# ethnhe/FFB6D

Measured on NVIDIA H100. Metric: fused KNN+gather points/sec at 12288 pts, higher is better.
Workload: dtype f32

## Files before the change

### ffb6d_b200/_lib.py

```python
import ctypes as C
import os

_HERE = os.path.dirname(os.path.abspath(__file__))
LIB_PATH = os.path.join(_HERE, "libffb6d_b200.so")

OK = 0
ERR_INVALID = -1
ERR_CUDA = -2
ERR_WORKSPACE = -3
ERR_NO_DEVICE = -4
LAYOUT_NCS = 0
LAYOUT_NSC = 1
MAX_K = 64


class FFB6DError(RuntimeError):

    def __init__(self, code, msg):
        super().__init__("libffb6d_b200 error %d: %s" % (code, msg))
        self.code = code


def _load():
    if not os.path.exists(LIB_PATH):
        raise ImportError(
            "%s not found: the CUDA library has not been built (run __graft_entry__.build() "
            "or `make -C ffb6d_b200/csrc`). There is no CPU fallback." % LIB_PATH)
    lib = C.CDLL(LIB_PATH)
    vp, i64, sz, ci, fp = C.c_void_p, C.c_int64, C.c_size_t, C.c_int, C.c_float
    sig = {
        "ffb6d_version": (ci, []),
        "ffb6d_last_error": (C.c_char_p, []),
        "ffb6d_device_count": (ci, []),
        "ffb6d_launch_count": (C.c_uint64, []),
        "ffb6d_knn_workspace_bytes": (sz, [i64, i64, i64, ci]),
        "ffb6d_knn_batch": (ci, [vp, vp, i64, i64, i64, ci, vp, ci, vp, sz, vp]),
        "ffb6d_knn_batch_algo": (ci, [vp, vp, i64, i64, i64, ci, vp, ci, vp, sz, ci, vp]),
        "ffb6d_knn_grid_bytes": (sz, [i64, i64]),
        "ffb6d_knn_grid_query_bytes": (sz, [i64, i64]),
        "ffb6d_knn_grid_build": (ci, [vp, i64, i64, ci, vp, sz, vp]),
        "ffb6d_knn_grid_query": (ci, [vp, vp, i64, i64, i64, ci, vp, ci, vp, sz, vp, sz, vp]),
        "ffb6d_knn_grid_query_organized": (ci, [vp, vp, i64, i64, i64, ci, vp, ci, vp, sz, vp, sz, i64, vp]),
        "ffb6d_knn_subset_nn": (ci, [vp, vp, i64, i64, i64, vp, ci, vp, ci, vp, sz, vp]),
        "ffb6d_build_indices_workspace_bytes": (sz, [i64, i64, i64, i64, ci]),
        "ffb6d_build_indices": (ci, [vp, vp, vp, vp, i64, i64, i64, i64, ci, vp, ci, vp, sz, vp]),
        "ffb6d_knn_grid_tune": (None, [fp, ci]),
        "ffb6d_knn_grid_tune_k1": (None, [fp]),
        "ffb6d_knn_batch_host": (ci, [vp, sz, sz, sz, vp, sz, sz, vp]),
        "ffb6d_knn_host": (ci, [vp, sz, sz, vp, sz, sz, vp]),
        "ffb6d_gather_max_fwd": (ci, [vp, vp, ci, i64, i64, i64, i64, ci, ci, vp, vp]),
        "ffb6d_check_indices": (ci, [vp, ci, i64, i64, vp]),
        "ffb6d_gather_kernel_name": (C.c_char_p, [i64, i64, i64, i64, ci, ci]),
        "ffb6d_gather_max_bwd": (ci, [vp, vp, ci, vp, i64, i64, i64, i64, ci, ci, vp, vp]),
        "ffb6d_gather_neighbour_fwd": (ci, [vp, vp, ci, i64, i64, i64, i64, ci, vp, vp]),
        "ffb6d_gather_neighbour_bwd": (ci, [vp, vp, ci, i64, i64, i64, i64, ci, vp, vp]),
        "ffb6d_relative_pos_encoding_fwd": (ci, [vp, vp, ci, i64, i64, ci, vp, vp]),
        "ffb6d_fusion_mlp_fwd": (ci, [vp, i64, vp, i64, vp, vp, vp, i64, i64, i64, ci, fp, vp, vp]),
        "ffb6d_fusion_mlp_pack_bytes": (sz, [i64, i64]),
        "ffb6d_fusion_mlp_pack": (ci, [vp, i64, i64, vp, sz, vp]),
        "ffb6d_fusion_mlp_fwd_packed": (ci, [vp, i64, vp, i64, vp, vp, vp, i64, i64, i64, ci, fp, vp, vp]),
        "ffb6d_fusion_mlp_fwd_ex": (ci, [vp, i64, vp, i64, vp, vp, vp, i64, i64, i64, ci, fp, vp, vp, ci, i64, ci, vp, vp]),
        "ffb6d_bn_workspace_bytes": (sz, [i64, i64]),
        "ffb6d_bn_train_fwd": (ci, [vp, i64, i64, i64, vp, vp, fp, fp, vp, vp, ci, fp, vp, vp, vp, sz, vp]),
        "ffb6d_bn_train_bwd": (ci, [vp, vp, vp, i64, i64, i64, ci, fp, vp, vp, vp, vp, sz, vp]),
        "ffb6d_bn_sync_moments": (ci, [vp, i64, i64, i64, vp, vp, sz, vp]),
        "ffb6d_bn_sync_fwd": (ci, [vp, i64, i64, i64, vp, i64, vp, vp, fp, fp, vp, vp, ci, fp, vp, vp, vp, vp]),
        "ffb6d_bn_sync_bwd_sums": (ci, [vp, vp, vp, i64, i64, i64, ci, fp, vp, vp, vp, vp, sz, vp]),
        "ffb6d_bn_sync_bwd": (ci, [vp, vp, vp, i64, i64, i64, vp, i64, vp, ci, fp, vp, vp, sz, vp]),
        "ffb6d_act_bwd": (ci, [vp, vp, i64, ci, fp, vp, vp]),
        "ffb6d_fusion_mlp_wgrad": (ci, [vp, vp, i64, vp, i64, i64, i64, i64, vp, vp]),
        "ffb6d_segment_plan_bytes": (sz, [i64, i64, i64]),
        "ffb6d_segment_plan": (ci, [vp, ci, i64, i64, i64, vp, sz, vp]),
        "ffb6d_segment_sum": (ci, [vp, vp, sz, i64, i64, i64, i64, vp, vp]),
        "ffb6d_segment_csr_bytes": (sz, [i64, i64, i64]),
        "ffb6d_segment_csr": (ci, [vp, ci, i64, i64, i64, vp, sz, vp]),
        "ffb6d_segment_sum_csr": (ci, [vp, vp, sz, i64, i64, i64, i64, vp, vp]),
        "ffb6d_gather_max_bwd_det_workspace_bytes": (sz, [i64, i64, i64, i64, ci]),
        "ffb6d_gather_max_bwd_det": (ci, [vp, vp, ci, vp, i64, i64, i64, i64, ci, ci, vp, sz, vp, vp]),
        "ffb6d_gather_neighbour_bwd_det_workspace_bytes": (sz, [i64, i64, i64, ci]),
        "ffb6d_gather_neighbour_bwd_det": (ci, [vp, vp, ci, i64, i64, i64, i64, ci, vp, sz, vp, vp]),
        "ffb6d_fusion_mlp_wgrad_det_workspace_bytes": (sz, [i64, i64, i64, i64, i64]),
        "ffb6d_fusion_mlp_wgrad_det": (ci, [vp, vp, i64, vp, i64, i64, i64, i64, vp, sz, vp, vp]),
        "ffb6d_att_pool_bwd": (ci, [vp, i64, vp, i64, vp, vp, i64, i64, ci, vp, vp, vp, vp]),
        "ffb6d_lfa_att_pool_fused": (ci, [vp, vp, ci, vp, vp, vp, vp, vp, vp, vp, vp, vp, vp, vp, i64, i64, ci, i64, i64, fp, vp, vp]),
        "ffb6d_att_pool_fwd": (ci, [vp, i64, vp, i64, vp, i64, i64, ci, vp, vp]),
        "ffb6d_relative_pos_encoding_cm_fwd": (ci, [vp, vp, ci, i64, i64, ci, vp, vp]),
        "ffb6d_backproject": (ci, [vp, i64, i64, i64, vp, ci, vp, i64, vp, vp, vp, vp, vp]),
        "ffb6d_sample_pixels_workspace_bytes": (sz, [i64, i64, i64]),
        "ffb6d_sample_pixels": (ci, [vp, i64, i64, i64, fp, i64, C.c_uint64, vp, vp, vp, sz, vp]),
        "ffb6d_fill_depth_workspace_bytes": (sz, [i64, i64, i64]),
        "ffb6d_fill_depth": (ci, [vp, i64, i64, i64, fp, vp, vp, vp, sz, vp]),
        "ffb6d_mean_shift_workspace_bytes": (sz, [i64, i64]),
        "ffb6d_mean_shift_fit": (ci, [vp, vp, i64, i64, i64, fp, ci, vp, vp, vp, vp, vp, sz, vp]),
        "ffb6d_best_fit_transform": (ci, [vp, vp, i64, i64, vp, vp]),
        "ffb6d_grid_subsample_host": (ci, [vp, sz, vp, sz, vp, sz, fp, vp, vp, vp, C.POINTER(sz)]),
    }
    for name, (res, args) in sig.items():
        fn = getattr(lib, name)
        fn.restype = res
        fn.argtypes = args
    return lib, sorted(sig)


lib, SYMBOLS = _load()


def last_error():
    return lib.ffb6d_last_error().decode("utf-8", "replace")


def check(rc):
    if rc != OK:
        raise FFB6DError(rc, last_error())


def launch_count():
    return int(lib.ffb6d_launch_count())
```

### ffb6d_b200/csrc/api.cu

```cuda
#include "common.cuh"
#include "knn_common.cuh"

#include <atomic>
#include <mutex>
#include <string.h>
#include <stdlib.h>

namespace ffb6d {

static thread_local char g_err[512] = "";
static std::atomic<uint64_t> g_launches{0};

void set_error(const char *fmt, ...)
{
    va_list ap;
    va_start(ap, fmt);
    vsnprintf(g_err, sizeof(g_err), fmt, ap);
    va_end(ap);
}
void count_launch(int n) { g_launches.fetch_add((uint64_t)n, std::memory_order_relaxed); }

int current_device()
{
    int dev = 0;
    if (cudaGetDevice(&dev) != cudaSuccess) {
        cudaGetLastError();
        dev = 0;
    }
    return dev;
}

const DeviceInfo &device_info()
{
    static DeviceInfo info[kMaxDevices];
    static std::atomic<unsigned long long> known{0};
    const int dev = current_device() & (kMaxDevices - 1);
    if (!((known.load(std::memory_order_acquire) >> dev) & 1ull)) {
        DeviceInfo d;
        if (cudaDeviceGetAttribute(&d.num_sms, cudaDevAttrMultiProcessorCount, dev) != cudaSuccess || d.num_sms < 1) {
            cudaGetLastError();
            d.num_sms = 132;
        }
        if (cudaDeviceGetAttribute(&d.max_smem_optin, cudaDevAttrMaxSharedMemoryPerBlockOptin, dev) != cudaSuccess) {
            cudaGetLastError();
            d.max_smem_optin = 48 * 1024;
        }
        info[dev] = d;
        known.fetch_or(1ull << dev, std::memory_order_release);
    }
    return info[dev];
}

const Env &env()
{
    static const Env e = [] {
        Env v;
        auto on = [](const char *n) { const char *x = getenv(n); return x && *x && strcmp(x, "0") != 0; };
        v.gather_direct = on("FFB6D_GATHER_DIRECT");
        v.check_indices = on("FFB6D_CHECK_INDICES");
        v.grid_thread_search = on("FFB6D_GRID_THREAD_SEARCH");
        v.subset_nn = on("FFB6D_SUBSET_NN");
        const char *x;
        v.grid_scale = (x = getenv("FFB6D_GRID_SCALE")) ? (float)atof(x) : 1.0f;
        v.grid_scale_k1 = (x = getenv("FFB6D_GRID_SCALE_K1")) ? (float)atof(x) : 2.5f;
        v.grid_quantile = (x = getenv("FFB6D_GRID_QUANTILE")) ? atoi(x) : 17;
        if (v.grid_quantile < 0) v.grid_quantile = 0;
        if (v.grid_quantile > 31) v.grid_quantile = 31;
        return v;
    }();
    return e;
}

struct HostScratch {
    std::mutex mu;
    void *buf[4] = {nullptr, nullptr, nullptr, nullptr};
    size_t cap[4] = {0, 0, 0, 0};
    int device = -1;
    int get(int slot, size_t bytes, void **out)
    {
        int dev = 0;
        FFB6D_CUDA(cudaGetDevice(&dev));
        if (dev != device) {
            for (int s = 0; s < 4; ++s) {
                if (buf[s]) {
                    cudaSetDevice(device);
                    cudaFree(buf[s]);
                    cudaSetDevice(dev);
                }
                buf[s] = nullptr;
                cap[s] = 0;
            }
            device = dev;
        }
        if (bytes > cap[slot]) {
            if (buf[slot]) FFB6D_CUDA(cudaFree(buf[slot]));
            buf[slot] = nullptr;
            cap[slot] = 0;
            const size_t want = align_up(bytes + bytes / 4, 1 << 20);
            FFB6D_CUDA(cudaMalloc(&buf[slot], want));
            cap[slot] = want;
        }
        *out = buf[slot];
        return FFB6D_OK;
    }
};
static HostScratch g_scratch;

static int knn_dispatch(const float *support, const float *query, int64_t B, int64_t S, int64_t Q,
                        int K, void *idx_out, int idx_is_i64, void *ws, size_t ws_bytes, int algo,
                        cudaStream_t st)
{
    FFB6D_CHECK_ARG(B >= 0 && S >= 0 && Q >= 0, "knn: negative size (B=%lld S=%lld Q=%lld)",
                    (long long)B, (long long)S, (long long)Q);
    FFB6D_CHECK_ARG(K >= 1 && K <= FFB6D_MAX_K, "knn: K=%d outside [1,%d]", K, FFB6D_MAX_K);
    FFB6D_CHECK_ARG(S < (1ll << 31) && Q < (1ll << 31) && B < 65536, "knn: size too large");
    FFB6D_CHECK_ARG(algo >= 0 && algo <= 2, "knn: unknown algo %d", algo);
    if (B == 0 || Q == 0) return FFB6D_OK;
    FFB6D_CHECK_ARG(query && idx_out, "knn: null query/idx_out");
    FFB6D_CHECK_ARG(S == 0 || support, "knn: null support");
    if (algo == 0) algo = knn_grid_workspace_bytes(B, S, Q, K) ? 2 : 1;
    if (algo == 2) {
        const size_t need = knn_grid_workspace_bytes(B, S, Q, K);
        if (need == 0) {
            algo = 1;
        } else {
            if (!ws || ws_bytes < need) {
                set_error("knn: workspace of %zu bytes required, %zu given", need, ws_bytes);
                return FFB6D_ERR_WORKSPACE;
            }
            return knn_grid_launch(support, query, B, S, Q, K, idx_out, idx_is_i64, ws, ws_bytes, st);
        }
    }
    return knn_brute_launch(support, query, B, S, Q, K, idx_out, idx_is_i64, st);
}

}

using namespace ffb6d;

extern "C" {

int ffb6d_version(void) { return 1; }
const char *ffb6d_last_error(void) { return g_err; }
uint64_t ffb6d_launch_count(void) { return g_launches.load(std::memory_order_relaxed); }

int ffb6d_device_count(void)
{
    int n = 0;
    if (cudaGetDeviceCount(&n) != cudaSuccess) {
        cudaGetLastError();
        return 0;
    }
    return n;
}

size_t ffb6d_knn_workspace_bytes(int64_t B, int64_t S, int64_t Q, int K)
{
    if (B <= 0 || S <= 0 || Q <= 0 || K < 1 || K > FFB6D_MAX_K) return 0;
    return knn_grid_workspace_bytes(B, S, Q, K);
}

int ffb6d_knn_batch(const float *support, const float *query, int64_t B, int64_t S, int64_t Q,
                    int K, void *idx_out, int idx_is_i64, void *workspace, size_t workspace_bytes,
                    ffb6d_stream_t stream)
{
    return knn_dispatch(support, query, B, S, Q, K, idx_out, idx_is_i64, workspace,
                        workspace_bytes, 0, (cudaStream_t)stream);
}

int ffb6d_knn_batch_algo(const float *support, const float *query, int64_t B, int64_t S, int64_t Q,
                         int K, void *idx_out, int idx_is_i64, void *workspace,
                         size_t workspace_bytes, int algo, ffb6d_stream_t stream)
{
    return knn_dispatch(support, query, B, S, Q, K, idx_out, idx_is_i64, workspace,
                        workspace_bytes, algo, (cudaStream_t)stream);
}

size_t ffb6d_knn_grid_bytes(int64_t B, int64_t S)
{
    if (B <= 0 || S <= 0) return 0;
    return knn_grid_store_bytes(B, S);
}

size_t ffb6d_knn_grid_query_bytes(int64_t B, int64_t Q)
{
    if (B <= 0 || Q <= 0) return 0;
    return knn_grid_query_bytes(B, Q);
}

int ffb6d_knn_grid_build(const float *support, int64_t B, int64_t S, int K_hint, void *grid,
                         size_t grid_bytes, ffb6d_stream_t stream)
{
    FFB6D_CHECK_ARG(B >= 1 && S >= 1 && B < 65536 && S < (1ll << 31), "knn_grid_build: bad size");
    FFB6D_CHECK_ARG(K_hint >= 1 && K_hint <= FFB6D_MAX_K, "knn_grid_build: K_hint=%d outside [1,%d]",
                    K_hint, FFB6D_MAX_K);
    FFB6D_CHECK_ARG(support && grid, "knn_grid_build: null pointer");
    return knn_grid_build(support, B, S, K_hint, grid, grid_bytes, (cudaStream_t)stream);
}

int ffb6d_knn_grid_query(const float *support, const float *query, int64_t B, int64_t S, int64_t Q,
                         int K, void *idx_out, int idx_is_i64, const void *grid, size_t grid_bytes,
                         void *scratch, size_t scratch_bytes, ffb6d_stream_t stream)
{
    FFB6D_CHECK_ARG(B >= 0 && S >= 1 && Q >= 0 && B < 65536 && S < (1ll << 31) && Q < (1ll << 31),
                    "knn_grid_query: bad size");
    FFB6D_CHECK_ARG(K >= 1 && K <= FFB6D_MAX_K, "knn_grid_query: K=%d outside [1,%d]", K, FFB6D_MAX_K);
    if (B == 0 || Q == 0) return FFB6D_OK;
    FFB6D_CHECK_ARG(support && query && idx_out && grid && scratch, "knn_grid_query: null pointer");
    return knn_grid_query(support, query, B, S, Q, K, idx_out, idx_is_i64, grid, grid_bytes, scratch,
                          scratch_bytes, (cudaStream_t)stream);
}

int ffb6d_knn_grid_query_organized(const float *support, const float *query, int64_t B, int64_t S, int64_t Q,
                                   int K, void *idx_out, int idx_is_i64, const void *grid, size_t grid_bytes,
                                   void *scratch, size_t scratch_bytes, int64_t query_width, ffb6d_stream_t stream)
{
    FFB6D_CHECK_ARG(B >= 0 && S >= 1 && Q >= 0 && B < 65536 && S < (1ll << 31) && Q < (1ll << 31),
                    "knn_grid_query: bad size");
    FFB6D_CHECK_ARG(K >= 1 && K <= FFB6D_MAX_K, "knn_grid_query: K=%d outside [1,%d]", K, FFB6D_MAX_K);
    FFB6D_CHECK_ARG(query_width >= 0 && (query_width == 0 || Q % query_width == 0),
                    "knn_grid_query: query_width=%lld does not divide Q=%lld", (long long)query_width, (long long)Q);
    if (B == 0 || Q == 0) return FFB6D_OK;
    FFB6D_CHECK_ARG(support && query && idx_out && grid && scratch, "knn_grid_query: null pointer");
    return knn_grid_query(support, query, B, S, Q, K, idx_out, idx_is_i64, grid, grid_bytes, scratch,
                          scratch_bytes, (cudaStream_t)stream, query_width);
}

int ffb6d_knn_subset_nn(const float *support, const float *query, int64_t B, int64_t S, int64_t Q, const void *knn_idx,
                        int K_list, void *idx_out, int idx_is_i64, void *scratch, size_t scratch_bytes,
                        ffb6d_stream_t stream)
{
    FFB6D_CHECK_ARG(B >= 0 && S >= 1 && Q >= 0 && B < 65536 && S < (1ll << 31) && Q < (1ll << 31),
                    "knn_subset_nn: bad size");
    FFB6D_CHECK_ARG(S <= Q || Q == 0, "knn_subset_nn: the support (%lld rows) must be a row prefix of the %lld queries",
                    (long long)S, (long long)Q);
    FFB6D_CHECK_ARG(K_list >= 1 && K_list <= FFB6D_MAX_K, "knn_subset_nn: K_list=%d outside [1,%d]", K_list, FFB6D_MAX_K);
    if (B == 0 || Q == 0) return FFB6D_OK;
    FFB6D_CHECK_ARG(support && query && knn_idx && idx_out && scratch, "knn_subset_nn: null pointer");
    return knn_subset_nn_from_knn(support, query, B, S, Q, knn_idx, K_list, idx_out, idx_is_i64, scratch, scratch_bytes,
                                  (cudaStream_t)stream);
}

void ffb6d_knn_grid_tune(float cell_scale, int quantile) { knn_grid_tune(cell_scale, quantile); }
void ffb6d_knn_grid_tune_k1(float cell_scale_k1) { knn_grid_tune_k1(cell_scale_k1); }

int ffb6d_knn_batch_host(const float *batch_data, size_t batch_size, size_t npts, size_t dim,
                         const float *queries, size_t nqueries, size_t K, long *batch_indices)
{
    FFB6D_CHECK_ARG(dim == 3, "knn_batch_host: dim=%zu, only 3 is supported", dim);
    FFB6D_CHECK_ARG(K >= 1 && K <= FFB6D_MAX_K, "knn_batch_host: K=%zu outside [1,%d]", K,
                    FFB6D_MAX_K);
    if (batch_size == 0 || nqueries == 0) return FFB6D_OK;
    FFB6D_CHECK_ARG(queries && batch_indices && (npts == 0 || batch_data),
                    "knn_batch_host: null pointer");
    if (ffb6d_device_count() == 0) {
        set_error("knn_batch_host: no CUDA device visible");
        return FFB6D_ERR_NO_DEVICE;
    }
    std::lock_guard<std::mutex> lock(g_scratch.mu);
    const size_t sup_b = batch_size * npts * 3 * sizeof(float);
    const size_t qry_b = batch_size * nqueries * 3 * sizeof(float);
    const size_t idx_b = batch_size * nqueries * K * sizeof(long);
    const size_t ws_b = ffb6d_knn_workspace_bytes((int64_t)batch_size, (int64_t)npts,
                                                  (int64_t)nqueries, (int)K);
    void *d_sup, *d_qry, *d_idx, *d_ws;
    int rc;
    if ((rc = g_scratch.get(0, sup_b ? sup_b : 16, &d_sup))) return rc;
    if ((rc = g_scratch.get(1, qry_b, &d_qry))) return rc;
    if ((rc = g_scratch.get(2, idx_b, &d_idx))) return rc;
    if ((rc = g_scratch.get(3, ws_b ? ws_b : 16, &d_ws))) return rc;
    cudaStream_t st = 0;
    if (sup_b) FFB6D_CUDA(cudaMemcpyAsync(d_sup, batch_data, sup_b, cudaMemcpyHostToDevice, st));
    FFB6D_CUDA(cudaMemcpyAsync(d_qry, queries, qry_b, cudaMemcpyHostToDevice, st));
    rc = knn_dispatch((const float *)d_sup, (const float *)d_qry, (int64_t)batch_size,
                      (int64_t)npts, (int64_t)nqueries, (int)K, d_idx, 1, d_ws, ws_b, 0, st);
    if (rc) return rc;
    FFB6D_CUDA(cudaMemcpyAsync(batch_indices, d_idx, idx_b, cudaMemcpyDeviceToHost, st));
    FFB6D_CUDA(cudaStreamSynchronize(st));
    return FFB6D_OK;
}

int ffb6d_knn_host(const float *points, size_t npts, size_t dim, const float *queries,
                   size_t nqueries, size_t K, long *indices)
{
    return ffb6d_knn_batch_host(points, 1, npts, dim, queries, nqueries, K, indices);
}

}
```

### ffb6d_b200/csrc/common.cuh

```cuda
#pragma once
#include <cuda_runtime.h>
#include <stdint.h>
#include <stdio.h>
#include <stdarg.h>
#include <atomic>

#include "../../include/ffb6d_b200.h"

namespace ffb6d {

void set_error(const char *fmt, ...);
void count_launch(int n = 1);

#define FFB6D_CHECK_ARG(cond, ...)                         \
    do {                                                   \
        if (!(cond)) {                                     \
            ::ffb6d::set_error(__VA_ARGS__);               \
            return FFB6D_ERR_INVALID;                      \
        }                                                  \
    } while (0)

#define FFB6D_CUDA(call)                                                             \
    do {                                                                             \
        cudaError_t e__ = (call);                                                    \
        if (e__ != cudaSuccess) {                                                    \
            ::ffb6d::set_error("%s failed: %s (%s:%d)", #call, cudaGetErrorString(e__), \
                               __FILE__, __LINE__);                                  \
            return FFB6D_ERR_CUDA;                                                   \
        }                                                                            \
    } while (0)

#define FFB6D_LAUNCH_OK(name)                                                          \
    do {                                                                               \
        cudaError_t e__ = cudaGetLastError();                                          \
        if (e__ != cudaSuccess) {                                                      \
            ::ffb6d::set_error("launch of %s failed: %s", name, cudaGetErrorString(e__)); \
            return FFB6D_ERR_CUDA;                                                     \
        }                                                                              \
        ::ffb6d::count_launch();                                                       \
    } while (0)

static inline int64_t ceil_div(int64_t a, int64_t b) { return (a + b - 1) / b; }
static inline size_t align_up(size_t x, size_t a) { return (x + a - 1) / a * a; }

constexpr int kMaxDevices = 64;
struct DeviceInfo {
    int num_sms;
    int max_smem_optin;
};
int current_device();
const DeviceInfo &device_info();
static inline int num_sms() { return device_info().num_sms; }

#define FFB6D_OPTIN_SMEM(kern, bytes)                                                              \
    do {                                                                                           \
        static std::atomic<unsigned long long> done__{0};                                          \
        const int dev__ = ::ffb6d::current_device() & (::ffb6d::kMaxDevices - 1);                  \
        if (!((done__.load(std::memory_order_relaxed) >> dev__) & 1ull)) {                         \
            FFB6D_CUDA(cudaFuncSetAttribute(kern, cudaFuncAttributeMaxDynamicSharedMemorySize,     \
                                            (int)(bytes)));                                        \
            done__.fetch_or(1ull << dev__, std::memory_order_relaxed);                             \
        }                                                                                          \
    } while (0)

int wgrad_small_launch(const float *grad_z, const float *x1, int64_t C1, const float *x2, int64_t C2, int64_t B, int64_t Co,
                       int64_t P, float *grad_w, cudaStream_t st);
int64_t wgrad_small_splits(int64_t B, int64_t P);
int wgrad_small_det_launch(const float *grad_z, const float *x1, int64_t C1, const float *x2, int64_t C2, int64_t B,
                           int64_t Co, int64_t P, float *part, cudaStream_t st);

struct Env {
    bool gather_direct;
    bool check_indices;
    bool grid_thread_search;
    bool subset_nn;
    float grid_scale, grid_scale_k1;
    int grid_quantile;
};
const Env &env();

__device__ __forceinline__ float ref_sqdist(float qx, float qy, float qz, float sx, float sy,
                                            float sz)
{
    const float dx = __fsub_rn(qx, sx);
    const float dy = __fsub_rn(qy, sy);
    const float dz = __fsub_rn(qz, sz);
    return __fadd_rn(__fadd_rn(__fmul_rn(dx, dx), __fmul_rn(dy, dy)), __fmul_rn(dz, dz));
}

}
```

### ffb6d_b200/csrc/knn_common.cuh

```cuda
#pragma once
#include "common.cuh"

namespace ffb6d {

template <int KCAP>
struct TopK {
    float d[KCAP];
    int i[KCAP];

    __device__ __forceinline__ void init()
    {
#pragma unroll
        for (int j = 0; j < KCAP; ++j) {
            d[j] = __int_as_float(0x7f800000);
            i[j] = 0;
        }
    }
    __device__ __forceinline__ float worst() const { return d[KCAP - 1]; }
    __device__ __forceinline__ float kth(int K) const
    {
        float v = d[KCAP - 1];
#pragma unroll
        for (int j = KCAP - 2; j >= 0; --j) v = (j >= K - 1) ? d[j] : v;
        return v;
    }
    __device__ __forceinline__ int worst_idx() const { return i[KCAP - 1]; }

    __device__ __forceinline__ void push_ordered(float dist, int id)
    {
#pragma unroll
        for (int j = KCAP - 1; j > 0; --j) {
            const bool shift = d[j - 1] > dist;
            const bool here = !shift && (d[j] > dist);
            const float nd = shift ? d[j - 1] : (here ? dist : d[j]);
            const int ni = shift ? i[j - 1] : (here ? id : i[j]);
            d[j] = nd;
            i[j] = ni;
        }
        if (d[0] > dist) {
            d[0] = dist;
            i[0] = id;
        }
    }

    __device__ __forceinline__ bool accepts(float dist, int id) const
    {
        return dist < d[KCAP - 1] || (dist == d[KCAP - 1] && id < i[KCAP - 1]);
    }

    __device__ __forceinline__ void push_any(float dist, int id)
    {
#pragma unroll
        for (int j = KCAP - 1; j > 0; --j) {
            const bool shift = d[j - 1] > dist || (d[j - 1] == dist && i[j - 1] > id);
            const bool after = d[j] > dist || (d[j] == dist && i[j] > id);
            const bool here = !shift && after;
            const float nd = shift ? d[j - 1] : (here ? dist : d[j]);
            const int ni = shift ? i[j - 1] : (here ? id : i[j]);
            d[j] = nd;
            i[j] = ni;
        }
        if (d[0] > dist || (d[0] == dist && i[0] > id)) {
            d[0] = dist;
            i[0] = id;
        }
    }
};

int knn_brute_launch(const float *support, const float *query, int64_t B, int64_t S, int64_t Q,
                     int K, void *idx_out, int idx_is_i64, cudaStream_t st);
size_t knn_grid_workspace_bytes(int64_t B, int64_t S, int64_t Q, int K);
int knn_grid_launch(const float *support, const float *query, int64_t B, int64_t S, int64_t Q,
                    int K, void *idx_out, int idx_is_i64, void *workspace, size_t workspace_bytes,
                    cudaStream_t st);
void knn_grid_tune(float cell_scale, int quantile);
void knn_grid_tune_k1(float cell_scale_k1);
size_t knn_grid_store_bytes(int64_t B, int64_t S);
size_t knn_grid_query_bytes(int64_t B, int64_t Q);
int knn_grid_build(const float *support, int64_t B, int64_t S, int K, void *grid_mem,
                   size_t grid_bytes, cudaStream_t st);
int knn_grid_query(const float *support, const float *query, int64_t B, int64_t S, int64_t Q, int K,
                   void *idx_out, int idx_is_i64, const void *grid_mem, size_t grid_bytes,
                   void *scratch, size_t scratch_bytes, cudaStream_t st, int64_t query_width = 0);

int knn_subset_nn_from_knn(const float *support, const float *query, int64_t B, int64_t S, int64_t Q, const void *knn,
                           int KL, void *idx_out, int idx_is_i64, void *scratch, size_t scratch_bytes, cudaStream_t st);

}
```

### ffb6d_b200/csrc/knn_grid.cu

```cuda
#include "common.cuh"
#include "knn_common.cuh"

#include <algorithm>
#include <cooperative_groups.h>
#include <math.h>
#include <stdlib.h>

namespace ffb6d {

constexpr int RMAX = 4;
constexpr int N_SAMPLES = 32;
constexpr int BUILD_CTAS = 8;
constexpr int BUILD_THREADS = 512;
constexpr int BUILD_WARPS = BUILD_THREADS / 32;
constexpr int BUILD_GT = BUILD_CTAS * BUILD_THREADS;
static_assert(N_SAMPLES == BUILD_CTAS * 4 && BUILD_WARPS == 16, "4 samples per CTA, 4 warps per sample");

struct __align__(16) GridParams {
    float lo[3];
    float h;
    float inv_h;
    float slack;
    int n[3];
    int ncells;
    float hi[3];
    int pad[3];
};
static_assert(sizeof(GridParams) == 64, "GridParams layout");

struct __align__(16) QueryState {
    int ovf_count;
    int dup_count;
    int rep_q;
    int pad;
};

struct GridStore {
    GridParams *params;
    int *cursor;
    int *rank;
    float4 *sorted;
    size_t maxc;
    size_t bytes;
};

struct QueryScratch {
    QueryState *state;
    int *ovf;
    size_t bytes;
};

static size_t max_cells_for(int64_t S)
{
    size_t m = (size_t)S * 8;
    if (m < 4096) m = 4096;
    if (m > ((size_t)1 << 22)) m = (size_t)1 << 22;
    return (m + 4095) / 4096 * 4096;
}

static GridStore carve_grid(void *base, int64_t B, int64_t S)
{
    GridStore w;
    w.maxc = max_cells_for(S);
    size_t off = 0;
    char *p = (char *)base;
    auto take = [&](size_t bytes) {
        char *r = p + off;
        off = align_up(off + bytes, 256);
        return r;
    };
    w.params = (GridParams *)take((size_t)B * sizeof(GridParams));
    w.cursor = (int *)take((size_t)B * w.maxc * sizeof(int));
    w.rank = (int *)take((size_t)B * (size_t)S * sizeof(int));
    w.sorted = (float4 *)take((size_t)B * (size_t)S * sizeof(float4));
    w.bytes = off;
    return w;
}

static QueryScratch carve_query(void *base, int64_t B, int64_t Q)
{
    QueryScratch w;
    size_t off = 0;
    char *p = (char *)base;
    w.state = (QueryState *)(p + off);
    off = align_up(off + (size_t)B * sizeof(QueryState), 256);
    w.ovf = (int *)(p + off);
    off = align_up(off + (size_t)B * (size_t)Q * sizeof(int), 256);
    w.bytes = off;
    return w;
}

size_t knn_grid_store_bytes(int64_t B, int64_t S) { return carve_grid(nullptr, B, S).bytes; }
size_t knn_grid_query_bytes(int64_t B, int64_t Q) { return carve_query(nullptr, B, Q).bytes; }

static bool grid_worthwhile(int64_t B, int64_t S, int64_t Q, int K)
{
    (void)B;
    (void)K;
    return S >= 512 && (double)S * (double)Q >= 2.0e5;
}

size_t knn_grid_workspace_bytes(int64_t B, int64_t S, int64_t Q, int K)
{
    if (!grid_worthwhile(B, S, Q, K)) return 0;
    return knn_grid_store_bytes(B, S) + knn_grid_query_bytes(B, Q);
}

__device__ __forceinline__ int cell_of(float p, float lo, float inv_h, int n)
{
    const int c = (int)floorf((p - lo) * inv_h);
    return min(max(c, 0), n - 1);
}

__global__ void __cluster_dims__(BUILD_CTAS, 1, 1) __launch_bounds__(BUILD_THREADS)
grid_build_kernel(const float *__restrict__ support, int S, int K, int maxc, float cell_scale, int quantile,
                  GridParams *__restrict__ params, int *__restrict__ cursor_all, int *__restrict__ rank_all,
                  float4 *__restrict__ sorted_all)
{
    namespace cg = cooperative_groups;
    cg::cluster_group cluster = cg::this_cluster();
    const int crank = (int)cluster.block_rank();
    const int b = blockIdx.y;
    const int tid = threadIdx.x, lane = tid & 31, wid = tid >> 5;
    const int gtid = crank * BUILD_THREADS + tid;
    const float *sup = support + (size_t)b * S * 3;
    int *cur = cursor_all + (size_t)b * maxc;
    int *rnk = rank_all + (size_t)b * S;
    float4 *sorted = sorted_all + (size_t)b * S;
    const float INF = __int_as_float(0x7f800000);

    __shared__ float s_red[6][BUILD_WARPS];
    __shared__ float s_box[6];
    __shared__ float s_cand[4][4][4];
    __shared__ float s_est[4];
    __shared__ float s_all[N_SAMPLES];
    __shared__ float s_pick;
    __shared__ GridParams s_P;
    __shared__ int s_tot[BUILD_CTAS];
    __shared__ int s_wsum[BUILD_WARPS];
    __shared__ int s_base;

    {
        float mn[3] = {INF, INF, INF}, mx[3] = {-INF, -INF, -INF};
        for (int s = gtid; s < S; s += BUILD_GT) {
#pragma unroll
            for (int a = 0; a < 3; ++a) {
                const float v = __ldg(sup + (size_t)s * 3 + a);
                mn[a] = fminf(mn[a], v);
                mx[a] = fmaxf(mx[a], v);
            }
        }
#pragma unroll
        for (int a = 0; a < 3; ++a) {
#pragma unroll
            for (int o = 16; o > 0; o >>= 1) {
                mn[a] = fminf(mn[a], __shfl_xor_sync(0xffffffffu, mn[a], o));
                mx[a] = fmaxf(mx[a], __shfl_xor_sync(0xffffffffu, mx[a], o));
            }
            if (lane == 0) {
                s_red[a][wid] = mn[a];
                s_red[3 + a][wid] = mx[a];
            }
        }
        if (tid < BUILD_CTAS) s_tot[tid] = 0;
        __syncthreads();
        if (wid == 0) {
#pragma unroll
            for (int a = 0; a < 3; ++a) {
                float u = lane < BUILD_WARPS ? s_red[a][lane] : INF, v = lane < BUILD_WARPS ? s_red[3 + a][lane] : -INF;
#pragma unroll
                for (int o = 16; o > 0; o >>= 1) {
                    u = fminf(u, __shfl_xor_sync(0xffffffffu, u, o));
                    v = fmaxf(v, __shfl_xor_sync(0xffffffffu, v, o));
                }
                if (lane == 0) {
                    s_box[a] = u;
                    s_box[3 + a] = v;
                }
            }
        }
    }
    {
        const int stride = max((S + 4095) / 4096, (K + 3) / 4);
        const int kk = max(1, (K + stride - 1) / stride);
        const int smp = crank * 4 + (wid >> 2), w4 = wid & 3;
        const int me = (int)((((long long)smp * S) / N_SAMPLES + S / (2 * N_SAMPLES)) % max(S, 1));
        float out[4] = {INF, INF, INF, INF};
        if (S > 1) {
            const float qx = __ldg(sup + (size_t)me * 3), qy = __ldg(sup + (size_t)me * 3 + 1),
                        qz = __ldg(sup + (size_t)me * 3 + 2);
            TopK<4> t4;
            t4.init();
            const int nsub = (S + stride - 1) / stride;
            for (int i0 = w4 * 32 + lane; i0 < nsub; i0 += 4 * 128) {
                float px[4], py[4], pz[4];
#pragma unroll
                for (int u = 0; u < 4; ++u) {
                    const int s = min((i0 + u * 128) * stride, S - 1);
                    px[u] = __ldg(sup + (size_t)s * 3);
                    py[u] = __ldg(sup + (size_t)s * 3 + 1);
                    pz[u] = __ldg(sup + (size_t)s * 3 + 2);
                }
#pragma unroll
                for (int u = 0; u < 4; ++u) {
                    const int i = i0 + u * 128, s = i * stride;
                    const float d = ref_sqdist(qx, qy, qz, px[u], py[u], pz[u]);
                    if (i < nsub && s != me && d < t4.worst()) t4.push_ordered(d, s);
                }
            }
#pragma unroll
            for (int round = 0; round < 4; ++round) {
                if (round >= kk) break;
                float m = t4.d[0];
#pragma unroll
                for (int o = 16; o > 0; o >>= 1) m = fminf(m, __shfl_xor_sync(0xffffffffu, m, o));
                const unsigned who = __ballot_sync(0xffffffffu, t4.d[0] == m);
                if (lane == __ffs(who) - 1) {
                    t4.d[0] = t4.d[1];
                    t4.d[1] = t4.d[2];
                    t4.d[2] = t4.d[3];
                    t4.d[3] = INF;
                }
                out[round] = m;
            }
        }
        if (lane == 0) {
#pragma unroll
            for (int j = 0; j < 4; ++j) s_cand[wid >> 2][w4][j] = out[j];
        }
        __syncthreads();
        if (wid < 4) {
            const float mine = lane < 16 ? s_cand[wid][lane >> 2][lane & 3] : INF;
            int rank = 0;
            for (int j = 0; j < 16; ++j) {
                const float o = __shfl_sync(0xffffffffu, mine, j);
                rank += (o < mine || (o == mine && j < lane)) ? 1 : 0;
            }
            if (lane < 16 && rank == kk - 1) {
                const float r = (S > 1) ? sqrtf(mine) * sqrtf((float)K / (float)(kk * stride)) : 0.f;
                s_est[wid] = (r == r && r < INF) ? r : 0.f;
            }
        }
    }
    cluster.sync();
    if (crank == 0) {
        if (wid == 0) {
            s_all[lane] = cluster.map_shared_rank(s_est, lane >> 2)[lane & 3];
            if (lane < 6) {
                float v = (lane < 3) ? INF : -INF;
                for (int c = 0; c < BUILD_CTAS; ++c) {
                    const float o = cluster.map_shared_rank(s_box, c)[lane];
                    v = (lane < 3) ? fminf(v, o) : fmaxf(v, o);
                }
                s_red[lane][0] = v;
            }
            __syncwarp();
            const float mine = s_all[lane];
            int rank = 0;
            for (int j = 0; j < N_SAMPLES; ++j) {
                const float o = s_all[j];
                rank += (o < mine || (o == mine && j < lane)) ? 1 : 0;
            }
            if (rank == quantile) s_pick = mine;
            __syncwarp();
            if (lane == 0) {
                float mn[3], mx[3];
                for (int a = 0; a < 3; ++a) {
                    mn[a] = s_red[a][0];
                    mx[a] = s_red[3 + a][0];
                }
                const float r_est = s_pick;
                GridParams P;
                float L[3], scale = 0.f;
                bool finite = true;
                for (int a = 0; a < 3; ++a) {
                    L[a] = mx[a] - mn[a];
                    finite = finite && isfinite(L[a]) && isfinite(mn[a]);
                    scale = fmaxf(scale, fmaxf(fabsf(mn[a]), fabsf(mx[a])));
                    P.lo[a] = mn[a];
                    P.hi[a] = mx[a];
                }
                const float l1 = fmaxf(L[0], fmaxf(L[1], L[2]));
                const float l3 = fminf(L[0], fminf(L[1], L[2]));
                const float l2 = L[0] + L[1] + L[2] - l1 - l3;
                float h = cell_scale * r_est;
                if (!(h > 0.f)) h = sqrtf((float)K * l1 * l2 / (float)max(S, 1));
                if (!(h > 0.f)) h = l1 * (float)K / (float)max(S, 1);
                int n[3] = {1, 1, 1};
                if (finite && h > 0.f && l1 > 0.f) {
                    for (int it = 0; it < 200; ++it) {
                        double prod = 1.0;
                        for (int a = 0; a < 3; ++a) {
                            const float f = floorf(L[a] / h);
                            n[a] = (f >= 4.0e6f) ? 4000000 : (int)f + 1;
                            prod *= (double)n[a];
                        }
                        if (prod <= (double)maxc) break;
                        h *= 1.2f;
                        if (it == 199) n[0] = n[1] = n[2] = 1;
                    }
                }
                const bool single = (n[0] == 1 && n[1] == 1 && n[2] == 1);
                P.h = single ? INF : h;
                P.inv_h = single ? 0.f : 1.0f / h;
                P.slack = 1e-5f * (scale + l1) + 1e-30f;
                P.n[0] = n[0];
                P.n[1] = n[1];
                P.n[2] = n[2];
                P.ncells = n[0] * n[1] * n[2];
                for (int a = 0; a < 3; ++a) P.pad[a] = 0;
                s_P = P;
                params[b] = P;
            }
        }
    }
    cluster.sync();
    if (crank != 0 && tid < 16)
        reinterpret_cast<float *>(&s_P)[tid] = reinterpret_cast<const float *>(cluster.map_shared_rank(&s_P, 0))[tid];
    __syncthreads();
    const GridParams P = s_P;
    const int ncells = P.ncells;
    const int slice = ((ncells + BUILD_CTAS * 128 - 1) / (BUILD_CTAS * 128)) * 128;
    {
        int4 *c4 = reinterpret_cast<int4 *>(cur);
        const int n4 = min((ncells + 3) / 4, maxc / 4);
        for (int i = gtid; i < n4; i += BUILD_GT) c4[i] = make_int4(0, 0, 0, 0);
    }
    cluster.sync();
    {
        int acc = 0;
        const int iters = (S + BUILD_GT - 1) / BUILD_GT;
        for (int it = 0; it < iters; ++it) {
            const int s = it * BUILD_GT + gtid;
            int sl = -1;
            if (s < S) {
                const float *p = sup + (size_t)s * 3;
                const int cx = cell_of(__ldg(p), P.lo[0], P.inv_h, P.n[0]);
                const int cy = cell_of(__ldg(p + 1), P.lo[1], P.inv_h, P.n[1]);
                const int cz = cell_of(__ldg(p + 2), P.lo[2], P.inv_h, P.n[2]);
                const int cell = (cz * P.n[1] + cy) * P.n[0] + cx;
                rnk[s] = atomicAdd(cur + cell, 1);
                sl = cell / slice;
            }
#pragma unroll
            for (int j = 0; j < BUILD_CTAS; ++j) {
                const int v = __popc(__ballot_sync(0xffffffffu, sl == j));
                if (lane == j) acc += v;
            }
        }
        if (lane < BUILD_CTAS && acc) atomicAdd(&s_tot[lane], acc);
    }
    cluster.sync();
    {
        if (wid == 0) {
            int t = 0;
            if (lane < BUILD_CTAS)
                for (int c = 0; c < BUILD_CTAS; ++c) t += cluster.map_shared_rank(s_tot, c)[lane];
            int before = (lane < crank) ? t : 0;
#pragma unroll
            for (int o = 16; o > 0; o >>= 1) before += __shfl_xor_sync(0xffffffffu, before, o);
            if (lane == 0) s_base = before;
        }
        const int lo = crank * slice, hi = min(ncells, lo + slice);
        const int run = ((slice / 128 + BUILD_WARPS - 1) / BUILD_WARPS) * 128;
        const int wlo = min(hi, lo + wid * run), whi = min(hi, wlo + run);
        int tot = 0;
        for (int i = wlo + 4 * lane; i < whi; i += 128) {
            const int4 v = *reinterpret_cast<const int4 *>(cur + i);
            tot += v.x + (i + 1 < whi ? v.y : 0) + (i + 2 < whi ? v.z : 0) + (i + 3 < whi ? v.w : 0);
        }
#pragma unroll
        for (int o = 16; o > 0; o >>= 1) tot += __shfl_xor_sync(0xffffffffu, tot, o);
        if (lane == 0) s_wsum[wid] = tot;
        __syncthreads();
        int carry = s_base;
        for (int w = 0; w < wid; ++w) carry += s_wsum[w];
        for (int i0 = wlo; i0 < whi; i0 += 128) {
            const int i = i0 + 4 * lane;
            int4 v = make_int4(0, 0, 0, 0);
            if (i < whi) {
                v = *reinterpret_cast<const int4 *>(cur + i);
                if (i + 1 >= whi) v.y = 0;
                if (i + 2 >= whi) v.z = 0;
                if (i + 3 >= whi) v.w = 0;
            }
            const int t = v.x + v.y + v.z + v.w;
            int incl = t;
#pragma unroll
            for (int o = 1; o < 32; o <<= 1) {
                const int u = __shfl_up_sync(0xffffffffu, incl, o);
                if (lane >= o) incl += u;
            }
            const int start = carry + incl - t;
            if (i < whi) {
                int4 e;
                e.x = start + v.x;
                e.y = e.x + v.y;
                e.z = e.y + v.z;
                e.w = e.z + v.w;
                if (i + 3 < whi) {
                    *reinterpret_cast<int4 *>(cur + i) = e;
                } else {
                    cur[i] = e.x;
                    if (i + 1 < whi) cur[i + 1] = e.y;
                    if (i + 2 < whi) cur[i + 2] = e.z;
                }
            }
            carry += __shfl_sync(0xffffffffu, incl, 31);
        }
    }
    cluster.sync();
    for (int s = gtid; s < S; s += BUILD_GT) {
        const float *p = sup + (size_t)s * 3;
        const float x = __ldg(p), y = __ldg(p + 1), z = __ldg(p + 2);
        const int cx = cell_of(x, P.lo[0], P.inv_h, P.n[0]);
        const int cy = cell_of(y, P.lo[1], P.inv_h, P.n[1]);
        const int cz = cell_of(z, P.lo[2], P.inv_h, P.n[2]);
        const int cell = (cz * P.n[1] + cy) * P.n[0] + cx;
        const int pos = (cell > 0 ? cur[cell - 1] : 0) + rnk[s];
        sorted[pos] = make_float4(x, y, z, __int_as_float(s));
    }
}

__constant__ signed char kRowOrder[81][2] = {{0,0}, {-1,0}, {0,-1}, {0,1}, {1,0}, {-1,-1}, {-1,1}, {1,-1}, {1,1}, {-2,0}, {0,-2}, {0,2}, {2,0}, {-2,-1}, {-2,1}, {-1,-2}, {-1,2}, {1,-2}, {1,2}, {2,-1}, {2,1}, {-2,-2}, {-2,2}, {2,-2}, {2,2}, {-3,0}, {0,-3}, {0,3}, {3,0}, {-3,-1}, {-3,1}, {-1,-3}, {-1,3}, {1,-3}, {1,3}, {3,-1}, {3,1}, {-3,-2}, {-3,2}, {-2,-3}, {-2,3}, {2,-3}, {2,3}, {3,-2}, {3,2}, {-3,-3}, {-3,3}, {3,-3}, {3,3}, {-4,0}, {0,-4}, {0,4}, {4,0}, {-4,-1}, {-4,1}, {-1,-4}, {-1,4}, {1,-4}, {1,4}, {4,-1}, {4,1}, {-4,-2}, {-4,2}, {-2,-4}, {-2,4}, {2,-4}, {2,4}, {4,-2}, {4,2}, {-4,-3}, {-4,3}, {-3,-4}, {-3,4}, {3,-4}, {3,4}, {4,-3}, {4,3}, {-4,-4}, {-4,4}, {4,-4}, {4,4}};

__device__ __forceinline__ float slab_dist2(float q, float lo, float h, int c, float slack)
{
    const float a = lo + (float)c * h, b = lo + (float)(c + 1) * h;
    const float d = fmaxf(fmaxf(a - q, q - b) - slack, 0.f);
    return d * d;
}

template <int KCAP>
__device__ __forceinline__ bool thread_search(float qx, float qy, float qz, int K, const GridParams &Ps,
                                              const int *__restrict__ cell_end, const float4 *__restrict__ sorted,
                                              TopK<KCAP> &top)
{
    const int nx = Ps.n[0], ny = Ps.n[1], nz = Ps.n[2];
    const float h = Ps.h, slack = Ps.slack;
    const int cx = cell_of(qx, Ps.lo[0], Ps.inv_h, nx);
    const int cy = cell_of(qy, Ps.lo[1], Ps.inv_h, ny);
    const int cz = cell_of(qz, Ps.lo[2], Ps.inv_h, nz);
    const float INF = __int_as_float(0x7f800000);
    const float out = fmaxf(fmaxf(fmaxf(Ps.lo[0] - qx, qx - Ps.hi[0]), fmaxf(Ps.lo[1] - qy, qy - Ps.hi[1])),
                            fmaxf(Ps.lo[2] - qz, qz - Ps.hi[2]));
    bool done = false;
    auto scan_range = [&](int beg, int end) {
        for (int p = beg; p < end; p += 4) {
            float4 c[4];
#pragma unroll
            for (int u = 0; u < 4; ++u) c[u] = __ldg(sorted + min(p + u, end - 1));
#pragma unroll
            for (int u = 0; u < 4; ++u) {
                const float d = ref_sqdist(qx, qy, qz, c[u].x, c[u].y, c[u].z);
                const int id = __float_as_int(c[u].w);
                if (p + u < end && top.accepts(d, id)) top.push_any(d, id);
            }
        }
    };
    auto cells = [&](int row, int a, int b2) {
        const int beg = (row + a > 0) ? __ldg(cell_end + row + a - 1) : 0;
        scan_range(beg, __ldg(cell_end + row + b2));
    };
    const int r_first = (out > (float)RMAX * h) ? RMAX + 1 : 1;
    int px0 = 1, px1 = 0, py0 = 1, py1 = 0, pz0 = 1, pz1 = 0;
    for (int r = r_first; r <= RMAX && !done; ++r) {
        const int x0 = max(cx - r, 0), x1 = min(cx + r, nx - 1);
        const int y0 = max(cy - r, 0), y1 = min(cy + r, ny - 1);
        const int z0 = max(cz - r, 0), z1 = min(cz + r, nz - 1);
        const int e0 = (2 * r - 1) * (2 * r - 1) * (r > r_first ? 1 : 0);
        const int e1 = (2 * r + 1) * (2 * r + 1);
        if (r > r_first) {
            for (int e = 0; e < e0; ++e) {
                const int z = cz + kRowOrder[e][0], y = cy + kRowOrder[e][1];
                if (z < pz0 || z > pz1 || y < py0 || y > py1) continue;
                const int row = (z * ny + y) * nx;
                if (x0 < px0) cells(row, x0, px0 - 1);
                if (x1 > px1) cells(row, px1 + 1, x1);
            }
        }
        for (int e = e0; e < e1; ++e) {
            const int z = cz + kRowOrder[e][0], y = cy + kRowOrder[e][1];
            if (z < z0 || z > z1 || y < y0 || y > y1) continue;
            const float dmin2 = slab_dist2(qy, Ps.lo[1], h, y, slack) + slab_dist2(qz, Ps.lo[2], h, z, slack);
            if (dmin2 > top.kth(K)) continue;
            cells((z * ny + y) * nx, x0, x1);
        }
        px0 = x0; px1 = x1; py0 = y0; py1 = y1; pz0 = z0; pz1 = z1;
        float m = INF;
        if (x0 > 0) m = fminf(m, qx - (Ps.lo[0] + (float)x0 * h));
        if (x1 < nx - 1) m = fminf(m, (Ps.lo[0] + (float)(x1 + 1) * h) - qx);
        if (y0 > 0) m = fminf(m, qy - (Ps.lo[1] + (float)y0 * h));
        if (y1 < ny - 1) m = fminf(m, (Ps.lo[1] + (float)(y1 + 1) * h) - qy);
        if (z0 > 0) m = fminf(m, qz - (Ps.lo[2] + (float)z0 * h));
        if (z1 < nz - 1) m = fminf(m, (Ps.lo[2] + (float)(z1 + 1) * h) - qz);
        if (m == INF) {
            done = true;
        } else {
            const float ms = m - slack;
            const float kth = top.kth(K);
            done = ms > 0.f && kth <= ms * ms * (1.0f - 1e-5f);
        }
    }
    return done;
}

__device__ __forceinline__ void register_overflow(const float *__restrict__ query, int Q, int b, int q, float qx, float qy,
                                                  float qz, QueryState *state_all, int *__restrict__ ovf_all)
{
    QueryState *Pw = state_all + b;
    int rep = *(volatile int *)&Pw->rep_q;
    if (rep == 0) rep = atomicCAS(&Pw->rep_q, 0, q + 1);
    rep -= 1;
    bool dup = false;
    if (rep != -1 && rep != q) {
        const float *rp = query + ((size_t)b * Q + rep) * 3;
        dup = (__ldg(rp) == qx) && (__ldg(rp + 1) == qy) && (__ldg(rp + 2) == qz);
    }
    if (dup) {
        auto g = cooperative_groups::coalesced_threads();
        int base = 0;
        if (g.thread_rank() == 0) base = atomicAdd(&Pw->dup_count, (int)g.size());
        const int slot = g.shfl(base, 0) + (int)g.thread_rank();
        ovf_all[(size_t)b * Q + (Q - 1 - slot)] = q;
    } else {
        auto g = cooperative_groups::coalesced_threads();
        int base = 0;
        if (g.thread_rank() == 0) base = atomicAdd(&Pw->ovf_count, (int)g.size());
        const int slot = g.shfl(base, 0) + (int)g.thread_rank();
        ovf_all[(size_t)b * Q + slot] = q;
    }
}

template <int KCAP, typename IdxT, bool SELF>
__global__ void __launch_bounds__(128)
grid_search_kernel(const float *__restrict__ query, int S, int Q, int K,
                   const GridParams *__restrict__ params_all, const int *__restrict__ cursor_all,
                   size_t cursor_stride, const float4 *__restrict__ sorted_all,
                   IdxT *__restrict__ idx_out, QueryState *state_all, int *__restrict__ ovf_all)
{
    const int b = blockIdx.y;
    const int t = blockIdx.x * blockDim.x + threadIdx.x;
    if (t >= Q) return;
    const GridParams Ps = params_all[b];
    const int *cell_end = cursor_all + (size_t)b * cursor_stride;
    const float4 *sorted = sorted_all + (size_t)b * S;
    float qx, qy, qz;
    int q;
    if (SELF) {
        const float4 me = sorted[t];
        qx = me.x;
        qy = me.y;
        qz = me.z;
        q = __float_as_int(me.w);
    } else {
        const float *qp = query + ((size_t)b * Q + t) * 3;
        qx = __ldg(qp);
        qy = __ldg(qp + 1);
        qz = __ldg(qp + 2);
        q = t;
    }
    TopK<KCAP> top;
    top.init();
    if (thread_search<KCAP>(qx, qy, qz, K, Ps, cell_end, sorted, top)) {
        IdxT *o = idx_out + ((size_t)b * Q + q) * K;
#pragma unroll
        for (int j = 0; j < KCAP; ++j)
            if (j < K) o[j] = (IdxT)top.i[j];
        return;
    }
    register_overflow(query, Q, b, q, qx, qy, qz, state_all, ovf_all);
}

typedef unsigned long long key_t64;

__device__ __forceinline__ key_t64 make_key(float d, int i)
{
    return ((key_t64)__float_as_uint(d) << 32) | (unsigned)i;
}
__device__ __forceinline__ float key_dist(key_t64 k) { return __uint_as_float((unsigned)(k >> 32)); }

constexpr key_t64 KEY_EMPTY = 0x7f80000000000000ull;
constexpr key_t64 KEY_INVALID = 0x7f8000007fffffffull;

__device__ __forceinline__ void warp_minmax(key_t64 &k, int j, bool keep_min)
{
    const key_t64 o = __shfl_xor_sync(0xffffffffu, k, j);
    if ((o < k) == keep_min) k = o;
}

__device__ __forceinline__ void warp_sort(key_t64 &k, int lane)
{
#pragma unroll
    for (int kk = 2; kk <= 32; kk <<= 1) {
#pragma unroll
        for (int j = kk >> 1; j > 0; j >>= 1) {
            const bool up = (lane & kk) == 0;
            warp_minmax(k, j, ((lane & j) == 0) == up);
        }
    }
}

__device__ __forceinline__ void warp_list_offer(key_t64 &mine, key_t64 cand, int K, int lane, bool &list_empty)
{
    const unsigned FULL = 0xffffffffu;
    if (list_empty) {
        warp_sort(cand, lane);
        mine = (cand < KEY_EMPTY) ? cand : KEY_EMPTY;
        list_empty = false;
        return;
    }
    const key_t64 thr = __shfl_sync(FULL, mine, K - 1);
    unsigned mask = __ballot_sync(FULL, cand < thr);
    if (__popc(mask) > 12) {
        warp_sort(cand, lane);
        const key_t64 rev = __shfl_sync(FULL, cand, 31 - lane);
        if (rev < mine) mine = rev;
#pragma unroll
        for (int jj = 16; jj > 0; jj >>= 1) warp_minmax(mine, jj, (lane & jj) == 0);
        if (mine > KEY_EMPTY) mine = KEY_EMPTY;
    } else {
        while (mask) {
            const int src = __ffs(mask) - 1;
            mask &= mask - 1;
            const key_t64 x = __shfl_sync(FULL, cand, src);
            const key_t64 pred = __shfl_up_sync(FULL, mine, 1);
            if (x < mine) mine = (lane > 0 && x < pred) ? pred : x;
        }
    }
}


template <typename IdxT>
__device__ __forceinline__ void register_far_k1(const float *__restrict__ query, int Q, int b, int q, float qx, float qy,
                                                float qz, QueryState *state_all, int *__restrict__ ovf_all,
                                                IdxT *__restrict__ idx_out)
{
    QueryState *Pw = state_all + b;
    int rep = *(volatile int *)&Pw->rep_q;
    if (rep == 0) rep = atomicCAS(&Pw->rep_q, 0, q + 1);
    rep -= 1;
    bool dup = false;
    if (rep != -1 && rep != q) {
        const float *rp = query + ((size_t)b * Q + rep) * 3;
        dup = (__ldg(rp) == qx) && (__ldg(rp + 1) == qy) && (__ldg(rp + 2) == qz);
    }
    if (dup) {
        idx_out[(size_t)b * Q + q] = (IdxT)-1;
    } else {
        auto g = cooperative_groups::coalesced_threads();
        int base = 0;
        if (g.thread_rank() == 0) base = atomicAdd(&Pw->ovf_count, (int)g.size());
        const int slot = g.shfl(base, 0) + (int)g.thread_rank();
        ovf_all[(size_t)b * Q + slot] = q;
    }
}

template <typename IdxT>
__global__ void __launch_bounds__(256)
grid_far_fill_kernel(int Q, const QueryState *__restrict__ state_all, IdxT *__restrict__ idx_out)
{
    const int b = blockIdx.y;
    const int rep = state_all[b].rep_q - 1;
    if (rep < 0) return;
    IdxT *o = idx_out + (size_t)b * Q;
    const IdxT v = o[rep];
    for (int q = blockIdx.x * blockDim.x + threadIdx.x; q < Q; q += gridDim.x * blockDim.x)
        if (o[q] == (IdxT)-1) o[q] = v;
}

template <typename IdxT, int NW>
__global__ void __launch_bounds__(NW * 32, 1024 / (NW * 32))
grid_search_k1_tile_kernel(const float *__restrict__ query, int S, int Q, int qw, int qh, int tiles_x, int n_tiles, int exact_div,
                            const GridParams *__restrict__ params_all, const int *__restrict__ cursor_all,
                            size_t cursor_stride, const float4 *__restrict__ sorted_all,
                            IdxT *__restrict__ idx_out, QueryState *state_all, int *__restrict__ ovf_all)
{
    constexpr int TW = 8, TH = 4;
    constexpr int MAX_ROWS = 32, MAX_X = 8;
    constexpr int TILE_CAND = 128;
    __shared__ float4 s_cand[NW][TILE_CAND];
    __shared__ int s_list[NW * 32];
    __shared__ int s_count;
    const unsigned FULL = 0xffffffffu;
    const int b = blockIdx.y;
    const int lane = threadIdx.x & 31, wid = threadIdx.x >> 5;
    const int tile = blockIdx.x * NW + wid;
    const GridParams Ps = params_all[b];
    const int *cell_end = cursor_all + (size_t)b * cursor_stride;
    const float4 *sorted = sorted_all + (size_t)b * S;
    const float INF = __int_as_float(0x7f800000);
    if (threadIdx.x == 0) s_count = 0;
    if (NW > 1) __syncthreads();
    else __syncwarp();

    const int trow = exact_div ? tile / tiles_x : (int)(((float)tile + 0.5f) * (1.0f / (float)tiles_x));
    const int px = (tile - trow * tiles_x) * TW + (lane & (TW - 1)), py = trow * TH + (lane >> 3);
    const bool inimg = tile < n_tiles && px < qw && py < qh;
    const int q = inimg ? py * qw + px : 0;
    float qx = 0.f, qy = 0.f, qz = 0.f;
    if (inimg) {
        const float *qp = query + ((size_t)b * Q + q) * 3;
        qx = __ldg(qp);
        qy = __ldg(qp + 1);
        qz = __ldg(qp + 2);
    }
    const int nx = Ps.n[0], ny = Ps.n[1], nz = Ps.n[2];
    const float h = Ps.h, slack = Ps.slack;
    const float out = fmaxf(fmaxf(fmaxf(Ps.lo[0] - qx, qx - Ps.hi[0]), fmaxf(Ps.lo[1] - qy, qy - Ps.hi[1])),
                            fmaxf(Ps.lo[2] - qz, qz - Ps.hi[2]));
    int state = !inimg ? 3 : ((out > (float)RMAX * h || !(qx == qx && qy == qy && qz == qz)) ? 2 : 1);
    const bool part = state == 1;
    const int cx = cell_of(qx, Ps.lo[0], Ps.inv_h, nx);
    const int cy = cell_of(qy, Ps.lo[1], Ps.inv_h, ny);
    const int cz = cell_of(qz, Ps.lo[2], Ps.inv_h, nz);
    const int big = 0x3fffffff;
    int X0 = __reduce_min_sync(FULL, part ? cx : big), X1 = __reduce_max_sync(FULL, part ? cx : -1);
    int Y0 = __reduce_min_sync(FULL, part ? cy : big), Y1 = __reduce_max_sync(FULL, part ? cy : -1);
    int Z0 = __reduce_min_sync(FULL, part ? cz : big), Z1 = __reduce_max_sync(FULL, part ? cz : -1);
    if (X1 >= 0) {
        X0 = max(X0 - 1, 0); X1 = min(X1 + 1, nx - 1);
        Y0 = max(Y0 - 1, 0); Y1 = min(Y1 + 1, ny - 1);
        Z0 = max(Z0 - 1, 0); Z1 = min(Z1 + 1, nz - 1);
        const int by = Y1 - Y0 + 1, nrows = by * (Z1 - Z0 + 1);
        if (nrows <= MAX_ROWS && X1 - X0 + 1 <= MAX_X) {
            int beg = 0, end = 0;
            if (lane < nrows) {
                const int rz = (int)(((float)lane + 0.5f) * (1.0f / (float)by));
                const int row = ((Z0 + rz) * ny + (Y0 + lane - rz * by)) * nx;
                beg = (row + X0 > 0) ? __ldg(cell_end + row + X0 - 1) : 0;
                end = __ldg(cell_end + row + X1);
            }
            const int cnt = end - beg;
            int incl = cnt;
#pragma unroll
            for (int o = 1; o < 32; o <<= 1) {
                const int u = __shfl_up_sync(FULL, incl, o);
                if (lane >= o) incl += u;
            }
            const int total = __shfl_sync(FULL, incl, 31);
            const int excl = incl - cnt;
            float4 *stage = s_cand[wid];
            key_t64 best = KEY_EMPTY;
            for (int c0 = 0; c0 < total; c0 += TILE_CAND) {
                const int n = min(TILE_CAND, total - c0);
                const int n4 = (n + 3) & ~3;
                __syncwarp();
                for (int u0 = 0; u0 < n4; u0 += 32) {
                    const int j = c0 + u0 + lane;
                    int seg = 0;
#pragma unroll
                    for (int step = 16; step > 0; step >>= 1) {
                        const int v = __shfl_sync(FULL, incl, seg + step - 1);
                        if (v <= j) seg += step;
                    }
                    const int sb = __shfl_sync(FULL, beg, seg & 31), se = __shfl_sync(FULL, excl, seg & 31);
                    float4 c = make_float4(INF, INF, INF, __int_as_float(0x7fffffff));
                    if (j < total) c = __ldg(sorted + sb + (j - se));
                    if (u0 + lane < n4) stage[u0 + lane] = c;
                }
                __syncwarp();
                for (int p = 0; p < n4; p += 4) {
                    float4 c[4];
#pragma unroll
                    for (int u = 0; u < 4; ++u) c[u] = stage[p + u];
#pragma unroll
                    for (int u = 0; u < 4; ++u) {
                        const key_t64 k = make_key(ref_sqdist(qx, qy, qz, c[u].x, c[u].y, c[u].z), __float_as_int(c[u].w));
                        best = k < best ? k : best;
                    }
                }
            }
            if (part) {
                const float bd = key_dist(best);
                float m = INF;
                if (X0 > 0) m = fminf(m, qx - (Ps.lo[0] + (float)X0 * h));
                if (X1 < nx - 1) m = fminf(m, (Ps.lo[0] + (float)(X1 + 1) * h) - qx);
                if (Y0 > 0) m = fminf(m, qy - (Ps.lo[1] + (float)Y0 * h));
                if (Y1 < ny - 1) m = fminf(m, (Ps.lo[1] + (float)(Y1 + 1) * h) - qy);
                if (Z0 > 0) m = fminf(m, qz - (Ps.lo[2] + (float)Z0 * h));
                if (Z1 < nz - 1) m = fminf(m, (Ps.lo[2] + (float)(Z1 + 1) * h) - qz);
                const float ms = m - slack;
                const bool ok = (m == INF) ? (bd < INF || S == 0) : (ms > 0.f && bd <= ms * ms * (1.0f - 1e-5f));
                if (ok) {
                    idx_out[(size_t)b * Q + q] = (IdxT)(unsigned)(best & 0xffffffffu);
                    state = 0;
                }
            }
        }
    }
    if (state == 1) s_list[atomicAdd(&s_count, 1)] = q;
    if (NW > 1) __syncthreads();
    else __syncwarp();
    const int n_retry = s_count;
    int q2 = -1;
    float rx = 0.f, ry = 0.f, rz = 0.f;
    bool retry_failed = false;
    if ((int)threadIdx.x < n_retry) {
        q2 = s_list[threadIdx.x];
        const float *qp = query + ((size_t)b * Q + q2) * 3;
        rx = __ldg(qp);
        ry = __ldg(qp + 1);
        rz = __ldg(qp + 2);
        TopK<1> top;
        top.init();
        if (thread_search<1>(rx, ry, rz, 1, Ps, cell_end, sorted, top))
            idx_out[(size_t)b * Q + q2] = (IdxT)top.i[0];
        else
            retry_failed = true;
    }
    if (retry_failed) register_overflow(query, Q, b, q2, rx, ry, rz, state_all, ovf_all);
    if (state == 2) register_far_k1<IdxT>(query, Q, b, q, qx, qy, qz, state_all, ovf_all, idx_out);
}

template <typename IdxT, bool SELF>
__global__ void __launch_bounds__(256, 5)
grid_search_warp_kernel(const float *__restrict__ query, int S, int Q, int K,
                        const GridParams *__restrict__ params_all, const int *__restrict__ cursor_all,
                        size_t cursor_stride, const float4 *__restrict__ sorted_all,
                        IdxT *__restrict__ idx_out, QueryState *state_all, int *__restrict__ ovf_all)
{
    const unsigned FULL = 0xffffffffu;
    const int b = blockIdx.y;
    const int lane = threadIdx.x & 31;
    const int t = blockIdx.x * (blockDim.x >> 5) + (threadIdx.x >> 5);
    if (t >= Q) return;
    const GridParams Ps = params_all[b];
    const int *cell_end = cursor_all + (size_t)b * cursor_stride;
    const float4 *sorted = sorted_all + (size_t)b * S;
    float qx, qy, qz;
    int q;
    if (SELF) {
        const float4 me = __ldg(sorted + t);
        qx = me.x;
        qy = me.y;
        qz = me.z;
        q = __float_as_int(me.w);
    } else {
        const float *qp = query + ((size_t)b * Q + t) * 3;
        qx = __ldg(qp);
        qy = __ldg(qp + 1);
        qz = __ldg(qp + 2);
        q = t;
    }
    const int nx = Ps.n[0], ny = Ps.n[1], nz = Ps.n[2];
    const float h = Ps.h, slack = Ps.slack;
    const int cx = cell_of(qx, Ps.lo[0], Ps.inv_h, nx);
    const int cy = cell_of(qy, Ps.lo[1], Ps.inv_h, ny);
    const int cz = cell_of(qz, Ps.lo[2], Ps.inv_h, nz);
    const float INF = __int_as_float(0x7f800000);
    const float out = fmaxf(fmaxf(fmaxf(Ps.lo[0] - qx, qx - Ps.hi[0]), fmaxf(Ps.lo[1] - qy, qy - Ps.hi[1])),
                            fmaxf(Ps.lo[2] - qz, qz - Ps.hi[2]));

    auto margin = [&](int r) {
        float m = INF;
        if (cx - r > 0) m = fminf(m, qx - (Ps.lo[0] + (float)(cx - r) * h));
        if (cx + r < nx - 1) m = fminf(m, (Ps.lo[0] + (float)(cx + r + 1) * h) - qx);
        if (cy - r > 0) m = fminf(m, qy - (Ps.lo[1] + (float)(cy - r) * h));
        if (cy + r < ny - 1) m = fminf(m, (Ps.lo[1] + (float)(cy + r + 1) * h) - qy);
        if (cz - r > 0) m = fminf(m, qz - (Ps.lo[2] + (float)(cz - r) * h));
        if (cz + r < nz - 1) m = fminf(m, (Ps.lo[2] + (float)(cz + r + 1) * h) - qz);
        return m;
    };

    key_t64 mine = KEY_EMPTY;
    bool list_empty = true;
    bool done = false;
    int r = (out > (float)RMAX * h) ? RMAX + 1 : 1;
    int e_prev = 0;
    int px0 = 0, px1 = -1;
    while (r <= RMAX) {
        const int x0 = max(cx - r, 0), x1 = min(cx + r, nx - 1);
        const int y0 = max(cy - r, 0), y1 = min(cy + r, ny - 1);
        const int z0 = max(cz - r, 0), z1 = min(cz + r, nz - 1);
        const int e_end = (2 * r + 1) * (2 * r + 1);
        const int nseg = 2 * e_prev + (e_end - e_prev);
        for (int s0 = 0; s0 < nseg; s0 += 32) {
            const float kth_now = key_dist(__shfl_sync(FULL, mine, K - 1));
            const int sidx = s0 + lane;
            int beg = 0, end = 0;
            if (sidx < nseg) {
                const bool old = sidx < 2 * e_prev;
                const int e = old ? (sidx >> 1) : (sidx - e_prev);
                const int z = cz + kRowOrder[e][0], y = cy + kRowOrder[e][1];
                int a = x0, c = x1;
                if (old) {
                    if (sidx & 1) a = px1 + 1;
                    else c = px0 - 1;
                }
                if (z >= z0 && z <= z1 && y >= y0 && y <= y1 && a <= c) {
                    const float dmin2 = slab_dist2(qy, Ps.lo[1], h, y, slack) + slab_dist2(qz, Ps.lo[2], h, z, slack);
                    if (!(dmin2 > kth_now)) {
                        const int row = (z * ny + y) * nx;
                        beg = (row + a > 0) ? __ldg(cell_end + row + a - 1) : 0;
                        end = __ldg(cell_end + row + c);
                    }
                }
            }
            const int cnt = end - beg;
            int incl = cnt;
#pragma unroll
            for (int o = 1; o < 32; o <<= 1) {
                const int u = __shfl_up_sync(FULL, incl, o);
                if (lane >= o) incl += u;
            }
            const int total = __shfl_sync(FULL, incl, 31);
            const int excl = incl - cnt;
            for (int j0 = 0; j0 < total; j0 += 32) {
                const int j = j0 + lane;
                int seg = 0;
#pragma unroll
                for (int step = 16; step > 0; step >>= 1) {
                    const int v = __shfl_sync(FULL, incl, seg + step - 1);
                    if (v <= j) seg += step;
                }
                const int sb = __shfl_sync(FULL, beg, seg);
                const int se = __shfl_sync(FULL, excl, seg);
                key_t64 cand = KEY_INVALID;
                if (j < total) {
                    const float4 c = __ldg(sorted + sb + (j - se));
                    cand = make_key(ref_sqdist(qx, qy, qz, c.x, c.y, c.z), __float_as_int(c.w));
                }
                warp_list_offer(mine, cand, K, lane, list_empty);
            }
        }
        e_prev = e_end;
        px0 = x0;
        px1 = x1;
        const float m = margin(r);
        const float kth = key_dist(__shfl_sync(FULL, mine, K - 1));
        if (m == INF) {
            done = true;
            break;
        }
        const float ms = m - slack;
        if (ms > 0.f && kth <= ms * ms * (1.0f - 1e-5f)) {
            done = true;
            break;
        }
        int rn = r + 1;
        if (kth < INF) {
            const float need = sqrtf(kth) * (1.0f + 1e-4f) + slack;
            while (rn <= RMAX && margin(rn) < need) ++rn;
        }
        r = rn;
    }
    if (done) {
        if (lane < K) idx_out[((size_t)b * Q + q) * K + lane] = (IdxT)(unsigned)(mine & 0xffffffffu);
        return;
    }
    if (lane == 0) {
        QueryState *Pw = state_all + b;
        const int rep = atomicCAS(&Pw->rep_q, 0, q + 1) - 1;
        bool dup = false;
        if (rep != -1 && rep != q) {
            const float *rp = query + ((size_t)b * Q + rep) * 3;
            dup = (__ldg(rp) == qx) && (__ldg(rp + 1) == qy) && (__ldg(rp + 2) == qz);
        }
        if (dup) {
            const int slot = atomicAdd(&Pw->dup_count, 1);
            ovf_all[(size_t)b * Q + (Q - 1 - slot)] = q;
        } else {
            const int slot = atomicAdd(&Pw->ovf_count, 1);
            ovf_all[(size_t)b * Q + slot] = q;
        }
    }
}

template <int W>
__device__ __forceinline__ void group_minmax(key_t64 &k, int j, bool keep_min)
{
    const key_t64 o = __shfl_xor_sync(0xffffffffu, k, j, W);
    if ((o < k) == keep_min) k = o;
}

template <int W>
__device__ __forceinline__ void group_sort(key_t64 &k, int sub)
{
#pragma unroll
    for (int kk = 2; kk <= W; kk <<= 1) {
#pragma unroll
        for (int j = kk >> 1; j > 0; j >>= 1) {
            const bool up = (sub & kk) == 0;
            group_minmax<W>(k, j, ((sub & j) == 0) == up);
        }
    }
}

template <typename IdxT, bool SELF, int W>
__global__ void __launch_bounds__(256, 5)
grid_search_group_kernel(const float *__restrict__ query, int S, int Q, int K,
                         const GridParams *__restrict__ params_all, const int *__restrict__ cursor_all,
                         size_t cursor_stride, const float4 *__restrict__ sorted_all,
                         IdxT *__restrict__ idx_out, QueryState *state_all, int *__restrict__ ovf_all)
{
    constexpr int G = 32 / W;
    const unsigned FULL = 0xffffffffu;
    const int b = blockIdx.y;
    const int lane = threadIdx.x & 31, sub = lane & (W - 1), grp = lane / W;
    const int t = (blockIdx.x * (blockDim.x >> 5) + (threadIdx.x >> 5)) * G + grp;
    if ((blockIdx.x * (blockDim.x >> 5) + (threadIdx.x >> 5)) * G >= Q) return;
    const bool valid = t < Q;
    const int tq = valid ? t : Q - 1;
    const GridParams Ps = params_all[b];
    const int *cell_end = cursor_all + (size_t)b * cursor_stride;
    const float4 *sorted = sorted_all + (size_t)b * S;
    float qx, qy, qz;
    int q;
    if (SELF) {
        const float4 me = __ldg(sorted + tq);
        qx = me.x;
        qy = me.y;
        qz = me.z;
        q = __float_as_int(me.w);
    } else {
        const float *qp = query + ((size_t)b * Q + tq) * 3;
        qx = __ldg(qp);
        qy = __ldg(qp + 1);
        qz = __ldg(qp + 2);
        q = tq;
    }
    const int nx = Ps.n[0], ny = Ps.n[1], nz = Ps.n[2];
    const float h = Ps.h, slack = Ps.slack;
    const int cx = cell_of(qx, Ps.lo[0], Ps.inv_h, nx);
    const int cy = cell_of(qy, Ps.lo[1], Ps.inv_h, ny);
    const int cz = cell_of(qz, Ps.lo[2], Ps.inv_h, nz);
    const float INF = __int_as_float(0x7f800000);
    const float out = fmaxf(fmaxf(fmaxf(Ps.lo[0] - qx, qx - Ps.hi[0]), fmaxf(Ps.lo[1] - qy, qy - Ps.hi[1])),
                            fmaxf(Ps.lo[2] - qz, qz - Ps.hi[2]));
    auto margin = [&](int r) {
        float m = INF;
        if (cx - r > 0) m = fminf(m, qx - (Ps.lo[0] + (float)(cx - r) * h));
        if (cx + r < nx - 1) m = fminf(m, (Ps.lo[0] + (float)(cx + r + 1) * h) - qx);
        if (cy - r > 0) m = fminf(m, qy - (Ps.lo[1] + (float)(cy - r) * h));
        if (cy + r < ny - 1) m = fminf(m, (Ps.lo[1] + (float)(cy + r + 1) * h) - qy);
        if (cz - r > 0) m = fminf(m, qz - (Ps.lo[2] + (float)(cz - r) * h));
        if (cz + r < nz - 1) m = fminf(m, (Ps.lo[2] + (float)(cz + r + 1) * h) - qz);
        return m;
    };

    key_t64 mine = KEY_EMPTY;
    bool done = false;
    int r = (out > (float)RMAX * h) ? RMAX + 1 : 1;
    bool active = valid && r <= RMAX;
    int e_prev = 0, px0 = 0, px1 = -1;
    while (__any_sync(FULL, active)) {
        const int x0 = max(cx - r, 0), x1 = min(cx + r, nx - 1);
        const int y0 = max(cy - r, 0), y1 = min(cy + r, ny - 1);
        const int z0 = max(cz - r, 0), z1 = min(cz + r, nz - 1);
        const int e_end = (2 * r + 1) * (2 * r + 1);
        const int nseg = active ? 2 * e_prev + (e_end - e_prev) : 0;
        for (int s0 = 0; __any_sync(FULL, s0 < nseg); s0 += W) {
            const float kth_now = key_dist(__shfl_sync(FULL, mine, K - 1, W));
            const int sidx = s0 + sub;
            int beg = 0, end = 0;
            if (sidx < nseg) {
                const bool old = sidx < 2 * e_prev;
                const int e = old ? (sidx >> 1) : (sidx - e_prev);
                const int z = cz + kRowOrder[e][0], y = cy + kRowOrder[e][1];
                int a = x0, c = x1;
                if (old) {
                    if (sidx & 1) a = px1 + 1;
                    else c = px0 - 1;
                }
                if (z >= z0 && z <= z1 && y >= y0 && y <= y1 && a <= c) {
                    const float dmin2 = slab_dist2(qy, Ps.lo[1], h, y, slack) + slab_dist2(qz, Ps.lo[2], h, z, slack);
                    if (!(dmin2 > kth_now)) {
                        const int row = (z * ny + y) * nx;
                        beg = (row + a > 0) ? __ldg(cell_end + row + a - 1) : 0;
                        end = __ldg(cell_end + row + c);
                    }
                }
            }
            const int cnt = end - beg;
            int incl = cnt;
#pragma unroll
            for (int o = 1; o < W; o <<= 1) {
                const int u = __shfl_up_sync(FULL, incl, o, W);
                if (sub >= o) incl += u;
            }
            const int total = __shfl_sync(FULL, incl, W - 1, W);
            const int excl = incl - cnt;
            for (int j0 = 0; __any_sync(FULL, j0 < total); j0 += W) {
                const int j = j0 + sub;
                int seg = 0;
#pragma unroll
                for (int step = W / 2; step > 0; step >>= 1) {
                    const int v = __shfl_sync(FULL, incl, seg + step - 1, W);
                    if (v <= j) seg += step;
                }
                const int sb = __shfl_sync(FULL, beg, seg, W);
                const int se = __shfl_sync(FULL, excl, seg, W);
                key_t64 cand = KEY_INVALID;
                if (j < total) {
                    const float4 c = __ldg(sorted + sb + (j - se));
                    cand = make_key(ref_sqdist(qx, qy, qz, c.x, c.y, c.z), __float_as_int(c.w));
                }
                const key_t64 thr = __shfl_sync(FULL, mine, K - 1, W);
                const unsigned ball = __ballot_sync(FULL, cand < thr);
                unsigned mask = (W == 32) ? ball : ((ball >> (W * grp)) & ((1u << W) - 1u));
                if (__any_sync(FULL, __popc(mask) > (3 * W) / 8)) {
                    group_sort<W>(cand, sub);
                    const key_t64 rev = __shfl_sync(FULL, cand, W - 1 - sub, W);
                    if (rev < mine) mine = rev;
#pragma unroll
                    for (int jj = W / 2; jj > 0; jj >>= 1) group_minmax<W>(mine, jj, (sub & jj) == 0);
                    if (mine > KEY_EMPTY) mine = KEY_EMPTY;
                } else {
                    while (__any_sync(FULL, mask != 0)) {
                        const int src = mask ? __ffs(mask) - 1 : 0;
                        key_t64 x = __shfl_sync(FULL, cand, src, W);
                        if (!mask) x = KEY_INVALID;
                        mask &= mask - 1;
                        const key_t64 pred = __shfl_up_sync(FULL, mine, 1, W);
                        if (x < mine) mine = (sub > 0 && x < pred) ? pred : x;
                    }
                }
            }
        }
        const float kth = key_dist(__shfl_sync(FULL, mine, K - 1, W));
        if (active) {
            e_prev = e_end;
            px0 = x0;
            px1 = x1;
            const float m = margin(r);
            if (m == INF) {
                done = true;
                active = false;
            } else {
                const float ms = m - slack;
                if (ms > 0.f && kth <= ms * ms * (1.0f - 1e-5f)) {
                    done = true;
                    active = false;
                } else {
                    int rn = r + 1;
                    if (kth < INF) {
                        const float need = sqrtf(kth) * (1.0f + 1e-4f) + slack;
                        while (rn <= RMAX && margin(rn) < need) ++rn;
                    }
                    r = rn;
                    active = r <= RMAX;
                }
            }
        }
    }
    if (!valid) return;
    if (done) {
        if (sub < K) idx_out[((size_t)b * Q + q) * K + sub] = (IdxT)(unsigned)(mine & 0xffffffffu);
        return;
    }
    if (sub == 0) {
        QueryState *Pw = state_all + b;
        const int rep = atomicCAS(&Pw->rep_q, 0, q + 1) - 1;
        bool dup = false;
        if (rep != -1 && rep != q) {
            const float *rp = query + ((size_t)b * Q + rep) * 3;
            dup = (__ldg(rp) == qx) && (__ldg(rp + 1) == qy) && (__ldg(rp + 2) == qz);
        }
        if (dup) {
            const int slot = atomicAdd(&Pw->dup_count, 1);
            ovf_all[(size_t)b * Q + (Q - 1 - slot)] = q;
        } else {
            const int slot = atomicAdd(&Pw->ovf_count, 1);
            ovf_all[(size_t)b * Q + slot] = q;
        }
    }
}

template <int KCAP, int THREADS, int TILE, typename IdxT>
__global__ void __launch_bounds__(THREADS)
grid_overflow_kernel(const float *__restrict__ support, const float *__restrict__ query, int S,
                     int Q, int K, const QueryState *__restrict__ state_all,
                     const int *__restrict__ ovf_all, IdxT *__restrict__ idx_out)
{
    const int b = blockIdx.y;
    const int count = state_all[b].ovf_count;
    __shared__ float4 tile[TILE];
    const float *sup = support + (size_t)b * S * 3;
    for (int first = blockIdx.x * THREADS; first < count; first += gridDim.x * THREADS) {
        const int t = first + threadIdx.x;
        const bool active = t < count;
        int q = 0;
        float qx = 0.f, qy = 0.f, qz = 0.f;
        if (active) {
            q = ovf_all[(size_t)b * Q + t];
            const float *qp = query + ((size_t)b * Q + q) * 3;
            qx = __ldg(qp);
            qy = __ldg(qp + 1);
            qz = __ldg(qp + 2);
        }
        TopK<KCAP> top;
        top.init();
        for (int s0 = 0; s0 < S; s0 += TILE) {
            const int n = min(TILE, S - s0);
            __syncthreads();
            const float *src = sup + (size_t)s0 * 3;
            for (int i = threadIdx.x; i < 3 * n; i += THREADS)
                reinterpret_cast<float *>(tile)[(i / 3) * 4 + (i % 3)] = __ldg(src + i);
            __syncthreads();
            if (active) {
#pragma unroll 4
                for (int i = 0; i < n; ++i) {
                    const float4 p = tile[i];
                    const float d = ref_sqdist(qx, qy, qz, p.x, p.y, p.z);
                    if (d < top.worst()) top.push_ordered(d, s0 + i);
                }
            }
        }
        if (active) {
            IdxT *o = idx_out + ((size_t)b * Q + q) * K;
#pragma unroll
            for (int j = 0; j < KCAP; ++j)
                if (j < K) o[j] = (IdxT)top.i[j];
        }
    }
}

template <typename IdxT>
__global__ void __launch_bounds__(256)
grid_overflow_warp_kernel(const float *__restrict__ support, const float *__restrict__ query, int S,
                          int Q, int K, QueryState *state_all, const int *__restrict__ ovf_all,
                          IdxT *__restrict__ idx_out)
{
    __shared__ key_t64 lists[8][32];
    __shared__ int last_flag;
    const int b = blockIdx.y;
    const int count = state_all[b].ovf_count;
    const int lane = threadIdx.x & 31, wid = threadIdx.x >> 5;
    const float *sup = support + (size_t)b * S * 3;
    for (int t = blockIdx.x; t < count; t += gridDim.x) {
        const int q = ovf_all[(size_t)b * Q + t];
        const float *qp = query + ((size_t)b * Q + q) * 3;
        const float qx = __ldg(qp), qy = __ldg(qp + 1), qz = __ldg(qp + 2);
        key_t64 mine = KEY_EMPTY;
        bool list_empty = true;
        for (int s0 = wid * 32; s0 < S; s0 += 8 * 32) {
            const int sI = s0 + lane;
            key_t64 cand = KEY_INVALID;
            if (sI < S)
                cand = make_key(ref_sqdist(qx, qy, qz, __ldg(sup + (size_t)sI * 3), __ldg(sup + (size_t)sI * 3 + 1),
                                           __ldg(sup + (size_t)sI * 3 + 2)), sI);
            warp_list_offer(mine, cand, K, lane, list_empty);
        }
        lists[wid][lane] = mine;
        __syncthreads();
        if (wid == 0) {
            list_empty = false;
            for (int w = 1; w < 8; ++w) warp_list_offer(mine, lists[w][lane], K, lane, list_empty);
            if (lane < K) idx_out[((size_t)b * Q + q) * K + lane] = (IdxT)(unsigned)(mine & 0xffffffffu);
        }
        __syncthreads();
    }
    const int dups = state_all[b].dup_count;
    if (dups == 0) return;
    __threadfence();
    __syncthreads();
    if (threadIdx.x == 0) last_flag = (atomicAdd(&state_all[b].pad, 1) == (int)gridDim.x - 1);
    __syncthreads();
    if (!last_flag) return;
    __threadfence();
    const int rep = state_all[b].rep_q - 1;
    const IdxT *src = idx_out + ((size_t)b * Q + rep) * K;
    for (int t = threadIdx.x; t < dups * K; t += blockDim.x) {
        const int q = ovf_all[(size_t)b * Q + (Q - 1 - t / K)];
        idx_out[((size_t)b * Q + q) * K + t % K] = __ldcg(src + t % K);
    }
}

template <typename IdxT>
__global__ void __launch_bounds__(256)
grid_dup_copy_kernel(int Q, int K, const QueryState *__restrict__ state_all,
                     const int *__restrict__ ovf_all, IdxT *__restrict__ idx_out)
{
    const int b = blockIdx.y;
    const int count = state_all[b].dup_count;
    const int rep = state_all[b].rep_q - 1;
    if (count == 0) return;
    const IdxT *src = idx_out + ((size_t)b * Q + rep) * K;
    for (int t = blockIdx.x * blockDim.x + threadIdx.x; t < count * K; t += gridDim.x * blockDim.x) {
        const int q = ovf_all[(size_t)b * Q + (Q - 1 - t / K)];
        idx_out[((size_t)b * Q + q) * K + t % K] = src[t % K];
    }
}

template <typename IdxT>
__global__ void __launch_bounds__(256)
subset_nn_from_knn_kernel(const IdxT *__restrict__ knn, int Q, int KL, int S, IdxT *__restrict__ idx_out,
                          QueryState *state_all, int *__restrict__ ovf_all)
{
    const int b = blockIdx.y;
    const int q = blockIdx.x * blockDim.x + threadIdx.x;
    if (q >= Q) return;
    const IdxT *row = knn + ((size_t)b * Q + q) * KL;
    const int kl = min(KL, Q);
    for (int j = 0; j < kl; ++j) {
        const IdxT v = __ldg(row + j);
        if (v >= 0 && v < (IdxT)S) {
            idx_out[(size_t)b * Q + q] = v;
            return;
        }
    }
    auto g = cooperative_groups::coalesced_threads();
    int base = 0;
    if (g.thread_rank() == 0) base = atomicAdd(&state_all[b].ovf_count, (int)g.size());
    ovf_all[(size_t)b * Q + g.shfl(base, 0) + (int)g.thread_rank()] = q;
}

int knn_subset_nn_from_knn(const float *support, const float *query, int64_t B, int64_t S, int64_t Q, const void *knn,
                           int KL, void *idx_out, int idx_is_i64, void *scratch, size_t scratch_bytes, cudaStream_t st)
{
    QueryScratch qs = carve_query(scratch, B, Q);
    if (!scratch || scratch_bytes < qs.bytes) {
        set_error("knn subset search: %zu bytes of scratch required, %zu given", qs.bytes, scratch_bytes);
        return FFB6D_ERR_WORKSPACE;
    }
    FFB6D_CUDA(cudaMemsetAsync(qs.state, 0, (size_t)B * sizeof(QueryState), st));
    dim3 grid((unsigned)ceil_div(Q, 256), (unsigned)B);
    const int64_t per_item = std::max<int64_t>(1, 4 * num_sms() / B);
    dim3 ogrid((unsigned)std::min<int64_t>(Q, per_item), (unsigned)B);
    if (idx_is_i64) {
        subset_nn_from_knn_kernel<long long><<<grid, 256, 0, st>>>((const long long *)knn, (int)Q, KL, (int)S,
                                                                   (long long *)idx_out, qs.state, qs.ovf);
        FFB6D_LAUNCH_OK("subset_nn_from_knn_kernel");
        grid_overflow_warp_kernel<long long><<<ogrid, 256, 0, st>>>(support, query, (int)S, (int)Q, 1, qs.state, qs.ovf,
                                                                    (long long *)idx_out);
    } else {
        subset_nn_from_knn_kernel<int><<<grid, 256, 0, st>>>((const int *)knn, (int)Q, KL, (int)S, (int *)idx_out, qs.state,
                                                             qs.ovf);
        FFB6D_LAUNCH_OK("subset_nn_from_knn_kernel");
        grid_overflow_warp_kernel<int><<<ogrid, 256, 0, st>>>(support, query, (int)S, (int)Q, 1, qs.state, qs.ovf,
                                                              (int *)idx_out);
    }
    FFB6D_LAUNCH_OK("grid_overflow_warp_kernel");
    return FFB6D_OK;
}

static bool g_force_thread_search = false;
static float g_cell_scale = 1.0f;
static float g_cell_scale_k1 = 2.5f;
static int g_quantile = 17;
static std::atomic<bool> g_env_read{false};

static void read_env()
{
    if (g_env_read.load(std::memory_order_acquire)) return;
    const Env &e = env();
    if (e.grid_scale > 0.f) g_cell_scale = e.grid_scale;
    if (e.grid_scale_k1 > 0.f) g_cell_scale_k1 = e.grid_scale_k1;
    g_force_thread_search = e.grid_thread_search;
    g_quantile = e.grid_quantile;
    g_env_read.store(true, std::memory_order_release);
}

void knn_grid_tune(float cell_scale, int quantile)
{
    read_env();
    if (cell_scale > 0.f) g_cell_scale = cell_scale;
    if (quantile >= 0) g_quantile = std::min(31, quantile);
}

void knn_grid_tune_k1(float cell_scale_k1)
{
    read_env();
    if (cell_scale_k1 > 0.f) g_cell_scale_k1 = cell_scale_k1;
}

template <int KCAP, typename IdxT>
static int launch_search(const float *support, const float *query, int64_t B, int64_t S, int64_t Q,
                         int K, void *idx_out, const GridStore &w, const QueryScratch &qs, int64_t query_width,
                         cudaStream_t st)
{
    const bool self = (support == query) && (S == Q);
    const bool warp = K >= 2 && K <= 32 && !g_force_thread_search;
    FFB6D_CUDA(cudaMemsetAsync(qs.state, 0, (size_t)B * sizeof(QueryState), st));
    const bool organised = K == 1 && !self && query_width >= 8 && Q % query_width == 0 && Q / query_width >= 4 &&
                           !g_force_thread_search;
    bool far_sentinels = false;
    if (organised) {
        const int64_t tiles_x = ceil_div(query_width, 8), tiles = tiles_x * ceil_div(Q / query_width, 4);
        far_sentinels = true;
        grid_search_k1_tile_kernel<IdxT, 1><<<dim3((unsigned)tiles, (unsigned)B), 32, 0, st>>>(
            query, (int)S, (int)Q, (int)query_width, (int)(Q / query_width), (int)tiles_x, (int)tiles,
            (int)(tiles + tiles_x >= 4000000), w.params, w.cursor, w.maxc, w.sorted, (IdxT *)idx_out, qs.state, qs.ovf);
    } else if (warp && K <= 16) {
        dim3 ggrid((unsigned)ceil_div(Q, 16), (unsigned)B);
        if (self)
            grid_search_group_kernel<IdxT, true, 16><<<ggrid, 256, 0, st>>>(
                query, (int)S, (int)Q, K, w.params, w.cursor, w.maxc, w.sorted, (IdxT *)idx_out, qs.state, qs.ovf);
        else
            grid_search_group_kernel<IdxT, false, 16><<<ggrid, 256, 0, st>>>(
                query, (int)S, (int)Q, K, w.params, w.cursor, w.maxc, w.sorted, (IdxT *)idx_out, qs.state, qs.ovf);
    } else if (warp) {
        dim3 wgrid((unsigned)ceil_div(Q, 8), (unsigned)B);
        if (self)
            grid_search_warp_kernel<IdxT, true><<<wgrid, 256, 0, st>>>(
                query, (int)S, (int)Q, K, w.params, w.cursor, w.maxc, w.sorted, (IdxT *)idx_out, qs.state, qs.ovf);
        else
            grid_search_warp_kernel<IdxT, false><<<wgrid, 256, 0, st>>>(
                query, (int)S, (int)Q, K, w.params, w.cursor, w.maxc, w.sorted, (IdxT *)idx_out, qs.state, qs.ovf);
    } else {
        dim3 grid((unsigned)ceil_div(Q, 128), (unsigned)B);
        if (self)
            grid_search_kernel<KCAP, IdxT, true><<<grid, 128, 0, st>>>(
                query, (int)S, (int)Q, K, w.params, w.cursor, w.maxc, w.sorted, (IdxT *)idx_out, qs.state, qs.ovf);
        else
            grid_search_kernel<KCAP, IdxT, false><<<grid, 128, 0, st>>>(
                query, (int)S, (int)Q, K, w.params, w.cursor, w.maxc, w.sorted, (IdxT *)idx_out, qs.state, qs.ovf);
    }
    FFB6D_LAUNCH_OK("grid_search_kernel");
    const int64_t per_item = std::max<int64_t>(1, 4 * num_sms() / B);
    if (K <= 32) {
        dim3 ogrid((unsigned)std::min<int64_t>(Q, per_item), (unsigned)B);
        grid_overflow_warp_kernel<IdxT><<<ogrid, 256, 0, st>>>(support, query, (int)S, (int)Q, K, qs.state,
                                                               qs.ovf, (IdxT *)idx_out);
        FFB6D_LAUNCH_OK("grid_overflow_warp_kernel");
        if (far_sentinels) {
            dim3 fgrid((unsigned)std::min<int64_t>(ceil_div(Q, 1024), 64), (unsigned)B);
            grid_far_fill_kernel<IdxT><<<fgrid, 256, 0, st>>>((int)Q, qs.state, (IdxT *)idx_out);
            FFB6D_LAUNCH_OK("grid_far_fill_kernel");
        }
    } else {
        constexpr int OT = (KCAP >= 32) ? 64 : 128;
        dim3 ogrid((unsigned)std::min<int64_t>(ceil_div(Q, OT), per_item), (unsigned)B);
        grid_overflow_kernel<KCAP, OT, 1024, IdxT><<<ogrid, OT, 0, st>>>(
            support, query, (int)S, (int)Q, K, qs.state, qs.ovf, (IdxT *)idx_out);
        FFB6D_LAUNCH_OK("grid_overflow_kernel");
        dim3 dgrid((unsigned)std::min<int64_t>(ceil_div(Q * K, 256), per_item), (unsigned)B);
        grid_dup_copy_kernel<IdxT><<<dgrid, 256, 0, st>>>((int)Q, K, qs.state, qs.ovf, (IdxT *)idx_out);
        FFB6D_LAUNCH_OK("grid_dup_copy_kernel");
    }
    return FFB6D_OK;
}

template <typename IdxT>
static int launch_search_k(const float *support, const float *query, int64_t B, int64_t S, int64_t Q,
                           int K, void *idx_out, const GridStore &w, const QueryScratch &qs, int64_t query_width,
                           cudaStream_t st)
{
    if (K == 1) return launch_search<1, IdxT>(support, query, B, S, Q, K, idx_out, w, qs, query_width, st);
    if (K <= 4) return launch_search<4, IdxT>(support, query, B, S, Q, K, idx_out, w, qs, query_width, st);
    if (K <= 8) return launch_search<8, IdxT>(support, query, B, S, Q, K, idx_out, w, qs, query_width, st);
    if (K <= 16) return launch_search<16, IdxT>(support, query, B, S, Q, K, idx_out, w, qs, query_width, st);
    if (K <= 32) return launch_search<32, IdxT>(support, query, B, S, Q, K, idx_out, w, qs, query_width, st);
    return launch_search<64, IdxT>(support, query, B, S, Q, K, idx_out, w, qs, query_width, st);
}

int knn_grid_build(const float *support, int64_t B, int64_t S, int K, void *grid_mem,
                   size_t grid_bytes, cudaStream_t st)
{
    read_env();
    GridStore w = carve_grid(grid_mem, B, S);
    if (!grid_mem || grid_bytes < w.bytes) {
        set_error("knn grid build: %zu bytes of grid storage required, %zu given", w.bytes, grid_bytes);
        return FFB6D_ERR_WORKSPACE;
    }
    grid_build_kernel<<<dim3(BUILD_CTAS, (unsigned)B), BUILD_THREADS, 0, st>>>(
        support, (int)S, K, (int)w.maxc, K == 1 ? g_cell_scale_k1 : g_cell_scale, g_quantile, w.params, w.cursor,
        w.rank, w.sorted);
    FFB6D_LAUNCH_OK("grid_build_kernel");
    return FFB6D_OK;
}

int knn_grid_query(const float *support, const float *query, int64_t B, int64_t S, int64_t Q, int K,
                   void *idx_out, int idx_is_i64, const void *grid_mem, size_t grid_bytes,
                   void *scratch, size_t scratch_bytes, cudaStream_t st, int64_t query_width)
{
    read_env();
    GridStore w = carve_grid(const_cast<void *>(grid_mem), B, S);
    QueryScratch qs = carve_query(scratch, B, Q);
    if (!grid_mem || grid_bytes < w.bytes || !scratch || scratch_bytes < qs.bytes) {
        set_error("knn grid query: storage too small (grid %zu/%zu, scratch %zu/%zu)", grid_bytes, w.bytes,
                  scratch_bytes, qs.bytes);
        return FFB6D_ERR_WORKSPACE;
    }
    if (idx_is_i64) return launch_search_k<long long>(support, query, B, S, Q, K, idx_out, w, qs, query_width, st);
    return launch_search_k<int>(support, query, B, S, Q, K, idx_out, w, qs, query_width, st);
}

int knn_grid_launch(const float *support, const float *query, int64_t B, int64_t S, int64_t Q, int K,
                    void *idx_out, int idx_is_i64, void *workspace, size_t workspace_bytes,
                    cudaStream_t st)
{
    const size_t gb = knn_grid_store_bytes(B, S), qb = knn_grid_query_bytes(B, Q);
    if (!workspace || workspace_bytes < gb + qb) {
        set_error("knn grid: workspace too small (%zu < %zu)", workspace_bytes, gb + qb);
        return FFB6D_ERR_WORKSPACE;
    }
    int rc = knn_grid_build(support, B, S, K, workspace, gb, st);
    if (rc) return rc;
    return knn_grid_query(support, query, B, S, Q, K, idx_out, idx_is_i64, workspace, gb,
                          (char *)workspace + gb, qb, st);
}

}
```

### ffb6d_b200/csrc/schedule.cu

```cuda
#include "common.cuh"
#include "knn_common.cuh"

#include <algorithm>

namespace ffb6d {

static const int kDsSr[4] = {4, 8, 8, 8};
static const int kUpSr[3] = {4, 2, 2};

struct Call {
    int sup_kind, sup_id;
    int qry_kind, qry_id;
    int K;
};

static void make_calls(int K, Call (&c)[22])
{
    int n = 0;
    for (int i = 0; i < 4; ++i) {
        c[n++] = {0, i, 0, i, K};
        c[n++] = {0, i + 1, 0, i, 1};
        c[n++] = {1, kDsSr[i], 0, i + 1, K};
        c[n++] = {0, i + 1, 1, kDsSr[i], 1};
    }
    for (int i = 0; i < 3; ++i) {
        const int lvl = 3 - i;
        c[n++] = {1, kUpSr[i], 0, lvl, K};
        c[n++] = {0, lvl, 1, kUpSr[i], 1};
    }
}

struct Sizes {
    int64_t cld[5];
    int64_t img[9];
};

static Sizes make_sizes(int64_t N0, int64_t H, int64_t W)
{
    Sizes s{};
    s.cld[0] = N0;
    for (int i = 1; i < 5; ++i) s.cld[i] = s.cld[i - 1] / 4;
    for (int sr : {2, 4, 8}) s.img[sr] = (H / sr) * (W / sr);
    return s;
}

static int64_t size_of(const Sizes &z, int kind, int id) { return kind == 0 ? z.cld[id] : z.img[id]; }

__global__ void __launch_bounds__(256)
strided_pixels_copy_kernel(const unsigned *__restrict__ in, unsigned *__restrict__ out, int Hc, int Wc, int Hp, int Wp, int f,
                           int words, long long total)
{
    const long long t = (long long)blockIdx.x * blockDim.x + threadIdx.x;
    if (t >= total) return;
    const int wd = (int)(t % words);
    long long px = t / words;
    const int c = (int)(px % Wc);
    px /= Wc;
    const int r = (int)(px % Hc);
    const long long b = px / Hc;
    out[t] = __ldg(in + (((b * Hp + (long long)r * f) * Wp + (long long)c * f) * words + wd));
}

struct Plan {
    size_t levels_off[5];
    size_t grid_off, scratch_off, total;
};

static Plan make_plan(int64_t B, const Sizes &z, int K)
{
    Plan p{};
    size_t off = 0;
    for (int i = 1; i < 5; ++i) {
        p.levels_off[i] = off;
        off = align_up(off + (size_t)B * (size_t)z.cld[i] * 3 * sizeof(float), 256);
    }
    Call calls[22];
    make_calls(K, calls);
    size_t grid = 0, scratch = 0;
    for (const Call &c : calls) {
        const int64_t S = size_of(z, c.sup_kind, c.sup_id), Q = size_of(z, c.qry_kind, c.qry_id);
        if (S > 0) grid = std::max(grid, knn_grid_store_bytes(B, S));
        if (Q > 0) scratch = std::max(scratch, knn_grid_query_bytes(B, Q));
    }
    p.grid_off = off;
    off = align_up(off + grid, 256);
    p.scratch_off = off;
    off = align_up(off + scratch, 256);
    p.total = off;
    return p;
}

}

using namespace ffb6d;

extern "C" size_t ffb6d_build_indices_workspace_bytes(int64_t B, int64_t N0, int64_t H, int64_t W, int K)
{
    if (B <= 0 || N0 < 256 || H < 8 || W < 8 || K < 1 || K > FFB6D_MAX_K) return 0;
    return make_plan(B, make_sizes(N0, H, W), K).total;
}

extern "C" int ffb6d_build_indices(const float *cld, const float *img2, const float *img4, const float *img8, int64_t B,
                                   int64_t N0, int64_t H, int64_t W, int K, void *const *out, int idx_is_i64,
                                   void *workspace, size_t workspace_bytes, ffb6d_stream_t stream)
{
    FFB6D_CHECK_ARG(B >= 0 && B < 65536, "build_indices: bad batch size");
    FFB6D_CHECK_ARG(N0 >= 256 && N0 % 256 == 0 && N0 < (1ll << 31), "build_indices: N0=%lld must be a positive multiple of 256",
                    (long long)N0);
    FFB6D_CHECK_ARG(H >= 8 && W >= 8 && H % 8 == 0 && W % 8 == 0, "build_indices: H, W must be multiples of 8");
    FFB6D_CHECK_ARG(K >= 1 && K <= FFB6D_MAX_K, "build_indices: K=%d outside [1,%d]", K, FFB6D_MAX_K);
    if (B == 0) return FFB6D_OK;
    FFB6D_CHECK_ARG(cld && img2 && img4 && img8 && out && workspace, "build_indices: null pointer");
    for (int i = 0; i < 22; ++i) FFB6D_CHECK_ARG(out[i], "build_indices: out[%d] is null", i);
    const Sizes z = make_sizes(N0, H, W);
    const Plan plan = make_plan(B, z, K);
    if (workspace_bytes < plan.total) {
        set_error("build_indices: workspace of %zu bytes required, %zu given", plan.total, workspace_bytes);
        return FFB6D_ERR_WORKSPACE;
    }
    cudaStream_t st = (cudaStream_t)stream;
    char *ws = (char *)workspace;
    const float *level[5] = {cld, nullptr, nullptr, nullptr, nullptr};
    for (int i = 1; i < 5; ++i) {
        float *dst = (float *)(ws + plan.levels_off[i]);
        FFB6D_CUDA(cudaMemcpy2DAsync(dst, (size_t)z.cld[i] * 12, cld, (size_t)N0 * 12, (size_t)z.cld[i] * 12, (size_t)B,
                                     cudaMemcpyDeviceToDevice, st));
        level[i] = dst;
    }
    auto set_ptr = [&](int kind, int id) -> const float * {
        if (kind == 0) return level[id];
        return id == 2 ? img2 : (id == 4 ? img4 : img8);
    };
    Call calls[22];
    make_calls(K, calls);
    bool done[22] = {};
    int parent[22];
    for (int i = 0; i < 22; ++i) {
        parent[i] = -1;
        if (calls[i].qry_kind != 0) continue;
        for (int j = 0; j < 22; ++j)
            if (j != i && calls[j].qry_kind == 0 && calls[j].sup_kind == calls[i].sup_kind && calls[j].sup_id == calls[i].sup_id &&
                calls[j].K == calls[i].K && calls[j].qry_id < calls[i].qry_id &&
                (parent[i] < 0 || calls[j].qry_id < calls[parent[i]].qry_id))
                parent[i] = j;
    }
    int stride_f[22];
    for (int i = 0; i < 22; ++i) {
        stride_f[i] = 0;
        if (calls[i].qry_kind != 1 || H % calls[i].qry_id != 0 || W % calls[i].qry_id != 0) continue;
        for (int j = 0; j < 22; ++j)
            if (j != i && calls[j].qry_kind == 1 && calls[j].sup_kind == calls[i].sup_kind && calls[j].sup_id == calls[i].sup_id &&
                calls[j].K == calls[i].K && calls[j].qry_id < calls[i].qry_id && calls[i].qry_id % calls[j].qry_id == 0 &&
                (parent[i] < 0 || calls[j].qry_id < calls[parent[i]].qry_id)) {
                parent[i] = j;
                stride_f[i] = calls[i].qry_id / calls[j].qry_id;
            }
    }
    void *grid = ws + plan.grid_off, *scratch = ws + plan.scratch_off;
    for (int i = 0; i < 22; ++i) {
        if (done[i]) continue;
        const Call &c = calls[i];
        const int64_t S = size_of(z, c.sup_kind, c.sup_id);
        const float *sup = set_ptr(c.sup_kind, c.sup_id);
        bool use_grid = false;
        for (int j = i; j < 22; ++j)
            if (calls[j].sup_kind == c.sup_kind && calls[j].sup_id == c.sup_id && calls[j].K == c.K)
                use_grid = use_grid || knn_grid_workspace_bytes(B, S, size_of(z, calls[j].qry_kind, calls[j].qry_id), c.K) > 0;
        if (use_grid) {
            const int rc = knn_grid_build(sup, B, S, c.K, grid, knn_grid_store_bytes(B, S), st);
            if (rc != FFB6D_OK) return rc;
        }
        for (int j = i; j < 22; ++j) {
            const Call &d = calls[j];
            if (done[j] || d.sup_kind != c.sup_kind || d.sup_id != c.sup_id || d.K != c.K) continue;
            if (parent[j] >= 0) continue;
            const int64_t Q = size_of(z, d.qry_kind, d.qry_id);
            const float *qry = set_ptr(d.qry_kind, d.qry_id);
            int rc;
            const bool from_self = env().subset_nn && d.K == 1 && K >= 8 && d.sup_kind == 0 && d.qry_kind == 0 && d.sup_id == d.qry_id + 1 &&
                                   j == 4 * d.qry_id + 1 && done[4 * d.qry_id] && knn_grid_workspace_bytes(B, S, Q, 1) > 0;
            if (from_self)
                rc = knn_subset_nn_from_knn(sup, qry, B, S, Q, out[4 * d.qry_id], K, out[j], idx_is_i64, scratch,
                                            knn_grid_query_bytes(B, Q), st);
            else if (use_grid)
                rc = knn_grid_query(sup, qry, B, S, Q, d.K, out[j], idx_is_i64, grid, knn_grid_store_bytes(B, S), scratch,
                                    knn_grid_query_bytes(B, Q), st, d.qry_kind == 1 ? W / d.qry_id : 0);
            else
                rc = knn_brute_launch(sup, qry, B, S, Q, d.K, out[j], idx_is_i64, st);
            if (rc != FFB6D_OK) return rc;
            done[j] = true;
        }
    }
    const size_t esz = idx_is_i64 ? 8 : 4;
    for (int i = 0; i < 22; ++i) {
        if (parent[i] < 0) continue;
        const int64_t Qc = size_of(z, calls[i].qry_kind, calls[i].qry_id), Qp = size_of(z, calls[parent[i]].qry_kind, calls[parent[i]].qry_id);
        const size_t row = (size_t)calls[i].K * esz;
        if (stride_f[i] > 0) {
            const int sc = calls[i].qry_id, sp = calls[parent[i]].qry_id, words = (int)(row / 4);
            const long long total = (long long)B * Qc * words;
            strided_pixels_copy_kernel<<<(unsigned)ceil_div(total, 256), 256, 0, st>>>(
                (const unsigned *)out[parent[i]], (unsigned *)out[i], (int)(H / sc), (int)(W / sc), (int)(H / sp), (int)(W / sp),
                stride_f[i], words, total);
            FFB6D_LAUNCH_OK("strided_pixels_copy_kernel");
            continue;
        }
        FFB6D_CUDA(cudaMemcpy2DAsync(out[i], (size_t)Qc * row, out[parent[i]], (size_t)Qp * row, (size_t)Qc * row, (size_t)B,
                                     cudaMemcpyDeviceToDevice, st));
    }
    return FFB6D_OK;
}
```

### ffb6d_b200/ops.py

```python
import ctypes as C

import numpy as np
import torch

from . import _lib
from ._lib import lib, check, LAYOUT_NCS, LAYOUT_NSC

import os as _os
_DEBUG_GRID = bool(_os.environ.get("FFB6D_DEBUG_GRID"))
_debug_ws = []
_I64 = (torch.int64,)
_IDX = (torch.int32, torch.int64)


def _stream(dev):
    return C.c_void_p(torch.cuda.current_stream(dev).cuda_stream)


def _need_cuda(t, name):
    if not isinstance(t, torch.Tensor):
        raise TypeError("%s must be a torch.Tensor, got %r" % (name, type(t)))
    if not t.is_cuda:
        raise RuntimeError("%s must be a CUDA tensor: ffb6d_b200 has no CPU path" % name)


def deterministic_backward(weight_grad=False):
    if torch.are_deterministic_algorithms_enabled():
        return True
    return bool(weight_grad) and bool(torch.backends.cudnn.deterministic)


def _idx_arg(idx, name):
    if idx.dtype not in _IDX:
        raise TypeError("%s must be int32 or int64, got %s" % (name, idx.dtype))
    return idx.contiguous(), int(idx.dtype == torch.int64)


def knn_search(support_pts, query_pts, k, out_dtype=None, algo=0):
    k = int(k)
    if isinstance(support_pts, np.ndarray) or isinstance(query_pts, np.ndarray):
        sup = np.ascontiguousarray(support_pts, dtype=np.float32)
        qry = np.ascontiguousarray(query_pts, dtype=np.float32)
        if sup.ndim != 3 or qry.ndim != 3 or sup.shape[0] != qry.shape[0]:
            raise ValueError("knn_search expects [B,N1,3] and [B,N2,3], got %s and %s"
                             % (sup.shape, qry.shape))
        B, S, dim = sup.shape
        Q = qry.shape[1]
        indices = np.zeros((B, Q, k), dtype=np.int64)
        check(lib.ffb6d_knn_batch_host(sup.ctypes.data, B, S, dim, qry.ctypes.data, Q, k,
                                       indices.ctypes.data))
        return indices.astype(np.int32)
    _need_cuda(support_pts, "support_pts")
    _need_cuda(query_pts, "query_pts")
    sup = support_pts.contiguous().float()
    qry = query_pts.contiguous().float()
    if sup.dim() != 3 or qry.dim() != 3 or sup.shape[0] != qry.shape[0] or sup.shape[2] != 3 \
            or qry.shape[2] != 3:
        raise ValueError("knn_search expects [B,N1,3] and [B,N2,3], got %s and %s"
                         % (tuple(sup.shape), tuple(qry.shape)))
    B, S, _ = sup.shape
    Q = qry.shape[1]
    dt = torch.int32 if out_dtype is None else out_dtype
    if dt not in _IDX:
        raise TypeError("out_dtype must be torch.int32 or torch.int64")
    out = torch.empty((B, Q, k), dtype=dt, device=sup.device)
    with torch.cuda.device(sup.device):
        ws_bytes = int(lib.ffb6d_knn_workspace_bytes(B, S, Q, k)) if algo != 1 else 0
        ws = torch.empty(ws_bytes, dtype=torch.uint8, device=sup.device) if ws_bytes else None
        check(lib.ffb6d_knn_batch_algo(sup.data_ptr(), qry.data_ptr(), B, S, Q, k, out.data_ptr(),
                                       int(dt == torch.int64), ws.data_ptr() if ws is not None else None,
                                       ws_bytes, int(algo), _stream(sup.device)))
    if _DEBUG_GRID:
        _debug_ws.append((B, S, Q, k, ws))
    return out


class KnnGrid:

    def __init__(self, support, k_hint):
        _need_cuda(support, "support")
        sup = support.contiguous().float()
        if sup.dim() != 3 or sup.shape[2] != 3 or sup.shape[1] < 1:
            raise ValueError("KnnGrid expects a non-empty [B,S,3] support, got %s" % (tuple(sup.shape),))
        self.support = sup
        self.B, self.S = sup.shape[0], sup.shape[1]
        self.k_hint = int(k_hint)
        with torch.cuda.device(sup.device):
            self.nbytes = int(lib.ffb6d_knn_grid_bytes(self.B, self.S))
            self.mem = torch.empty(self.nbytes, dtype=torch.uint8, device=sup.device)
            check(lib.ffb6d_knn_grid_build(sup.data_ptr(), self.B, self.S, self.k_hint,
                                           self.mem.data_ptr(), self.nbytes, _stream(sup.device)))

    def query(self, query_pts, k, out_dtype=None, query_width=0):
        _need_cuda(query_pts, "query_pts")
        qry = self.support if query_pts is self.support else query_pts.contiguous().float()
        if qry.dim() != 3 or qry.shape[0] != self.B or qry.shape[2] != 3:
            raise ValueError("query must be [B,Q,3] with B=%d, got %s" % (self.B, tuple(qry.shape)))
        k = int(k)
        Q = qry.shape[1]
        dt = torch.int32 if out_dtype is None else out_dtype
        if dt not in _IDX:
            raise TypeError("out_dtype must be torch.int32 or torch.int64")
        dev = self.support.device
        out = torch.empty((self.B, Q, k), dtype=dt, device=dev)
        with torch.cuda.device(dev):
            sb = int(lib.ffb6d_knn_grid_query_bytes(self.B, Q))
            scratch = torch.empty(max(sb, 1), dtype=torch.uint8, device=dev)
            qw = int(query_width) if query_width and Q % int(query_width) == 0 else 0
            check(lib.ffb6d_knn_grid_query_organized(self.support.data_ptr(), qry.data_ptr(), self.B, self.S, Q, k,
                                                     out.data_ptr(), int(dt == torch.int64), self.mem.data_ptr(),
                                                     self.nbytes, scratch.data_ptr(), sb, qw, _stream(dev)))
        return out


def knn_uses_grid(B, S, Q, k):
    return int(lib.ffb6d_knn_workspace_bytes(B, S, Q, int(k))) > 0


def subset_nn_from_knn(support, query_pts, knn_idx):
    _need_cuda(support, "support")
    _need_cuda(query_pts, "query_pts")
    _need_cuda(knn_idx, "knn_idx")
    sup, qry = support.contiguous().float(), query_pts.contiguous().float()
    if sup.dim() != 3 or qry.dim() != 3 or sup.shape[2] != 3 or qry.shape[2] != 3 or sup.shape[0] != qry.shape[0]:
        raise ValueError("expected support [B,S,3] and query [B,Q,3]")
    B, S, Q = sup.shape[0], sup.shape[1], qry.shape[1]
    if knn_idx.dim() != 3 or knn_idx.shape[0] != B or knn_idx.shape[1] != Q or knn_idx.dtype not in _IDX:
        raise ValueError("knn_idx must be an int32 / int64 [B,Q,K] tensor, got %s %s" % (tuple(knn_idx.shape), knn_idx.dtype))
    if S < 1 or S > Q:
        raise ValueError("the support (%d rows) must be a non-empty row prefix of the %d queries" % (S, Q))
    knn = knn_idx.contiguous()
    out = torch.empty((B, Q, 1), dtype=knn.dtype, device=sup.device)
    with torch.cuda.device(sup.device):
        sb = int(lib.ffb6d_knn_grid_query_bytes(B, Q))
        scratch = torch.empty(max(sb, 1), dtype=torch.uint8, device=sup.device)
        check(lib.ffb6d_knn_subset_nn(sup.data_ptr(), qry.data_ptr(), B, S, Q, knn.data_ptr(), int(knn.shape[2]),
                                      out.data_ptr(), int(knn.dtype == torch.int64), scratch.data_ptr(), sb, _stream(sup.device)))
    return out


def _layout_of(f3):
    B, Cc, S = f3.shape
    sb, sc, ss = f3.stride()
    if f3.is_contiguous():
        return f3, LAYOUT_NCS
    if S > 1 and Cc > 1 and sc == 1 and ss == Cc and (B == 1 or sb == Cc * S):
        return f3, LAYOUT_NSC
    return f3.contiguous(), LAYOUT_NCS


class _GatherMax(torch.autograd.Function):
    @staticmethod
    def forward(ctx, f3, idx):
        f3, layout = _layout_of(f3)
        idx_c, i64 = _idx_arg(idx, "index")
        B, Cc, S = f3.shape
        Q, K = idx_c.shape[1], idx_c.shape[2]
        if layout == LAYOUT_NCS:
            out = torch.empty((B, Cc, Q), dtype=torch.float32, device=f3.device)
        else:
            out = torch.empty((B, Q, Cc), dtype=torch.float32, device=f3.device).transpose(1, 2)
        with torch.cuda.device(f3.device):
            check(lib.ffb6d_gather_max_fwd(f3.data_ptr(), idx_c.data_ptr(), i64, B, Cc, S, Q, K,
                                           layout, out.data_ptr(), _stream(f3.device)))
        ctx.save_for_backward(f3, idx_c)
        ctx.layout = layout
        return out

    @staticmethod
    @torch.autograd.function.once_differentiable
    def backward(ctx, gout):
        f3, idx_c = ctx.saved_tensors
        return _gather_max_bwd(f3, idx_c, gout, ctx.layout), None


def _gather_max_bwd(f3, idx_c, gout, layout):
    B, Cc, S = f3.shape
    Q, K = idx_c.shape[1], idx_c.shape[2]
    if layout == LAYOUT_NCS:
        g = gout.contiguous()
        gf = torch.empty((B, Cc, S), dtype=torch.float32, device=f3.device)
    else:
        g = gout.transpose(1, 2).contiguous().transpose(1, 2)
        gf = torch.empty((B, S, Cc), dtype=torch.float32, device=f3.device).transpose(1, 2)
    if deterministic_backward():
        if K == 1 and layout == LAYOUT_NCS and _counter_plan_fits(Q, S):
            return segment_sum(g, None, S, plan=SegmentPlan(idx_c.reshape(B, Q), S))
        _gather_max_bwd_det(f3, idx_c, g, layout, gf)
        return gf
    with torch.cuda.device(f3.device):
        check(lib.ffb6d_gather_max_bwd(f3.data_ptr(), idx_c.data_ptr(),
                                       int(idx_c.dtype == torch.int64), g.data_ptr(), B, Cc, S,
                                       Q, K, layout, gf.data_ptr(), _stream(f3.device)))
    return gf


def _counter_plan_fits(P, NA):
    return NA * -(-P // 1024) <= P + NA


def _gather_max_bwd_det(f3, idx_c, g, layout, gf):
    B, Cc, S = f3.shape
    Q, K = idx_c.shape[1], idx_c.shape[2]
    dev = f3.device
    with torch.cuda.device(dev):
        nbytes = int(lib.ffb6d_gather_max_bwd_det_workspace_bytes(B, Cc, S, Q, K))
        ws = torch.empty(max(nbytes, 16), dtype=torch.uint8, device=dev)
        check(lib.ffb6d_gather_max_bwd_det(f3.data_ptr(), idx_c.data_ptr(), int(idx_c.dtype == torch.int64),
                                           g.data_ptr(), B, Cc, S, Q, K, layout, ws.data_ptr(), nbytes,
                                           gf.data_ptr(), _stream(dev)))


def _gather_max(feature, idx3):
    _need_cuda(feature, "feature")
    _need_cuda(idx3, "index")
    if feature.dtype != torch.float32:
        raise TypeError("feature must be float32 (the reference runs amp O0), got %s" % feature.dtype)
    if feature.dim() == 4:
        if feature.shape[3] != 1:
            raise ValueError("feature must be [B,C,N,1], got %s" % (tuple(feature.shape),))
        f3 = feature.squeeze(3)
    elif feature.dim() == 3:
        f3 = feature
    else:
        raise ValueError("feature must be [B,C,N] or [B,C,N,1], got %s" % (tuple(feature.shape),))
    if idx3.dim() != 3 or idx3.shape[0] != f3.shape[0]:
        raise ValueError("index must be [B,N',K] with the batch of feature, got %s"
                         % (tuple(idx3.shape),))
    if idx3.shape[2] < 1 or idx3.shape[2] > _lib.MAX_K:
        raise ValueError("neighbour count %d outside [1,%d]" % (idx3.shape[2], _lib.MAX_K))
    return _GatherMax.apply(f3, idx3)


def random_sample(feature, pool_idx):
    return _gather_max(feature, pool_idx).unsqueeze(3)


def nearest_interpolation(feature, interp_idx):
    if feature.dim() != 4:
        raise ValueError("feature must be [B,C,N,1], got %s" % (tuple(feature.shape),))
    B, up = interp_idx.shape[0], interp_idx.shape[1]
    return _gather_max(feature, interp_idx.reshape(B, up, 1)).unsqueeze(3)


def choose_gather(rgb_emb, choose):
    B, Cc = rgb_emb.shape[0], rgb_emb.shape[1]
    f3 = rgb_emb.reshape(B, Cc, -1) if rgb_emb.dim() == 4 and rgb_emb.is_contiguous() else \
        rgb_emb.flatten(2)
    return _gather_max(f3, choose.reshape(B, -1, 1))


def check_indices(idx, S):
    _need_cuda(idx, "idx")
    idx_c, i64 = _idx_arg(idx, "idx")
    with torch.cuda.device(idx_c.device):
        check(lib.ffb6d_check_indices(idx_c.data_ptr(), i64, idx_c.numel(), int(S), _stream(idx_c.device)))


class _GatherNeighbour(torch.autograd.Function):
    @staticmethod
    def forward(ctx, pc, idx):
        pc = pc.contiguous()
        idx_c, i64 = _idx_arg(idx, "neighbor_idx")
        B, S, D = pc.shape
        N, K = idx_c.shape[1], idx_c.shape[2]
        out = torch.empty((B, N, K, D), dtype=torch.float32, device=pc.device)
        with torch.cuda.device(pc.device):
            check(lib.ffb6d_gather_neighbour_fwd(pc.data_ptr(), idx_c.data_ptr(), i64, B, S, D, N, K,
                                                 out.data_ptr(), _stream(pc.device)))
        ctx.save_for_backward(idx_c)
        ctx.shape = (B, S, D)
        return out

    @staticmethod
    @torch.autograd.function.once_differentiable
    def backward(ctx, gout):
        (idx_c,) = ctx.saved_tensors
        B, S, D = ctx.shape
        N, K = idx_c.shape[1], idx_c.shape[2]
        g = gout.contiguous()
        gpc = torch.empty((B, S, D), dtype=torch.float32, device=g.device)
        if deterministic_backward():
            with torch.cuda.device(g.device):
                nbytes = int(lib.ffb6d_gather_neighbour_bwd_det_workspace_bytes(B, S, N, K))
                ws = torch.empty(max(nbytes, 16), dtype=torch.uint8, device=g.device)
                check(lib.ffb6d_gather_neighbour_bwd_det(g.data_ptr(), idx_c.data_ptr(), int(idx_c.dtype == torch.int64),
                                                         B, S, D, N, K, ws.data_ptr(), nbytes, gpc.data_ptr(),
                                                         _stream(g.device)))
            return gpc, None
        with torch.cuda.device(g.device):
            check(lib.ffb6d_gather_neighbour_bwd(g.data_ptr(), idx_c.data_ptr(),
                                                 int(idx_c.dtype == torch.int64), B, S, D, N, K,
                                                 gpc.data_ptr(), _stream(g.device)))
        return gpc, None


def gather_neighbour(pc, neighbor_idx):
    _need_cuda(pc, "pc")
    _need_cuda(neighbor_idx, "neighbor_idx")
    if pc.dtype != torch.float32:
        raise TypeError("pc must be float32, got %s" % pc.dtype)
    if pc.dim() != 3 or neighbor_idx.dim() != 3 or pc.shape[0] != neighbor_idx.shape[0]:
        raise ValueError("gather_neighbour expects pc [B,N,d] and idx [B,N,K], got %s, %s"
                         % (tuple(pc.shape), tuple(neighbor_idx.shape)))
    return _GatherNeighbour.apply(pc, neighbor_idx)


def relative_pos_encoding(xyz, neigh_idx, channel_major=False):
    _need_cuda(xyz, "xyz")
    _need_cuda(neigh_idx, "neigh_idx")
    xyz = xyz.contiguous().float()
    idx_c, i64 = _idx_arg(neigh_idx, "neigh_idx")
    if xyz.dim() != 3 or xyz.shape[2] != 3 or idx_c.dim() != 3 or idx_c.shape[:2] != xyz.shape[:2]:
        raise ValueError("relative_pos_encoding expects xyz [B,N,3] and idx [B,N,K]")
    B, N, _ = xyz.shape
    K = idx_c.shape[2]
    if channel_major:
        out = torch.empty((B, 10, N, K), dtype=torch.float32, device=xyz.device)
        with torch.cuda.device(xyz.device):
            check(lib.ffb6d_relative_pos_encoding_cm_fwd(xyz.data_ptr(), idx_c.data_ptr(), i64, B, N, K,
                                                         out.data_ptr(), _stream(xyz.device)))
        return out
    out = torch.empty((B, N, K, 10), dtype=torch.float32, device=xyz.device)
    with torch.cuda.device(xyz.device):
        check(lib.ffb6d_relative_pos_encoding_fwd(xyz.data_ptr(), idx_c.data_ptr(), i64, B, N, K,
                                                  out.data_ptr(), _stream(xyz.device)))
    return out


def fold_batchnorm(bn):
    var, mean = bn.running_var.float(), bn.running_mean.float()
    gamma = bn.weight.float() if bn.weight is not None else torch.ones_like(var)
    beta = bn.bias.float() if bn.bias is not None else torch.zeros_like(var)
    scale = gamma / torch.sqrt(var + bn.eps)
    return scale.contiguous(), (beta - mean * scale).contiguous()


class PackedWeight:

    def __init__(self, weight):
        _need_cuda(weight, "weight")
        w = weight.detach().reshape(weight.shape[0], -1).contiguous().float()
        self.Co, self.Ci = int(w.shape[0]), int(w.shape[1])
        self.device = w.device
        nbytes = lib.ffb6d_fusion_mlp_pack_bytes(self.Co, self.Ci)
        self.data = torch.empty(nbytes, dtype=torch.uint8, device=w.device)
        with torch.cuda.device(w.device):
            check(lib.ffb6d_fusion_mlp_pack(w.data_ptr(), self.Co, self.Ci, self.data.data_ptr(), nbytes,
                                            _stream(w.device)))


def fusion_mlp_pack(weight):
    return PackedWeight(weight)


def fusion_mlp(x1, x2, weight, scale, shift, relu=True, negative_slope=None, add=None, add_idx=None,
               out_channels_last=False):
    _need_cuda(x1, "x1")
    if x1.dtype != torch.float32:
        raise TypeError("x1 must be float32")
    B, C1 = x1.shape[0], x1.shape[1]
    tail = tuple(x1.shape[2:])
    x1c = x1.contiguous()
    P = x1c.numel() // max(B * C1, 1)
    C2 = 0
    x2c = None
    if x2 is not None:
        _need_cuda(x2, "x2")
        if x2.dtype != torch.float32 or x2.shape[0] != B or tuple(x2.shape[2:]) != tail:
            raise ValueError("x2 must be float32 with the batch and trailing shape of x1")
        x2c = x2.contiguous()
        C2 = x2.shape[1]
    packed = weight if isinstance(weight, PackedWeight) else PackedWeight(weight)
    Co, Ci = packed.Co, packed.Ci
    if packed.device != x1.device:
        raise ValueError("packed weight lives on %s, inputs on %s" % (packed.device, x1.device))
    if Ci != C1 + C2:
        raise ValueError("weight has %d input channels, inputs have %d" % (Ci, C1 + C2))
    sc, sh = scale.contiguous().float(), shift.contiguous().float()
    if sc.numel() != Co or sh.numel() != Co:
        raise ValueError("scale/shift must have %d elements" % Co)
    addc, idxc, i64, NA = None, None, 0, 0
    if add is not None:
        _need_cuda(add, "add")
        if add_idx is None:
            raise ValueError("add needs add_idx")
        _need_cuda(add_idx, "add_idx")
        if add.dtype != torch.float32 or add.dim() != 3 or add.shape[0] != B or add.shape[2] != Co:
            raise ValueError("add must be float32 [B, NA, Co], got %s" % (tuple(add.shape),))
        addc = add.contiguous()
        NA = addc.shape[1]
        idxc, i64 = _idx_arg(add_idx.reshape(B, -1), "add_idx")
        if idxc.shape[1] != P:
            raise ValueError("add_idx must hold one index per position (%d), got %d" % (P, idxc.shape[1]))
    if out_channels_last:
        out = torch.empty((B, P, Co), dtype=torch.float32, device=x1.device)
    else:
        out = torch.empty((B, Co) + tail, dtype=torch.float32, device=x1.device)
    with torch.cuda.device(x1.device):
        check(lib.ffb6d_fusion_mlp_fwd_ex(
            x1c.data_ptr(), C1, x2c.data_ptr() if x2c is not None else None, C2, packed.data.data_ptr(),
            sc.data_ptr(), sh.data_ptr(), B, Co, P, 2 if negative_slope is not None else int(bool(relu)),
            float(negative_slope or 0.0), addc.data_ptr() if addc is not None else None,
            idxc.data_ptr() if idxc is not None else None, i64, NA,
            LAYOUT_NSC if out_channels_last else LAYOUT_NCS, out.data_ptr(), _stream(x1.device)))
    return out


class SegmentPlan:
    _bytes, _build, _sum = "ffb6d_segment_plan_bytes", "ffb6d_segment_plan", "ffb6d_segment_sum"

    def __init__(self, idx, n_segments):
        if not isinstance(idx, torch.Tensor):
            raise TypeError("idx must be a torch.Tensor, got %r" % type(idx))
        if idx.dtype not in _IDX:
            raise TypeError("idx must be int32 or int64, got %s" % idx.dtype)
        if idx.dim() not in (2, 3) or (idx.dim() == 3 and idx.shape[2] != 1) or idx.numel() == 0:
            raise ValueError("idx must be a non-empty [B, P] or [B, P, 1], got %s" % (tuple(idx.shape),))
        if int(n_segments) < 1:
            raise ValueError("n_segments must be >= 1, got %d" % int(n_segments))
        _need_cuda(idx, "idx")
        idx_c, i64 = _idx_arg(idx.reshape(idx.shape[0], -1), "idx")
        self.B, self.P, self.NA = int(idx_c.shape[0]), int(idx_c.shape[1]), int(n_segments)
        self.device = idx_c.device
        self.nbytes = int(getattr(lib, self._bytes)(self.B, self.P, self.NA))
        if self.nbytes == 0:
            raise ValueError("no segment plan for B=%d, P=%d, n_segments=%d" % (self.B, self.P, self.NA))
        self.data = torch.empty(self.nbytes, dtype=torch.uint8, device=self.device)
        with torch.cuda.device(self.device):
            check(getattr(lib, self._build)(idx_c.data_ptr(), i64, self.B, self.P, self.NA, self.data.data_ptr(),
                                            self.nbytes, _stream(self.device)))

    def csr(self):
        words = self.data.view(torch.int32).view(self.B, -1)
        return words[:, :self.NA + 1], words[:, self.NA + 1:self.NA + 1 + self.P]


class SegmentCSR(SegmentPlan):
    _bytes, _build, _sum = "ffb6d_segment_csr_bytes", "ffb6d_segment_csr", "ffb6d_segment_sum_csr"


def segment_plan(idx, n_segments):
    return SegmentPlan(idx, n_segments)


def segment_csr(idx, n_segments):
    return SegmentCSR(idx, n_segments)


def segment_sum(grad, idx, n_segments, plan=None):
    if not isinstance(grad, torch.Tensor):
        raise TypeError("grad must be a torch.Tensor, got %r" % type(grad))
    if grad.dtype != torch.float32:
        raise TypeError("grad must be float32, got %s" % grad.dtype)
    if grad.dim() not in (3, 4) or grad.numel() == 0:
        raise ValueError("grad must be a non-empty [B, C, P] or [B, C, h, w], got %s" % (tuple(grad.shape),))
    _need_cuda(grad, "grad")
    B, Cc = int(grad.shape[0]), int(grad.shape[1])
    g = grad.contiguous().reshape(B, Cc, -1)
    if plan is None:
        plan = SegmentPlan(idx, n_segments)
    elif not isinstance(plan, SegmentPlan):
        raise TypeError("plan must be a SegmentPlan, got %r" % type(plan))
    if (plan.B, plan.P, plan.NA) != (B, g.shape[2], int(n_segments)):
        raise ValueError("plan is for B=%d, P=%d, n_segments=%d; grad has B=%d, P=%d and n_segments=%d"
                         % (plan.B, plan.P, plan.NA, B, g.shape[2], int(n_segments)))
    if plan.device != grad.device:
        raise ValueError("plan lives on %s, grad on %s" % (plan.device, grad.device))
    out = torch.empty((B, Cc, plan.NA), dtype=torch.float32, device=grad.device)
    with torch.cuda.device(grad.device):
        check(getattr(lib, plan._sum)(g.data_ptr(), plan.data.data_ptr(), plan.nbytes, B, Cc, plan.P, plan.NA,
                                      out.data_ptr(), _stream(grad.device)))
    return out


def att_pool(f1, f2, att):
    _need_cuda(f1, "f1")
    _need_cuda(att, "att")
    f1c = f1.contiguous()
    f2c = f2.contiguous() if f2 is not None else None
    B, C1, N, K = f1c.shape
    C2 = f2c.shape[1] if f2c is not None else 0
    a = att.contiguous()
    if tuple(a.shape) != (B, C1 + C2, N, K) or f1c.dtype != torch.float32 or a.dtype != torch.float32:
        raise ValueError("att must be float32 [B,C1+C2,N,K] matching f1/f2")
    out = torch.empty((B, C1 + C2, N, 1), dtype=torch.float32, device=f1.device)
    with torch.cuda.device(f1.device):
        check(lib.ffb6d_att_pool_fwd(f1c.data_ptr(), C1, f2c.data_ptr() if f2c is not None else None, C2,
                                     a.data_ptr(), B, N, K, out.data_ptr(), _stream(f1.device)))
    return out


def lfa_att_pool_fused(xyz, neigh_idx, feature, mlp1, mlp2, fc_weight, mlp_out, negative_slope=0.2):
    _need_cuda(xyz, "xyz")
    _need_cuda(feature, "feature")
    xyz = xyz.contiguous().float()
    idx_c, i64 = _idx_arg(neigh_idx, "neigh_idx")
    B, N, K = idx_c.shape
    f = feature.reshape(B, feature.shape[1], N).contiguous().float()
    Dh = f.shape[1]

    def prep(layer):
        w, sc, sh = layer
        return w.reshape(w.shape[0], -1).contiguous().float(), sc.contiguous().float(), sh.contiguous().float()

    w1, s1, t1 = prep(mlp1)
    w2, s2, t2 = prep(mlp2) if mlp2 is not None else (None, None, None)
    wo, so, to = prep(mlp_out)
    wfc = fc_weight.reshape(fc_weight.shape[0], -1).contiguous().float()
    Do = wo.shape[0]
    if w1.shape != (Dh, 10) or wfc.shape != (2 * Dh, 2 * Dh) or wo.shape[1] != 2 * Dh or (w2 is not None and w2.shape != (Dh, Dh)):
        raise ValueError("layer shapes do not match d/2 = %d" % Dh)
    out = torch.empty((B, Do, N, 1), dtype=torch.float32, device=f.device)
    with torch.cuda.device(f.device):
        check(lib.ffb6d_lfa_att_pool_fused(
            xyz.data_ptr(), idx_c.data_ptr(), i64, f.data_ptr(), w1.data_ptr(), s1.data_ptr(), t1.data_ptr(),
            w2.data_ptr() if w2 is not None else None, s2.data_ptr() if w2 is not None else None,
            t2.data_ptr() if w2 is not None else None, wfc.data_ptr(), wo.data_ptr(), so.data_ptr(), to.data_ptr(),
            B, N, K, Dh, Do, float(negative_slope), out.data_ptr(), _stream(f.device)))
    return out


def lfa_fusable(d_half, k):
    return int(k) == 16 and int(d_half) in (16, 32, 64)


def backproject(depth, K, choose):
    _need_cuda(depth, "depth")
    _need_cuda(choose, "choose")
    if depth.dim() != 3 or depth.dtype != torch.float32:
        raise ValueError("depth must be float32 [B,H,W], got %s %s" % (depth.dtype, tuple(depth.shape)))
    depth = depth.contiguous()
    B, H, W = depth.shape
    dev = depth.device
    if isinstance(K, torch.Tensor) and K.is_cuda:
        if K.dtype != torch.float64 or K.shape not in ((4,), (B, 4)):
            raise ValueError("device intrinsics must be float64 [4] or [B,4] = (fx, fy, cx, cy)")
        intr_d, per_frame = K.contiguous(), int(K.dim() == 2)
        return _backproject(depth, intr_d, per_frame, choose)
    Kn = np.asarray(K, dtype=np.float64)
    if Kn.shape == (3, 3):
        intr = np.array([Kn[0, 0], Kn[1, 1], Kn[0, 2], Kn[1, 2]], np.float64)
        per_frame = 0
    elif Kn.shape == (B, 3, 3):
        intr = np.stack([Kn[:, 0, 0], Kn[:, 1, 1], Kn[:, 0, 2], Kn[:, 1, 2]], 1).copy()
        per_frame = 1
    else:
        raise ValueError("K must be [3,3] or [B,3,3], got %s" % (Kn.shape,))
    return _backproject(depth, torch.from_numpy(intr).to(dev), per_frame, choose)


def sample_valid_pixels(depth, n_points, seed=0, min_depth=1e-8, return_count=False):
    _need_cuda(depth, "depth")
    if depth.dim() != 3 or depth.dtype != torch.float32:
        raise ValueError("depth must be float32 [B,H,W]")
    depth = depth.contiguous()
    B, H, W = depth.shape
    dev = depth.device
    choose = torch.empty((B, 1, int(n_points)), dtype=torch.int32, device=dev)
    count = torch.empty((B,), dtype=torch.int32, device=dev)
    with torch.cuda.device(dev):
        nbytes = int(lib.ffb6d_sample_pixels_workspace_bytes(B, H, W))
        ws = torch.empty(max(nbytes, 1), dtype=torch.uint8, device=dev)
        check(lib.ffb6d_sample_pixels(depth.data_ptr(), B, H, W, float(min_depth), int(n_points), int(seed) & (2 ** 64 - 1),
                                      choose.data_ptr(), count.data_ptr(), ws.data_ptr(), nbytes, _stream(dev)))
    return (choose, count) if return_count else choose


def fill_missing(dpt, cam_scale, scale_2_80m=1, fill_type='multiscale', extrapolate=False, show_process=False,
                 blur_type='bilateral'):
    return _fill_depth(dpt, cam_scale, scale_2_80m, fill_type, extrapolate, blur_type, want_m=False)[0]


def _fill_depth(dpt, cam_scale, scale_2_80m=1, fill_type='multiscale', extrapolate=False, blur_type='bilateral',
                want_raw=True, want_m=True):
    if fill_type != 'multiscale':
        raise ValueError("fill_type %r is not implemented: only 'multiscale' (the YCB dataset's)" % (fill_type,))
    if extrapolate is not False:
        raise ValueError("extrapolate=%r is not implemented: only False (the YCB dataset's)" % (extrapolate,))
    if blur_type != 'bilateral':
        raise ValueError("blur_type %r is not implemented: only 'bilateral' (the YCB dataset's)" % (blur_type,))
    if isinstance(scale_2_80m, bool) or scale_2_80m != 1:
        raise ValueError("scale_2_80m=%r is not implemented: only 1 (the YCB dataset's)" % (scale_2_80m,))
    cs = float(np.float32(cam_scale))
    if not (cs > 0.0 and np.isfinite(cs)):
        raise ValueError("cam_scale must be positive and finite, got %r" % (cam_scale,))
    if not isinstance(dpt, torch.Tensor):
        raise TypeError("dpt must be a torch.Tensor, got %r" % type(dpt))
    if dpt.dtype != torch.uint16 or dpt.dim() not in (2, 3) or dpt.numel() == 0:
        raise ValueError("dpt must be a non-empty torch.uint16 [B,H,W] or [H,W] tensor, got %s %s"
                         % (dpt.dtype, tuple(dpt.shape)))
    _need_cuda(dpt, "dpt")
    raw = dpt.contiguous()
    B, H, W = (1,) + tuple(raw.shape) if raw.dim() == 2 else tuple(raw.shape)
    dev = raw.device
    outs = [torch.empty(raw.shape, dtype=torch.float32, device=dev) if want else None for want in (want_raw, want_m)]
    with torch.cuda.device(dev):
        nbytes = int(lib.ffb6d_fill_depth_workspace_bytes(B, H, W))
        ws = torch.empty(max(nbytes, 1), dtype=torch.uint8, device=dev)
        check(lib.ffb6d_fill_depth(raw.data_ptr(), B, H, W, cs, *(o.data_ptr() if o is not None else None for o in outs),
                                   ws.data_ptr(), nbytes, _stream(dev)))
    return tuple(outs)


def intrinsics_to_device(K, device, batch=None):
    Kn = np.asarray(K, dtype=np.float64)
    if Kn.ndim == 2:
        v = np.array([Kn[0, 0], Kn[1, 1], Kn[0, 2], Kn[1, 2]], np.float64)
    else:
        v = np.stack([Kn[:, 0, 0], Kn[:, 1, 1], Kn[:, 0, 2], Kn[:, 1, 2]], 1).copy()
    return torch.from_numpy(v).to(device)


def _backproject(depth, intr_d, per_frame, choose):
    B, H, W = depth.shape
    dev = depth.device
    ch = choose.reshape(B, -1)
    if ch.dtype != torch.int32 or not ch.is_contiguous():
        ch = ch.to(torch.int32).contiguous()
    N = ch.shape[1]
    cld = torch.empty((B, N, 3), dtype=torch.float32, device=dev)
    pyr = {s: torch.empty((B, (H // s) * (W // s), 3), dtype=torch.float32, device=dev) for s in (2, 4, 8)}
    with torch.cuda.device(dev):
        check(lib.ffb6d_backproject(depth.data_ptr(), B, H, W, intr_d.data_ptr(), per_frame, ch.data_ptr(), N,
                                    cld.data_ptr(), pyr[2].data_ptr(), pyr[4].data_ptr(), pyr[8].data_ptr(),
                                    _stream(dev)))
    return cld, pyr


def grid_sub_sampling(points, features=None, labels=None, grid_size=0.1, verbose=0):
    pts = np.ascontiguousarray(points, dtype=np.float32)
    if pts.ndim != 2 or pts.shape[1] != 3:
        raise RuntimeError("Wrong dimensions : points.shape is not (N, 3)")
    N = pts.shape[0]
    if N < 1:
        raise RuntimeError("Error")
    feats = None
    fdim = 0
    if features is not None:
        feats = np.ascontiguousarray(features, dtype=np.float32)
        if feats.ndim != 2 or feats.shape[0] != N:
            raise RuntimeError("Wrong dimensions : features.shape is not (N, d)")
        fdim = feats.shape[1]
    cls = None
    ldim = 0
    if labels is not None:
        cls = np.ascontiguousarray(labels, dtype=np.int32)
        if cls.ndim > 2 or cls.shape[0] != N:
            raise RuntimeError("Wrong dimensions : classes.shape is not (N,) or (N, d)")
        ldim = 1 if cls.ndim == 1 else cls.shape[1]
    sub_p = np.empty((N, 3), np.float32)
    sub_f = np.empty((N, max(fdim, 1)), np.float32)
    sub_c = np.empty((N, max(ldim, 1)), np.int32)
    M = C.c_size_t(0)
    check(lib.ffb6d_grid_subsample_host(
        pts.ctypes.data, N, feats.ctypes.data if feats is not None else None, fdim,
        cls.ctypes.data if cls is not None else None, ldim, float(grid_size),
        sub_p.ctypes.data, sub_f.ctypes.data, sub_c.ctypes.data, C.byref(M)))
    m = M.value
    out = [sub_p[:m].copy()]
    if feats is not None:
        out.append(sub_f[:m, :fdim].copy())
    if cls is not None:
        out.append(sub_c[:m, :ldim].copy())
    return out[0] if len(out) == 1 else tuple(out)


def mean_shift_fit(votes, valid=None, bandwidth=0.05, max_iter=300, return_modes=False):
    _need_cuda(votes, "votes")
    if votes.dim() != 3 or votes.shape[2] != 3 or votes.dtype != torch.float32:
        raise ValueError("votes must be float32 [G,N,3]")
    votes = votes.contiguous()
    G, N, _ = votes.shape
    dev = votes.device
    stride = 0
    vptr = None
    if valid is not None:
        _need_cuda(valid, "valid")
        if valid.dtype == torch.bool:
            valid = valid.to(torch.uint8)
        if valid.dtype != torch.uint8:
            raise ValueError("valid must be bool or uint8")
        valid = valid.contiguous()
        if tuple(valid.shape) == (N,):
            stride = 0
        elif tuple(valid.shape) == (G, N):
            stride = N
        else:
            raise ValueError("valid must be [N] or [G,N]")
        vptr = valid.data_ptr()
    centres = torch.empty((G, 3), dtype=torch.float32, device=dev)
    labels = torch.empty((G, N), dtype=torch.uint8, device=dev)
    iters = torch.empty((G,), dtype=torch.int32, device=dev)
    modes = torch.empty((G, N, 3), dtype=torch.float32, device=dev) if return_modes else None
    with torch.cuda.device(dev):
        nbytes = int(lib.ffb6d_mean_shift_workspace_bytes(G, N))
        ws = torch.empty(max(nbytes, 1), dtype=torch.uint8, device=dev)
        check(lib.ffb6d_mean_shift_fit(votes.data_ptr(), vptr, stride, G, N, float(bandwidth), int(max_iter),
                                       centres.data_ptr(), labels.data_ptr(), iters.data_ptr(),
                                       modes.data_ptr() if modes is not None else None, ws.data_ptr(), nbytes, _stream(dev)))
    out = (centres, labels.bool(), iters)
    return out + (modes,) if return_modes else out


def best_fit_transform(A, B):
    _need_cuda(A, "A")
    _need_cuda(B, "B")
    single = A.dim() == 2
    if single:
        A, B = A[None], B[None]
    if A.shape != B.shape or A.dim() != 3 or A.shape[2] != 3:
        raise ValueError("A and B must both be [G,M,3]")
    A = A.to(torch.float32).contiguous()
    B = B.to(torch.float32).contiguous()
    G, M, _ = A.shape
    T = torch.empty((G, 3, 4), dtype=torch.float64, device=A.device)
    with torch.cuda.device(A.device):
        check(lib.ffb6d_best_fit_transform(A.data_ptr(), B.data_ptr(), G, M, T.data_ptr(), _stream(A.device)))
    return T[0] if single else T
```

### ffb6d_b200/schedule.py

```python
import contextlib
import os

import torch

from .ops import knn_search, KnnGrid, knn_uses_grid, subset_nn_from_knn

from .tables import (RGB_DS_SR, RGB_UP_SR, PCLD_SUB_S_R, N_DS_LAYERS, N_UP_LAYERS, K_NEIGH,
                     DS_RGB_OC, DS_RNDLA_OC, UP_RGB_OC, UP_RNDLA_OC, knn_schedule, set_size, gather_schedule,
                     fusion_mlp_schedule, knn_alg_bytes, gather_alg_bytes, frame_alg_bytes, derived_searches, derived_image_searches,
                     derived_subset_searches)


def image_pyramid(dpt_xyz, levels=(1, 2, 4, 8)):
    B, H, W, _ = dpt_xyz.shape
    pyr = {}
    for sr in levels:
        nh, nw = H // sr, W // sr
        pyr[sr] = dpt_xyz[:, :nh * sr:sr, :nw * sr:sr, :].reshape(B, nh * nw, 3).contiguous()
    return pyr


def build_ffb6d_indices(cld, dpt_xyz=None, k=K_NEIGH, index_dtype=torch.int32, timer=None, streams=None,
                        pyramid=None, image_hw=None, events=None, priority=None, build_streams=None):
    if cld.dim() != 3 or cld.shape[2] != 3:
        raise ValueError("expected cld [B,N,3]")
    cld = cld.contiguous().float()
    B, n0, _ = cld.shape
    used = sorted(set(RGB_DS_SR) | set(RGB_UP_SR))
    if pyramid is not None:
        if image_hw is None:
            raise ValueError("image_hw=(H, W) is required with pyramid=")
        H, W = image_hw
        sets = {("img", sr): pyramid[sr] for sr in used}
    else:
        if dpt_xyz is None or dpt_xyz.dim() != 4 or cld.shape[0] != dpt_xyz.shape[0]:
            raise ValueError("expected dpt_xyz [B,H,W,3] (or pyramid=)")
        H, W = dpt_xyz.shape[1], dpt_xyz.shape[2]
        sets = {("img", sr): p for sr, p in image_pyramid(dpt_xyz.float(), used).items()}
    n = n0
    for i in range(N_DS_LAYERS + 1):
        sets[("cld", i)] = cld if i == 0 else cld[:, :n, :].contiguous()
        if i < N_DS_LAYERS:
            n //= PCLD_SUB_S_R[i]
    inputs = {}
    calls = knn_schedule(n0, H, W, k)
    groups = {}
    for key, s, q, kk in calls:
        groups.setdefault((s, kk), []).append((key, q))
    derived_sub = {c: p_ for c, p_ in derived_subset_searches(calls).items()
                   if k >= 8 and os.environ.get("FFB6D_SUBSET_NN", "0") == "1"}
    derived_sub = {c: p_ for c, p_ in derived_sub.items()
                   if any(key == c and knn_uses_grid(B, sets[s].shape[1], sets[q].shape[1], kk) for key, s, q, kk in calls)}
    gridded = [g for g, members in groups.items()
               if any(knn_uses_grid(B, sets[g[0]].shape[1], sets[q].shape[1], g[1]) for key_, q in members
                      if key_ not in derived_sub)]
    grids = {}
    main = torch.cuda.current_stream(cld.device)
    par = streams is not None and timer is None
    bstreams = list(build_streams) if (build_streams and par) else []

    def fork():
        if par:
            for st in streams + bstreams:
                st.wait_stream(main)

    def join():
        if par:
            for st in streams + bstreams:
                main.wait_stream(st)

    def on(i, pool=None):
        pool = pool or streams
        return torch.cuda.stream(pool[i % len(pool)]) if par else contextlib.nullcontext()

    derived = derived_searches(calls)
    children = {}
    for child, parent in derived.items():
        children.setdefault(parent, []).append(child)
    derived_img = derived_image_searches(calls, H, W)
    children_img = {}
    for child, (parent, f) in derived_img.items():
        children_img.setdefault(parent, []).append((child, f))

    fork()
    built = {}
    if par and priority:
        order = sorted(calls, key=lambda c: -priority.get(c[0], 0.0))
        first_use = {}
        for pos, (key, s_, q_, kk_) in enumerate(order):
            first_use.setdefault((s_, kk_), pos)
        build_order = sorted(gridded, key=lambda g: first_use.get(g, len(order)))
    else:
        order = sorted(calls, key=lambda c: -(sets[c[2]].shape[1] * c[3])) if par else calls
        build_order = sorted(gridded, key=lambda g: -sets[g[0]].shape[1])
    for i, g in enumerate(build_order):
        with on(i, bstreams or None):
            if timer is not None:
                timer.start("knn_build:%s%d:k%d" % (g[0][0], g[0][1], g[1]), 0)
            grids[g] = KnnGrid(sets[g[0]], g[1])
            if timer is not None:
                timer.stop()
            if par:
                built[g] = torch.cuda.Event()
                built[g].record()
    order = [c for c in order if c[0] not in derived and c[0] not in derived_img and c[0] not in derived_sub]
    qsize = {key: sets[q].shape[1] for key, s, q, kk in calls}
    for i, (key, s, q, kk) in enumerate(order):
        sup, qry = sets[s], sets[q]
        with on(i):
            if timer is not None:
                timer.start("knn:" + key, knn_alg_bytes(sup.shape[1], qry.shape[1], kk) * B)
            if (s, kk) in grids:
                if par:
                    torch.cuda.current_stream(cld.device).wait_event(built[(s, kk)])
                inputs[key] = grids[(s, kk)].query(qry, kk, out_dtype=index_dtype,
                                                   query_width=(W // q[1]) if q[0] == "img" else 0)
            else:
                inputs[key] = knn_search(sup, qry, kk, out_dtype=index_dtype, algo=1)
            if timer is not None:
                timer.stop()
            done = [key]
            if key.startswith("cld_nei_idx"):
                lvl = int(key[len("cld_nei_idx"):])
                n_sub = sets[("cld", lvl + 1)].shape[1]
                inputs["cld_sub_idx%d" % lvl] = inputs[key][:, :n_sub, :].contiguous()
                done.append("cld_sub_idx%d" % lvl)
                child = "cld_interp_idx%d" % lvl
                if derived_sub.get(child) == key:
                    sub = sets[("cld", lvl + 1)]
                    if timer is not None:
                        timer.start("knn:" + child, knn_alg_bytes(sub.shape[1], qry.shape[1], 1) * B)
                    inputs[child] = subset_nn_from_knn(sub, qry, inputs[key])
                    if timer is not None:
                        timer.stop()
                    done.append(child)
            for child in children.get(key, ()):
                inputs[child] = inputs[key][:, :qsize[child], :].contiguous()
                done.append(child)
            for child, f in children_img.get(key, ()):
                hp, wp = H // q[1], W // q[1]
                inputs[child] = inputs[key].view(B, hp, wp, kk)[:, ::f, ::f, :].reshape(B, -1, kk)
                done.append(child)
            if par and events is not None:
                ev = torch.cuda.Event()
                ev.record()
                for name in done:
                    events[name] = ev
    if par and events is not None:
        events["_keepalive"] = (grids, sets)
    else:
        join()
    for i in range(N_DS_LAYERS):
        inputs["cld_xyz%d" % i] = sets[("cld", i)]
    return inputs


def build_ffb6d_indices_native(cld, pyramid, image_hw, k=K_NEIGH, index_dtype=torch.int32):
    import ctypes
    from ._lib import lib, check
    from .ops import _stream
    if cld.dim() != 3 or cld.shape[2] != 3 or not cld.is_cuda:
        raise ValueError("expected cld [B,N,3] on a CUDA device")
    cld = cld.contiguous().float()
    B, n0, _ = cld.shape
    H, W = image_hw
    img = {sr: pyramid[sr].contiguous().float() for sr in (2, 4, 8)}
    for sr in (2, 4, 8):
        if tuple(img[sr].shape) != (B, (H // sr) * (W // sr), 3):
            raise ValueError("pyramid[%d] must be [B, %d, 3]" % (sr, (H // sr) * (W // sr)))
    calls = knn_schedule(n0, H, W, k)
    inputs, ptrs = {}, (ctypes.c_void_p * len(calls))()
    for j, (key, s, q, kk) in enumerate(calls):
        inputs[key] = torch.empty((B, set_size(q, n0, H, W), kk), dtype=index_dtype, device=cld.device)
        ptrs[j] = inputs[key].data_ptr()
    nbytes = int(lib.ffb6d_build_indices_workspace_bytes(B, n0, H, W, int(k)))
    ws = torch.empty(max(nbytes, 1), dtype=torch.uint8, device=cld.device)
    with torch.cuda.device(cld.device):
        check(lib.ffb6d_build_indices(cld.data_ptr(), img[2].data_ptr(), img[4].data_ptr(), img[8].data_ptr(), B, n0, H, W,
                                      int(k), ctypes.cast(ptrs, ctypes.c_void_p), int(index_dtype == torch.int64),
                                      ws.data_ptr(), nbytes, _stream(cld.device)))
    n = n0
    for i in range(N_DS_LAYERS):
        inputs["cld_xyz%d" % i] = cld if i == 0 else cld[:, :n, :].contiguous()
        n //= PCLD_SUB_S_R[i]
        inputs["cld_sub_idx%d" % i] = inputs["cld_nei_idx%d" % i][:, :n, :].contiguous()
    return inputs


def build_ffb6d_indices_from_depth(depth, K, choose, k=K_NEIGH, index_dtype=torch.int32, streams=None):
    from .ops import backproject
    cld, pyr = backproject(depth, K, choose)
    return build_ffb6d_indices(cld, None, k=k, index_dtype=index_dtype, streams=streams, pyramid=pyr,
                               image_hw=(depth.shape[1], depth.shape[2]))


MSK_DP_THRESHOLD = 1e-6


def build_ffb6d_indices_from_raw_depth(dpt_raw, cam_scale, K, n_points, seed=0, k=K_NEIGH, index_dtype=torch.int32,
                                       streams=None):
    from .ops import _fill_depth, sample_valid_pixels
    if not isinstance(dpt_raw, torch.Tensor) or dpt_raw.dim() != 3:
        raise ValueError("dpt_raw must be a [B,H,W] torch.uint16 CUDA tensor")
    filled, depth_m = _fill_depth(dpt_raw, cam_scale)
    choose = sample_valid_pixels(filled, n_points, seed=seed, min_depth=MSK_DP_THRESHOLD)
    inputs = build_ffb6d_indices_from_depth(depth_m, K, choose, k=k, index_dtype=index_dtype, streams=streams)
    inputs["choose"] = choose
    inputs["dpt_map_m"] = depth_m
    return inputs
```

### include/ffb6d_b200.h

```cpp
#ifndef FFB6D_B200_H_
#define FFB6D_B200_H_

#include <stddef.h>
#include <stdint.h>

#ifdef __cplusplus
extern "C" {
#endif

#define FFB6D_OK              0
#define FFB6D_ERR_INVALID    -1
#define FFB6D_ERR_CUDA       -2
#define FFB6D_ERR_WORKSPACE  -3
#define FFB6D_ERR_NO_DEVICE  -4

#define FFB6D_LAYOUT_NCS 0
#define FFB6D_LAYOUT_NSC 1

#define FFB6D_MAX_K 64

typedef void *ffb6d_stream_t;

int ffb6d_version(void);
const char *ffb6d_last_error(void);
int ffb6d_device_count(void);
uint64_t ffb6d_launch_count(void);

size_t ffb6d_knn_workspace_bytes(int64_t B, int64_t S, int64_t Q, int K);
int ffb6d_knn_batch(const float *support, const float *query,
                    int64_t B, int64_t S, int64_t Q, int K,
                    void *idx_out, int idx_is_i64,
                    void *workspace, size_t workspace_bytes,
                    ffb6d_stream_t stream);

int ffb6d_knn_batch_algo(const float *support, const float *query,
                         int64_t B, int64_t S, int64_t Q, int K,
                         void *idx_out, int idx_is_i64,
                         void *workspace, size_t workspace_bytes,
                         int algo, ffb6d_stream_t stream);

size_t ffb6d_knn_grid_bytes(int64_t B, int64_t S);
size_t ffb6d_knn_grid_query_bytes(int64_t B, int64_t Q);
int ffb6d_knn_grid_build(const float *support, int64_t B, int64_t S, int K_hint,
                         void *grid, size_t grid_bytes, ffb6d_stream_t stream);
int ffb6d_knn_grid_query(const float *support, const float *query,
                         int64_t B, int64_t S, int64_t Q, int K,
                         void *idx_out, int idx_is_i64,
                         const void *grid, size_t grid_bytes,
                         void *scratch, size_t scratch_bytes, ffb6d_stream_t stream);
int ffb6d_knn_grid_query_organized(const float *support, const float *query,
                                   int64_t B, int64_t S, int64_t Q, int K,
                                   void *idx_out, int idx_is_i64,
                                   const void *grid, size_t grid_bytes,
                                   void *scratch, size_t scratch_bytes,
                                   int64_t query_width, ffb6d_stream_t stream);

int ffb6d_knn_subset_nn(const float *support, const float *query, int64_t B, int64_t S, int64_t Q,
                        const void *knn_idx, int K_list, void *idx_out, int idx_is_i64,
                        void *scratch, size_t scratch_bytes, ffb6d_stream_t stream);

size_t ffb6d_build_indices_workspace_bytes(int64_t B, int64_t N0, int64_t H, int64_t W, int K);
int ffb6d_build_indices(const float *cld, const float *img2, const float *img4, const float *img8,
                        int64_t B, int64_t N0, int64_t H, int64_t W, int K,
                        void *const *out, int idx_is_i64, void *workspace, size_t workspace_bytes,
                        ffb6d_stream_t stream);

void ffb6d_knn_grid_tune(float cell_scale, int quantile);
void ffb6d_knn_grid_tune_k1(float cell_scale_k1);

int ffb6d_knn_batch_host(const float *batch_data, size_t batch_size, size_t npts, size_t dim,
                         const float *queries, size_t nqueries, size_t K, long *batch_indices);
int ffb6d_knn_host(const float *points, size_t npts, size_t dim,
                   const float *queries, size_t nqueries, size_t K, long *indices);

int ffb6d_gather_max_fwd(const float *feat, const void *idx, int idx_is_i64,
                         int64_t B, int64_t C, int64_t S, int64_t Q, int K,
                         int layout, float *out, ffb6d_stream_t stream);
int ffb6d_check_indices(const void *idx, int idx_is_i64, int64_t count, int64_t S, ffb6d_stream_t stream);
const char *ffb6d_gather_kernel_name(int64_t B, int64_t C, int64_t S, int64_t Q, int K, int layout);
int ffb6d_gather_max_bwd(const float *feat, const void *idx, int idx_is_i64,
                         const float *grad_out,
                         int64_t B, int64_t C, int64_t S, int64_t Q, int K,
                         int layout, float *grad_feat, ffb6d_stream_t stream);

int ffb6d_gather_neighbour_fwd(const float *pc, const void *idx, int idx_is_i64,
                               int64_t B, int64_t S, int64_t D, int64_t N, int K,
                               float *out, ffb6d_stream_t stream);
int ffb6d_gather_neighbour_bwd(const float *grad_out, const void *idx, int idx_is_i64,
                               int64_t B, int64_t S, int64_t D, int64_t N, int K,
                               float *grad_pc, ffb6d_stream_t stream);

int ffb6d_relative_pos_encoding_fwd(const float *xyz, const void *idx, int idx_is_i64,
                                    int64_t B, int64_t N, int K,
                                    float *out, ffb6d_stream_t stream);
int ffb6d_relative_pos_encoding_cm_fwd(const float *xyz, const void *idx, int idx_is_i64,
                                       int64_t B, int64_t N, int K,
                                       float *out, ffb6d_stream_t stream);

int ffb6d_fusion_mlp_fwd(const float *x1, int64_t C1, const float *x2, int64_t C2,
                         const float *weight, const float *scale, const float *shift,
                         int64_t B, int64_t Co, int64_t P, int act, float negative_slope,
                         float *out, ffb6d_stream_t stream);

size_t ffb6d_fusion_mlp_pack_bytes(int64_t Co, int64_t Ci);
int ffb6d_fusion_mlp_pack(const float *weight, int64_t Co, int64_t Ci, void *packed, size_t packed_bytes,
                          ffb6d_stream_t stream);
int ffb6d_fusion_mlp_fwd_packed(const float *x1, int64_t C1, const float *x2, int64_t C2,
                                const void *packed, const float *scale, const float *shift,
                                int64_t B, int64_t Co, int64_t P, int act, float negative_slope,
                                float *out, ffb6d_stream_t stream);

int ffb6d_fusion_mlp_fwd_ex(const float *x1, int64_t C1, const float *x2, int64_t C2,
                            const void *packed, const float *scale, const float *shift,
                            int64_t B, int64_t Co, int64_t P, int act, float negative_slope,
                            const float *addend, const void *add_idx, int add_idx_is_i64, int64_t NA,
                            int out_layout, float *out, ffb6d_stream_t stream);

size_t ffb6d_bn_workspace_bytes(int64_t C, int64_t P);
int ffb6d_bn_train_fwd(const float *z, int64_t B, int64_t C, int64_t P, const float *gamma, const float *beta,
                       float eps, float momentum, float *running_mean, float *running_var,
                       int act, float negative_slope, float *stats, float *y,
                       void *workspace, size_t workspace_bytes, ffb6d_stream_t stream);
int ffb6d_bn_train_bwd(const float *z, const float *grad_y, const float *stats, int64_t B, int64_t C, int64_t P,
                       int act, float negative_slope, float *grad_gamma, float *grad_beta, float *grad_z,
                       void *workspace, size_t workspace_bytes, ffb6d_stream_t stream);
int ffb6d_bn_sync_moments(const float *z, int64_t B, int64_t C, int64_t P, double *moments,
                          void *workspace, size_t workspace_bytes, ffb6d_stream_t stream);
int ffb6d_bn_sync_fwd(const float *z, int64_t B, int64_t C, int64_t P, const double *gathered, int64_t W,
                      const float *gamma, const float *beta, float eps, float momentum, float *running_mean,
                      float *running_var, int act, float negative_slope, float *stats, double *count, float *y,
                      ffb6d_stream_t stream);
int ffb6d_bn_sync_bwd_sums(const float *z, const float *grad_y, const float *stats, int64_t B, int64_t C, int64_t P,
                           int act, float negative_slope, double *sums, float *grad_gamma, float *grad_beta,
                           void *workspace, size_t workspace_bytes, ffb6d_stream_t stream);
int ffb6d_bn_sync_bwd(const float *z, const float *grad_y, const float *stats, int64_t B, int64_t C, int64_t P,
                      const double *gathered, int64_t W, const double *count, int act, float negative_slope,
                      float *grad_z, void *workspace, size_t workspace_bytes, ffb6d_stream_t stream);
int ffb6d_act_bwd(const float *z, const float *grad_y, int64_t n, int act, float negative_slope, float *grad_z,
                  ffb6d_stream_t stream);
int ffb6d_fusion_mlp_wgrad(const float *grad_z, const float *x1, int64_t C1, const float *x2, int64_t C2,
                           int64_t B, int64_t Co, int64_t P, float *grad_w, ffb6d_stream_t stream);

size_t ffb6d_segment_plan_bytes(int64_t B, int64_t P, int64_t NA);
int ffb6d_segment_plan(const void *idx, int idx_is_i64, int64_t B, int64_t P, int64_t NA, void *plan,
                       size_t plan_bytes, ffb6d_stream_t stream);
int ffb6d_segment_sum(const float *grad, const void *plan, size_t plan_bytes, int64_t B, int64_t C, int64_t P,
                      int64_t NA, float *out, ffb6d_stream_t stream);

size_t ffb6d_segment_csr_bytes(int64_t B, int64_t P, int64_t NA);
int ffb6d_segment_csr(const void *idx, int idx_is_i64, int64_t B, int64_t P, int64_t NA, void *plan,
                      size_t plan_bytes, ffb6d_stream_t stream);
int ffb6d_segment_sum_csr(const float *grad, const void *plan, size_t plan_bytes, int64_t B, int64_t C, int64_t P,
                          int64_t NA, float *out, ffb6d_stream_t stream);
size_t ffb6d_gather_max_bwd_det_workspace_bytes(int64_t B, int64_t C, int64_t S, int64_t Q, int K);
int ffb6d_gather_max_bwd_det(const float *feat, const void *idx, int idx_is_i64, const float *grad_out,
                             int64_t B, int64_t C, int64_t S, int64_t Q, int K, int layout, void *workspace,
                             size_t workspace_bytes, float *grad_feat, ffb6d_stream_t stream);
size_t ffb6d_gather_neighbour_bwd_det_workspace_bytes(int64_t B, int64_t S, int64_t N, int K);
int ffb6d_gather_neighbour_bwd_det(const float *grad_out, const void *idx, int idx_is_i64, int64_t B, int64_t S,
                                   int64_t D, int64_t N, int K, void *workspace, size_t workspace_bytes,
                                   float *grad_pc, ffb6d_stream_t stream);
size_t ffb6d_fusion_mlp_wgrad_det_workspace_bytes(int64_t C1, int64_t C2, int64_t B, int64_t Co, int64_t P);
int ffb6d_fusion_mlp_wgrad_det(const float *grad_z, const float *x1, int64_t C1, const float *x2, int64_t C2,
                               int64_t B, int64_t Co, int64_t P, void *workspace, size_t workspace_bytes,
                               float *grad_w, ffb6d_stream_t stream);

int ffb6d_att_pool_fwd(const float *f1, int64_t C1, const float *f2, int64_t C2, const float *att,
                       int64_t B, int64_t N, int K, float *out, ffb6d_stream_t stream);
int ffb6d_att_pool_bwd(const float *f1, int64_t C1, const float *f2, int64_t C2, const float *att,
                       const float *grad_out, int64_t B, int64_t N, int K,
                       float *grad_f1, float *grad_f2, float *grad_att, ffb6d_stream_t stream);

int ffb6d_lfa_att_pool_fused(const float *xyz, const void *idx, int idx_is_i64, const float *feature,
                             const float *w_x1, const float *scale_x1, const float *shift_x1,
                             const float *w_x2, const float *scale_x2, const float *shift_x2,
                             const float *w_fc, const float *w_out, const float *scale_out, const float *shift_out,
                             int64_t B, int64_t N, int K, int64_t Dh, int64_t Do, float negative_slope,
                             float *out, ffb6d_stream_t stream);

int ffb6d_backproject(const float *depth, int64_t B, int64_t H, int64_t W,
                      const double *intrinsics, int intrinsics_per_frame,
                      const int *choose, int64_t N,
                      float *cld, float *pyr2, float *pyr4, float *pyr8, ffb6d_stream_t stream);

size_t ffb6d_sample_pixels_workspace_bytes(int64_t B, int64_t H, int64_t W);
int ffb6d_sample_pixels(const float *depth, int64_t B, int64_t H, int64_t W, float min_depth, int64_t N,
                        uint64_t seed, int *choose, int *valid_count, void *workspace, size_t workspace_bytes,
                        ffb6d_stream_t stream);

size_t ffb6d_fill_depth_workspace_bytes(int64_t B, int64_t H, int64_t W);
int ffb6d_fill_depth(const uint16_t *depth_raw, int64_t B, int64_t H, int64_t W, float cam_scale,
                     float *filled_raw, float *depth_m, void *workspace, size_t workspace_bytes,
                     ffb6d_stream_t stream);

size_t ffb6d_mean_shift_workspace_bytes(int64_t G, int64_t N);
int ffb6d_mean_shift_fit(const float *votes, const unsigned char *valid, int64_t valid_stride, int64_t G, int64_t N,
                         float bandwidth, int max_iter, float *centres, unsigned char *labels, int *iters,
                         float *modes, void *workspace, size_t workspace_bytes, ffb6d_stream_t stream);

int ffb6d_best_fit_transform(const float *A, const float *B, int64_t G, int64_t M, double *T, ffb6d_stream_t stream);

int ffb6d_grid_subsample_host(const float *points, size_t N,
                              const float *features, size_t fdim,
                              const int *classes, size_t ldim,
                              float sampleDl,
                              float *sub_points, float *sub_features, int *sub_classes,
                              size_t *M_out);

#ifdef __cplusplus
}
#endif
#endif
```

Before: 84.44 million.

## Add narrower multi-slot group KNN search and spatially ordered query traversal

Generalizes the warp-group grid KNN search kernel so each lane holds multiple top-K slots, which allows 8-lane groups (4 queries per warp) when the batch is large. It also lets a query set that already has its own grid supply its cell-sorted points, so queries are processed in spatial order, and wires this into build_indices and the Python scheduler. The goal is more queries per warp and more coherent memory access, at the cost of extra shuffles, register pressure and an additional query-grid build.

```diff
diff --git a/ffb6d_b200/_lib.py b/ffb6d_b200/_lib.py
--- a/ffb6d_b200/_lib.py
+++ b/ffb6d_b200/_lib.py
@@ -41,11 +41,13 @@
         "ffb6d_knn_grid_build": (ci, [vp, i64, i64, ci, vp, sz, vp]),
         "ffb6d_knn_grid_query": (ci, [vp, vp, i64, i64, i64, ci, vp, ci, vp, sz, vp, sz, vp]),
         "ffb6d_knn_grid_query_organized": (ci, [vp, vp, i64, i64, i64, ci, vp, ci, vp, sz, vp, sz, i64, vp]),
+        "ffb6d_knn_grid_query_ordered": (ci, [vp, vp, i64, i64, i64, ci, vp, ci, vp, sz, vp, sz, vp, sz, vp]),
         "ffb6d_knn_subset_nn": (ci, [vp, vp, i64, i64, i64, vp, ci, vp, ci, vp, sz, vp]),
         "ffb6d_build_indices_workspace_bytes": (sz, [i64, i64, i64, i64, ci]),
         "ffb6d_build_indices": (ci, [vp, vp, vp, vp, i64, i64, i64, i64, ci, vp, ci, vp, sz, vp]),
         "ffb6d_knn_grid_tune": (None, [fp, ci]),
         "ffb6d_knn_grid_tune_k1": (None, [fp]),
+        "ffb6d_knn_grid_tune_group": (None, [ci]),
         "ffb6d_knn_batch_host": (ci, [vp, sz, sz, sz, vp, sz, sz, vp]),
         "ffb6d_knn_host": (ci, [vp, sz, sz, vp, sz, sz, vp]),
         "ffb6d_gather_max_fwd": (ci, [vp, vp, ci, i64, i64, i64, i64, ci, ci, vp, vp]),
diff --git a/ffb6d_b200/csrc/api.cu b/ffb6d_b200/csrc/api.cu
--- a/ffb6d_b200/csrc/api.cu
+++ b/ffb6d_b200/csrc/api.cu
@@ -66,6 +66,8 @@
         v.grid_quantile = (x = getenv("FFB6D_GRID_QUANTILE")) ? atoi(x) : 17;
         if (v.grid_quantile < 0) v.grid_quantile = 0;
         if (v.grid_quantile > 31) v.grid_quantile = 31;
+        v.grid_group_w = (x = getenv("FFB6D_GRID_GROUP_W")) ? atoi(x) : 0;
+        if (v.grid_group_w != 8 && v.grid_group_w != 16) v.grid_group_w = 0;
         return v;
     }();
     return e;
@@ -226,6 +228,21 @@
                           scratch_bytes, (cudaStream_t)stream, query_width);
 }
 
+int ffb6d_knn_grid_query_ordered(const float *support, const float *query, int64_t B, int64_t S, int64_t Q, int K,
+                                 void *idx_out, int idx_is_i64, const void *grid, size_t grid_bytes, void *scratch,
+                                 size_t scratch_bytes, const void *query_grid, size_t query_grid_bytes, ffb6d_stream_t stream)
+{
+    FFB6D_CHECK_ARG(B >= 0 && S >= 1 && Q >= 0 && B < 65536 && S < (1ll << 31) && Q < (1ll << 31),
+                    "knn_grid_query: bad size");
+    FFB6D_CHECK_ARG(K >= 1 && K <= FFB6D_MAX_K, "knn_grid_query: K=%d outside [1,%d]", K, FFB6D_MAX_K);
+    if (B == 0 || Q == 0) return FFB6D_OK;
+    FFB6D_CHECK_ARG(support && query && idx_out && grid && scratch && query_grid, "knn_grid_query: null pointer");
+    FFB6D_CHECK_ARG(query_grid_bytes >= knn_grid_store_bytes(B, Q), "knn_grid_query: query grid of %zu bytes, %zu required",
+                    query_grid_bytes, knn_grid_store_bytes(B, Q));
+    return knn_grid_query(support, query, B, S, Q, K, idx_out, idx_is_i64, grid, grid_bytes, scratch, scratch_bytes,
+                          (cudaStream_t)stream, 0, query_grid, query_grid_bytes);
+}
+
 int ffb6d_knn_subset_nn(const float *support, const float *query, int64_t B, int64_t S, int64_t Q, const void *knn_idx,
                         int K_list, void *idx_out, int idx_is_i64, void *scratch, size_t scratch_bytes,
                         ffb6d_stream_t stream)
@@ -243,6 +260,7 @@
 
 void ffb6d_knn_grid_tune(float cell_scale, int quantile) { knn_grid_tune(cell_scale, quantile); }
 void ffb6d_knn_grid_tune_k1(float cell_scale_k1) { knn_grid_tune_k1(cell_scale_k1); }
+void ffb6d_knn_grid_tune_group(int width) { knn_grid_tune_group(width); }
 
 int ffb6d_knn_batch_host(const float *batch_data, size_t batch_size, size_t npts, size_t dim,
                          const float *queries, size_t nqueries, size_t K, long *batch_indices)
diff --git a/ffb6d_b200/csrc/common.cuh b/ffb6d_b200/csrc/common.cuh
--- a/ffb6d_b200/csrc/common.cuh
+++ b/ffb6d_b200/csrc/common.cuh
@@ -76,6 +76,7 @@
     bool subset_nn;
     float grid_scale, grid_scale_k1;
     int grid_quantile;
+    int grid_group_w;
 };
 const Env &env();
 
diff --git a/ffb6d_b200/csrc/knn_common.cuh b/ffb6d_b200/csrc/knn_common.cuh
--- a/ffb6d_b200/csrc/knn_common.cuh
+++ b/ffb6d_b200/csrc/knn_common.cuh
@@ -75,13 +75,15 @@
                     cudaStream_t st);
 void knn_grid_tune(float cell_scale, int quantile);
 void knn_grid_tune_k1(float cell_scale_k1);
+void knn_grid_tune_group(int width);
 size_t knn_grid_store_bytes(int64_t B, int64_t S);
 size_t knn_grid_query_bytes(int64_t B, int64_t Q);
 int knn_grid_build(const float *support, int64_t B, int64_t S, int K, void *grid_mem,
                    size_t grid_bytes, cudaStream_t st);
 int knn_grid_query(const float *support, const float *query, int64_t B, int64_t S, int64_t Q, int K,
                    void *idx_out, int idx_is_i64, const void *grid_mem, size_t grid_bytes,
-                   void *scratch, size_t scratch_bytes, cudaStream_t st, int64_t query_width = 0);
+                   void *scratch, size_t scratch_bytes, cudaStream_t st, int64_t query_width = 0,
+                   const void *query_grid = nullptr, size_t query_grid_bytes = 0);
 
 int knn_subset_nn_from_knn(const float *support, const float *query, int64_t B, int64_t S, int64_t Q, const void *knn,
                            int KL, void *idx_out, int idx_is_i64, void *scratch, size_t scratch_bytes, cudaStream_t st);
diff --git a/ffb6d_b200/csrc/knn_grid.cu b/ffb6d_b200/csrc/knn_grid.cu
--- a/ffb6d_b200/csrc/knn_grid.cu
+++ b/ffb6d_b200/csrc/knn_grid.cu
@@ -974,15 +974,27 @@
     if ((o < k) == keep_min) k = o;
 }
 
-template <int W>
-__device__ __forceinline__ void group_sort(key_t64 &k, int sub)
-{
-#pragma unroll
-    for (int kk = 2; kk <= W; kk <<= 1) {
+__device__ __forceinline__ void slot_minmax(key_t64 &a, key_t64 &b, bool up)
+{
+    const key_t64 lo = a < b ? a : b, hi = a < b ? b : a;
+    a = up ? lo : hi;
+    b = up ? hi : lo;
+}
+
+template <int W, int SLOTS>
+__device__ __forceinline__ void group_sort(key_t64 (&k)[SLOTS], int sub)
+{
+#pragma unroll
+    for (int kk = 2; kk <= W * SLOTS; kk <<= 1) {
 #pragma unroll
         for (int j = kk >> 1; j > 0; j >>= 1) {
-            const bool up = (sub & kk) == 0;
-            group_minmax<W>(k, j, ((sub & j) == 0) == up);
+            const bool up = ((sub * SLOTS) & kk) == 0;
+            if (j >= SLOTS) {
+#pragma unroll
+                for (int s = 0; s < SLOTS; ++s) group_minmax<W>(k[s], j / SLOTS, ((sub & (j / SLOTS)) == 0) == up);
+            } else {
+                slot_minmax(k[0], k[SLOTS - 1], up);
+            }
         }
     }
 }
@@ -992,9 +1004,13 @@
 grid_search_group_kernel(const float *__restrict__ query, int S, int Q, int K,
                          const GridParams *__restrict__ params_all, const int *__restrict__ cursor_all,
                          size_t cursor_stride, const float4 *__restrict__ sorted_all,
-                         IdxT *__restrict__ idx_out, QueryState *state_all, int *__restrict__ ovf_all)
+                         const float4 *__restrict__ qorder_all, IdxT *__restrict__ idx_out,
+                         QueryState *state_all, int *__restrict__ ovf_all)
 {
     constexpr int G = 32 / W;
+    constexpr int SLOTS = 16 / W;
+    constexpr int NB = W * SLOTS;
+    static_assert(W * SLOTS == 16 && (SLOTS == 1 || SLOTS == 2), "group widths 8 and 16");
     const unsigned FULL = 0xffffffffu;
     const int b = blockIdx.y;
     const int lane = threadIdx.x & 31, sub = lane & (W - 1), grp = lane / W;
@@ -1007,8 +1023,8 @@
     const float4 *sorted = sorted_all + (size_t)b * S;
     float qx, qy, qz;
     int q;
-    if (SELF) {
-        const float4 me = __ldg(sorted + tq);
+    if (SELF || qorder_all) {
+        const float4 me = __ldg((SELF ? sorted : qorder_all + (size_t)b * Q) + tq);
         qx = me.x;
         qy = me.y;
         qz = me.z;
@@ -1039,7 +1055,13 @@
         return m;
     };
 
-    key_t64 mine = KEY_EMPTY;
+    key_t64 mine[SLOTS];
+#pragma unroll
+    for (int s = 0; s < SLOTS; ++s) mine[s] = KEY_EMPTY;
+    const int k_lane = (K - 1) / SLOTS, k_slot = (K - 1) % SLOTS;
+    auto kth_key = [&]() {
+        return __shfl_sync(FULL, (SLOTS > 1 && k_slot) ? mine[SLOTS - 1] : mine[0], k_lane, W);
+    };
     bool done = false;
     int r = (out > (float)RMAX * h) ? RMAX + 1 : 1;
     bool active = valid && r <= RMAX;
@@ -1051,7 +1073,7 @@
         const int e_end = (2 * r + 1) * (2 * r + 1);
         const int nseg = active ? 2 * e_prev + (e_end - e_prev) : 0;
         for (int s0 = 0; __any_sync(FULL, s0 < nseg); s0 += W) {
-            const float kth_now = key_dist(__shfl_sync(FULL, mine, K - 1, W));
+            const float kth_now = key_dist(kth_key());
             const int sidx = s0 + sub;
             int beg = 0, end = 0;
             if (sidx < nseg) {
@@ -1081,44 +1103,71 @@
             }
             const int total = __shfl_sync(FULL, incl, W - 1, W);
             const int excl = incl - cnt;
-            for (int j0 = 0; __any_sync(FULL, j0 < total); j0 += W) {
-                const int j = j0 + sub;
-                int seg = 0;
-#pragma unroll
-                for (int step = W / 2; step > 0; step >>= 1) {
-                    const int v = __shfl_sync(FULL, incl, seg + step - 1, W);
-                    if (v <= j) seg += step;
-                }
-                const int sb = __shfl_sync(FULL, beg, seg, W);
-                const int se = __shfl_sync(FULL, excl, seg, W);
-                key_t64 cand = KEY_INVALID;
-                if (j < total) {
-                    const float4 c = __ldg(sorted + sb + (j - se));
-                    cand = make_key(ref_sqdist(qx, qy, qz, c.x, c.y, c.z), __float_as_int(c.w));
-                }
-                const key_t64 thr = __shfl_sync(FULL, mine, K - 1, W);
-                const unsigned ball = __ballot_sync(FULL, cand < thr);
-                unsigned mask = (W == 32) ? ball : ((ball >> (W * grp)) & ((1u << W) - 1u));
-                if (__any_sync(FULL, __popc(mask) > (3 * W) / 8)) {
-                    group_sort<W>(cand, sub);
-                    const key_t64 rev = __shfl_sync(FULL, cand, W - 1 - sub, W);
-                    if (rev < mine) mine = rev;
-#pragma unroll
-                    for (int jj = W / 2; jj > 0; jj >>= 1) group_minmax<W>(mine, jj, (sub & jj) == 0);
-                    if (mine > KEY_EMPTY) mine = KEY_EMPTY;
+            for (int j0 = 0; __any_sync(FULL, j0 < total); j0 += NB) {
+                key_t64 cand[SLOTS];
+#pragma unroll
+                for (int s = 0; s < SLOTS; ++s) {
+                    const int j = j0 + s * W + sub;
+                    int seg = 0;
+#pragma unroll
+                    for (int step = W / 2; step > 0; step >>= 1) {
+                        const int v = __shfl_sync(FULL, incl, seg + step - 1, W);
+                        if (v <= j) seg += step;
+                    }
+                    const int sb = __shfl_sync(FULL, beg, seg, W);
+                    const int se = __shfl_sync(FULL, excl, seg, W);
+                    cand[s] = KEY_INVALID;
+                    if (j < total) {
+                        const float4 c = __ldg(sorted + sb + (j - se));
+                        cand[s] = make_key(ref_sqdist(qx, qy, qz, c.x, c.y, c.z), __float_as_int(c.w));
+                    }
+                }
+                const key_t64 thr = kth_key();
+                unsigned mask = 0;
+#pragma unroll
+                for (int s = 0; s < SLOTS; ++s) {
+                    const unsigned ball = __ballot_sync(FULL, cand[s] < thr);
+                    mask |= ((ball >> (W * grp)) & ((1u << W) - 1u)) << (s * W);
+                }
+                if (__any_sync(FULL, __popc(mask) > (3 * NB) / 8)) {
+                    group_sort<W, SLOTS>(cand, sub);
+                    key_t64 rev[SLOTS];
+#pragma unroll
+                    for (int s = 0; s < SLOTS; ++s) rev[s] = __shfl_sync(FULL, cand[SLOTS - 1 - s], W - 1 - sub, W);
+#pragma unroll
+                    for (int s = 0; s < SLOTS; ++s)
+                        if (rev[s] < mine[s]) mine[s] = rev[s];
+#pragma unroll
+                    for (int jj = NB / 2; jj > 0; jj >>= 1) {
+                        if (jj >= SLOTS) {
+#pragma unroll
+                            for (int s = 0; s < SLOTS; ++s) group_minmax<W>(mine[s], jj / SLOTS, (sub & (jj / SLOTS)) == 0);
+                        } else {
+                            slot_minmax(mine[0], mine[SLOTS - 1], true);
+                        }
+                    }
+#pragma unroll
+                    for (int s = 0; s < SLOTS; ++s)
+                        if (mine[s] > KEY_EMPTY) mine[s] = KEY_EMPTY;
                 } else {
                     while (__any_sync(FULL, mask != 0)) {
                         const int src = mask ? __ffs(mask) - 1 : 0;
-                        key_t64 x = __shfl_sync(FULL, cand, src, W);
+                        const key_t64 mine_src = (SLOTS > 1 && src >= W) ? cand[SLOTS - 1] : cand[0];
+                        key_t64 x = __shfl_sync(FULL, mine_src, src & (W - 1), W);
                         if (!mask) x = KEY_INVALID;
                         mask &= mask - 1;
-                        const key_t64 pred = __shfl_up_sync(FULL, mine, 1, W);
-                        if (x < mine) mine = (sub > 0 && x < pred) ? pred : x;
+                        const key_t64 pred0 = __shfl_up_sync(FULL, mine[SLOTS - 1], 1, W);
+#pragma unroll
+                        for (int s = SLOTS - 1; s >= 0; --s) {
+                            const key_t64 pred = s > 0 ? mine[s > 0 ? s - 1 : 0] : pred0;
+                            const bool has_pred = s > 0 || sub > 0;
+                            if (x < mine[s]) mine[s] = (has_pred && x < pred) ? pred : x;
+                        }
                     }
                 }
             }
         }
-        const float kth = key_dist(__shfl_sync(FULL, mine, K - 1, W));
+        const float kth = key_dist(kth_key());
         if (active) {
             e_prev = e_end;
             px0 = x0;
@@ -1146,7 +1195,10 @@
     }
     if (!valid) return;
     if (done) {
-        if (sub < K) idx_out[((size_t)b * Q + q) * K + sub] = (IdxT)(unsigned)(mine & 0xffffffffu);
+#pragma unroll
+        for (int s = 0; s < SLOTS; ++s)
+            if (sub * SLOTS + s < K)
+                idx_out[((size_t)b * Q + q) * K + sub * SLOTS + s] = (IdxT)(unsigned)(mine[s] & 0xffffffffu);
         return;
     }
     if (sub == 0) {
@@ -1339,6 +1391,7 @@
 static float g_cell_scale = 1.0f;
 static float g_cell_scale_k1 = 2.5f;
 static int g_quantile = 17;
+static int g_group_w = 0;
 static std::atomic<bool> g_env_read{false};
 
 static void read_env()
@@ -1349,6 +1402,7 @@
     if (e.grid_scale_k1 > 0.f) g_cell_scale_k1 = e.grid_scale_k1;
     g_force_thread_search = e.grid_thread_search;
     g_quantile = e.grid_quantile;
+    g_group_w = e.grid_group_w;
     g_env_read.store(true, std::memory_order_release);
 }
 
@@ -1365,10 +1419,29 @@
     if (cell_scale_k1 > 0.f) g_cell_scale_k1 = cell_scale_k1;
 }
 
+void knn_grid_tune_group(int width)
+{
+    read_env();
+    if (width == 0 || width == 8 || width == 16) g_group_w = width;
+}
+
+template <typename IdxT, int W>
+static void launch_group(bool self, const float *query, int64_t B, int64_t S, int64_t Q, int K, void *idx_out,
+                         const GridStore &w, const float4 *qorder, const QueryScratch &qs, cudaStream_t st)
+{
+    dim3 ggrid((unsigned)ceil_div(Q, 8 * (32 / W)), (unsigned)B);
+    if (self)
+        grid_search_group_kernel<IdxT, true, W><<<ggrid, 256, 0, st>>>(
+            query, (int)S, (int)Q, K, w.params, w.cursor, w.maxc, w.sorted, nullptr, (IdxT *)idx_out, qs.state, qs.ovf);
+    else
+        grid_search_group_kernel<IdxT, false, W><<<ggrid, 256, 0, st>>>(
+            query, (int)S, (int)Q, K, w.params, w.cursor, w.maxc, w.sorted, qorder, (IdxT *)idx_out, qs.state, qs.ovf);
+}
+
 template <int KCAP, typename IdxT>
 static int launch_search(const float *support, const float *query, int64_t B, int64_t S, int64_t Q,
                          int K, void *idx_out, const GridStore &w, const QueryScratch &qs, int64_t query_width,
-                         cudaStream_t st)
+                         const float4 *qorder, cudaStream_t st)
 {
     const bool self = (support == query) && (S == Q);
     const bool warp = K >= 2 && K <= 32 && !g_force_thread_search;
@@ -1383,13 +1456,11 @@
             query, (int)S, (int)Q, (int)query_width, (int)(Q / query_width), (int)tiles_x, (int)tiles,
             (int)(tiles + tiles_x >= 4000000), w.params, w.cursor, w.maxc, w.sorted, (IdxT *)idx_out, qs.state, qs.ovf);
     } else if (warp && K <= 16) {
-        dim3 ggrid((unsigned)ceil_div(Q, 16), (unsigned)B);
-        if (self)
-            grid_search_group_kernel<IdxT, true, 16><<<ggrid, 256, 0, st>>>(
-                query, (int)S, (int)Q, K, w.params, w.cursor, w.maxc, w.sorted, (IdxT *)idx_out, qs.state, qs.ovf);
+        const int gw = g_group_w ? g_group_w : (B * Q >= 65536 ? 8 : 16);
+        if (gw == 16)
+            launch_group<IdxT, 16>(self, query, B, S, Q, K, idx_out, w, qorder, qs, st);
         else
-            grid_search_group_kernel<IdxT, false, 16><<<ggrid, 256, 0, st>>>(
-                query, (int)S, (int)Q, K, w.params, w.cursor, w.maxc, w.sorted, (IdxT *)idx_out, qs.state, qs.ovf);
+            launch_group<IdxT, 8>(self, query, B, S, Q, K, idx_out, w, qorder, qs, st);
     } else if (warp) {
         dim3 wgrid((unsigned)ceil_div(Q, 8), (unsigned)B);
         if (self)
@@ -1435,14 +1506,14 @@
 template <typename IdxT>
 static int launch_search_k(const float *support, const float *query, int64_t B, int64_t S, int64_t Q,
                            int K, void *idx_out, const GridStore &w, const QueryScratch &qs, int64_t query_width,
-                           cudaStream_t st)
-{
-    if (K == 1) return launch_search<1, IdxT>(support, query, B, S, Q, K, idx_out, w, qs, query_width, st);
-    if (K <= 4) return launch_search<4, IdxT>(support, query, B, S, Q, K, idx_out, w, qs, query_width, st);
-    if (K <= 8) return launch_search<8, IdxT>(support, query, B, S, Q, K, idx_out, w, qs, query_width, st);
-    if (K <= 16) return launch_search<16, IdxT>(support, query, B, S, Q, K, idx_out, w, qs, query_width, st);
-    if (K <= 32) return launch_search<32, IdxT>(support, query, B, S, Q, K, idx_out, w, qs, query_width, st);
-    return launch_search<64, IdxT>(support, query, B, S, Q, K, idx_out, w, qs, query_width, st);
+                           const float4 *qorder, cudaStream_t st)
+{
+    if (K == 1) return launch_search<1, IdxT>(support, query, B, S, Q, K, idx_out, w, qs, query_width, qorder, st);
+    if (K <= 4) return launch_search<4, IdxT>(support, query, B, S, Q, K, idx_out, w, qs, query_width, qorder, st);
+    if (K <= 8) return launch_search<8, IdxT>(support, query, B, S, Q, K, idx_out, w, qs, query_width, qorder, st);
+    if (K <= 16) return launch_search<16, IdxT>(support, query, B, S, Q, K, idx_out, w, qs, query_width, qorder, st);
+    if (K <= 32) return launch_search<32, IdxT>(support, query, B, S, Q, K, idx_out, w, qs, query_width, qorder, st);
+    return launch_search<64, IdxT>(support, query, B, S, Q, K, idx_out, w, qs, query_width, qorder, st);
 }
 
 int knn_grid_build(const float *support, int64_t B, int64_t S, int K, void *grid_mem,
@@ -1463,7 +1534,8 @@
 
 int knn_grid_query(const float *support, const float *query, int64_t B, int64_t S, int64_t Q, int K,
                    void *idx_out, int idx_is_i64, const void *grid_mem, size_t grid_bytes,
-                   void *scratch, size_t scratch_bytes, cudaStream_t st, int64_t query_width)
+                   void *scratch, size_t scratch_bytes, cudaStream_t st, int64_t query_width,
+                   const void *query_grid, size_t query_grid_bytes)
 {
     read_env();
     GridStore w = carve_grid(const_cast<void *>(grid_mem), B, S);
@@ -1473,8 +1545,17 @@
                   scratch_bytes, qs.bytes);
         return FFB6D_ERR_WORKSPACE;
     }
-    if (idx_is_i64) return launch_search_k<long long>(support, query, B, S, Q, K, idx_out, w, qs, query_width, st);
-    return launch_search_k<int>(support, query, B, S, Q, K, idx_out, w, qs, query_width, st);
+    const float4 *qorder = nullptr;
+    if (query_grid) {
+        const GridStore qg = carve_grid(const_cast<void *>(query_grid), B, Q);
+        if (query_grid_bytes < qg.bytes) {
+            set_error("knn grid query: query grid too small (%zu/%zu)", query_grid_bytes, qg.bytes);
+            return FFB6D_ERR_WORKSPACE;
+        }
+        qorder = qg.sorted;
+    }
+    if (idx_is_i64) return launch_search_k<long long>(support, query, B, S, Q, K, idx_out, w, qs, query_width, qorder, st);
+    return launch_search_k<int>(support, query, B, S, Q, K, idx_out, w, qs, query_width, qorder, st);
 }
 
 int knn_grid_launch(const float *support, const float *query, int64_t B, int64_t S, int64_t Q, int K,
diff --git a/ffb6d_b200/csrc/schedule.cu b/ffb6d_b200/csrc/schedule.cu
--- a/ffb6d_b200/csrc/schedule.cu
+++ b/ffb6d_b200/csrc/schedule.cu
@@ -61,8 +61,32 @@
     out[t] = __ldg(in + (((b * Hp + (long long)r * f) * Wp + (long long)c * f) * words + wd));
 }
 
+static int prefix_parent(const Call (&calls)[22], int i)
+{
+    int p = -1;
+    if (calls[i].qry_kind != 0) return p;
+    for (int j = 0; j < 22; ++j)
+        if (j != i && calls[j].qry_kind == 0 && calls[j].sup_kind == calls[i].sup_kind && calls[j].sup_id == calls[i].sup_id &&
+            calls[j].K == calls[i].K && calls[j].qry_id < calls[i].qry_id && (p < 0 || calls[j].qry_id < calls[p].qry_id))
+            p = j;
+    return p;
+}
+
+static bool ordered_level(const Call (&calls)[22], const Sizes &z, int64_t B, int l)
+{
+    for (int j = 0; j < 22; ++j) {
+        const Call &c = calls[j];
+        if (c.sup_kind == 1 && c.qry_kind == 0 && c.qry_id == l && c.K >= 2 && c.K <= 16 && prefix_parent(calls, j) < 0 &&
+            knn_grid_workspace_bytes(B, z.img[c.sup_id], z.cld[l], c.K) > 0 &&
+            knn_grid_workspace_bytes(B, z.cld[l], z.cld[l], c.K) > 0)
+            return true;
+    }
+    return false;
+}
+
 struct Plan {
     size_t levels_off[5];
+    size_t qgrid_off[5];
     size_t grid_off, scratch_off, total;
 };
 
@@ -81,6 +105,11 @@
         const int64_t S = size_of(z, c.sup_kind, c.sup_id), Q = size_of(z, c.qry_kind, c.qry_id);
         if (S > 0) grid = std::max(grid, knn_grid_store_bytes(B, S));
         if (Q > 0) scratch = std::max(scratch, knn_grid_query_bytes(B, Q));
+    }
+    for (int l = 1; l < 5; ++l) {
+        if (!ordered_level(calls, z, B, l)) continue;
+        p.qgrid_off[l] = off;
+        off = align_up(off + knn_grid_store_bytes(B, z.cld[l]), 256);
     }
     p.grid_off = off;
     off = align_up(off + grid, 256);
@@ -135,15 +164,7 @@
     make_calls(K, calls);
     bool done[22] = {};
     int parent[22];
-    for (int i = 0; i < 22; ++i) {
-        parent[i] = -1;
-        if (calls[i].qry_kind != 0) continue;
-        for (int j = 0; j < 22; ++j)
-            if (j != i && calls[j].qry_kind == 0 && calls[j].sup_kind == calls[i].sup_kind && calls[j].sup_id == calls[i].sup_id &&
-                calls[j].K == calls[i].K && calls[j].qry_id < calls[i].qry_id &&
-                (parent[i] < 0 || calls[j].qry_id < calls[parent[i]].qry_id))
-                parent[i] = j;
-    }
+    for (int i = 0; i < 22; ++i) parent[i] = prefix_parent(calls, i);
     int stride_f[22];
     for (int i = 0; i < 22; ++i) {
         stride_f[i] = 0;
@@ -157,6 +178,13 @@
             }
     }
     void *grid = ws + plan.grid_off, *scratch = ws + plan.scratch_off;
+    bool qgrid_built[5] = {};
+    auto level_grid = [&](int l, void **g) {
+        *g = ws + plan.qgrid_off[l];
+        if (qgrid_built[l]) return (int)FFB6D_OK;
+        qgrid_built[l] = true;
+        return knn_grid_build(level[l], B, z.cld[l], K, *g, knn_grid_store_bytes(B, z.cld[l]), st);
+    };
     for (int i = 0; i < 22; ++i) {
         if (done[i]) continue;
         const Call &c = calls[i];
@@ -166,7 +194,11 @@
         for (int j = i; j < 22; ++j)
             if (calls[j].sup_kind == c.sup_kind && calls[j].sup_id == c.sup_id && calls[j].K == c.K)
                 use_grid = use_grid || knn_grid_workspace_bytes(B, S, size_of(z, calls[j].qry_kind, calls[j].qry_id), c.K) > 0;
-        if (use_grid) {
+        void *g = grid;
+        if (use_grid && c.sup_kind == 0 && c.K == K && plan.qgrid_off[c.sup_id]) {
+            const int rc = level_grid(c.sup_id, &g);
+            if (rc != FFB6D_OK) return rc;
+        } else if (use_grid) {
             const int rc = knn_grid_build(sup, B, S, c.K, grid, knn_grid_store_bytes(B, S), st);
             if (rc != FFB6D_OK) return rc;
         }
@@ -182,9 +214,16 @@
             if (from_self)
                 rc = knn_subset_nn_from_knn(sup, qry, B, S, Q, out[4 * d.qry_id], K, out[j], idx_is_i64, scratch,
                                             knn_grid_query_bytes(B, Q), st);
-            else if (use_grid)
-                rc = knn_grid_query(sup, qry, B, S, Q, d.K, out[j], idx_is_i64, grid, knn_grid_store_bytes(B, S), scratch,
-                                    knn_grid_query_bytes(B, Q), st, d.qry_kind == 1 ? W / d.qry_id : 0);
+            else if (use_grid) {
+                void *qg = nullptr;
+                if (d.sup_kind == 1 && d.qry_kind == 0 && d.K == K && d.K >= 2 && d.K <= 16 && plan.qgrid_off[d.qry_id]) {
+                    rc = level_grid(d.qry_id, &qg);
+                    if (rc != FFB6D_OK) return rc;
+                }
+                rc = knn_grid_query(sup, qry, B, S, Q, d.K, out[j], idx_is_i64, g, knn_grid_store_bytes(B, S), scratch,
+                                    knn_grid_query_bytes(B, Q), st, d.qry_kind == 1 ? W / d.qry_id : 0, qg,
+                                    qg ? knn_grid_store_bytes(B, Q) : 0);
+            }
             else
                 rc = knn_brute_launch(sup, qry, B, S, Q, d.K, out[j], idx_is_i64, st);
             if (rc != FFB6D_OK) return rc;
diff --git a/ffb6d_b200/ops.py b/ffb6d_b200/ops.py
--- a/ffb6d_b200/ops.py
+++ b/ffb6d_b200/ops.py
@@ -91,7 +91,7 @@
             check(lib.ffb6d_knn_grid_build(sup.data_ptr(), self.B, self.S, self.k_hint,
                                            self.mem.data_ptr(), self.nbytes, _stream(sup.device)))
 
-    def query(self, query_pts, k, out_dtype=None, query_width=0):
+    def query(self, query_pts, k, out_dtype=None, query_width=0, order=None):
         _need_cuda(query_pts, "query_pts")
         qry = self.support if query_pts is self.support else query_pts.contiguous().float()
         if qry.dim() != 3 or qry.shape[0] != self.B or qry.shape[2] != 3:
@@ -107,6 +107,14 @@
             sb = int(lib.ffb6d_knn_grid_query_bytes(self.B, Q))
             scratch = torch.empty(max(sb, 1), dtype=torch.uint8, device=dev)
             qw = int(query_width) if query_width and Q % int(query_width) == 0 else 0
+            if order is not None:
+                if order.B != self.B or order.S != Q:
+                    raise ValueError("order must be a KnnGrid of the %d queries, got one of %d points" % (Q, order.S))
+                check(lib.ffb6d_knn_grid_query_ordered(self.support.data_ptr(), qry.data_ptr(), self.B, self.S, Q, k,
+                                                       out.data_ptr(), int(dt == torch.int64), self.mem.data_ptr(),
+                                                       self.nbytes, scratch.data_ptr(), sb, order.mem.data_ptr(),
+                                                       order.nbytes, _stream(dev)))
+                return out
             check(lib.ffb6d_knn_grid_query_organized(self.support.data_ptr(), qry.data_ptr(), self.B, self.S, Q, k,
                                                      out.data_ptr(), int(dt == torch.int64), self.mem.data_ptr(),
                                                      self.nbytes, scratch.data_ptr(), sb, qw, _stream(dev)))
diff --git a/ffb6d_b200/schedule.py b/ffb6d_b200/schedule.py
--- a/ffb6d_b200/schedule.py
+++ b/ffb6d_b200/schedule.py
@@ -55,6 +55,10 @@
                if any(knn_uses_grid(B, sets[g[0]].shape[1], sets[q].shape[1], g[1]) for key_, q in members
                       if key_ not in derived_sub)]
     grids = {}
+
+    def order_grid(s, q, kk):
+        return (q, kk) if q[0] == "cld" and q != s and 2 <= kk <= 16 and (q, kk) in gridded else None
+
     main = torch.cuda.current_stream(cld.device)
     par = streams is not None and timer is None
     bstreams = list(build_streams) if (build_streams and par) else []
@@ -89,6 +93,8 @@
         first_use = {}
         for pos, (key, s_, q_, kk_) in enumerate(order):
             first_use.setdefault((s_, kk_), pos)
+            if order_grid(s_, q_, kk_):
+                first_use.setdefault(order_grid(s_, q_, kk_), pos)
         build_order = sorted(gridded, key=lambda g: first_use.get(g, len(order)))
     else:
         order = sorted(calls, key=lambda c: -(sets[c[2]].shape[1] * c[3])) if par else calls
@@ -111,10 +117,14 @@
             if timer is not None:
                 timer.start("knn:" + key, knn_alg_bytes(sup.shape[1], qry.shape[1], kk) * B)
             if (s, kk) in grids:
+                og = order_grid(s, q, kk)
                 if par:
                     torch.cuda.current_stream(cld.device).wait_event(built[(s, kk)])
+                    if og:
+                        torch.cuda.current_stream(cld.device).wait_event(built[og])
                 inputs[key] = grids[(s, kk)].query(qry, kk, out_dtype=index_dtype,
-                                                   query_width=(W // q[1]) if q[0] == "img" else 0)
+                                                   query_width=(W // q[1]) if q[0] == "img" else 0,
+                                                   order=grids[og] if og else None)
             else:
                 inputs[key] = knn_search(sup, qry, kk, out_dtype=index_dtype, algo=1)
             if timer is not None:
diff --git a/include/ffb6d_b200.h b/include/ffb6d_b200.h
--- a/include/ffb6d_b200.h
+++ b/include/ffb6d_b200.h
@@ -54,6 +54,12 @@
                                    const void *grid, size_t grid_bytes,
                                    void *scratch, size_t scratch_bytes,
                                    int64_t query_width, ffb6d_stream_t stream);
+int ffb6d_knn_grid_query_ordered(const float *support, const float *query,
+                                 int64_t B, int64_t S, int64_t Q, int K,
+                                 void *idx_out, int idx_is_i64,
+                                 const void *grid, size_t grid_bytes,
+                                 void *scratch, size_t scratch_bytes,
+                                 const void *query_grid, size_t query_grid_bytes, ffb6d_stream_t stream);
 
 int ffb6d_knn_subset_nn(const float *support, const float *query, int64_t B, int64_t S, int64_t Q,
                         const void *knn_idx, int K_list, void *idx_out, int idx_is_i64,
@@ -67,6 +73,7 @@
 
 void ffb6d_knn_grid_tune(float cell_scale, int quantile);
 void ffb6d_knn_grid_tune_k1(float cell_scale_k1);
+void ffb6d_knn_grid_tune_group(int width);
 
 int ffb6d_knn_batch_host(const float *batch_data, size_t batch_size, size_t npts, size_t dim,
                          const float *queries, size_t nqueries, size_t K, long *batch_indices);
```

Measured after the change: 86.31 million, median of 6. 2.2% higher.
